# yangl1996/hbbft

Measured on AMD Instinct MI355X. Metric: RBC encode+Merkle+decode payload GB/s, N=64, 1/8 GPUs; fraction of HBM peak, higher is better.
Workload: dtype u8; 1 GPU; cfg3: N=64 f=21 (22+42 shards), 262144 B payloads, 32768 instances/GPU, f random erasures; n=64, f=21, payload_bytes=262144, instances_per_gpu=32768, global_batch=32768, parallelism=instance-sharded x1

## Files before the change

__graft_entry__.py:

```python
import os
import subprocess
import sys

ROOT = os.path.dirname(os.path.abspath(__file__))


def build_jobs():
    try:
        return max(1, int(os.environ["MAX_JOBS"]))
    except (KeyError, ValueError):
        return max(1, min(16, len(os.sched_getaffinity(0))))


def build():
    jobs = str(min(8, build_jobs()))
    oracle = subprocess.Popen(["make", "-s", "-j", "2", "-C", os.path.join(ROOT, "oracle")])
    try:
        subprocess.check_call(["make", "-s", "-j", jobs, "-C",
                               os.path.join(ROOT, "hbbft_amd", "csrc")])
    finally:
        rc = oracle.wait()
    if rc != 0:
        raise subprocess.CalledProcessError(rc, oracle.args)
    subprocess.check_call(["make", "-s", "-C", os.path.join(ROOT, "tests", "cpp")])
    if ROOT not in sys.path:
        sys.path.insert(0, ROOT)
    import hbbft_amd
    hbbft_amd.lib()
    todo = [t for t in jit_tasks() if not os.path.exists(
        os.path.join(ROOT, "hbbft_amd", "jit", _jit_name(*t)))]
    if todo:
        from concurrent.futures import ThreadPoolExecutor
        todo.sort(key=lambda t: -t[1] * t[2])
        with ThreadPoolExecutor(min(len(todo), build_jobs())) as pool:
            list(pool.map(_jit_spawn, todo))


def jit_tasks():
    if ROOT not in sys.path:
        sys.path.insert(0, ROOT)
    import hbbft_amd
    from hbbft_amd.sharded import Topology
    tasks = []
    for k, m in SPECIALISED:
        n = k + m
        for rb in [0] + [r for r in VALIDATOR_BLOCKS.get(n, []) if r < n]:
            tasks += [("enc", k, m, g, rb, None) for g in range(hbbft_amd.jit_encode_groups(k, m))]
    for n, pres, rb in decoder_patterns(Topology):
        f = (n - 1) // 3
        k, m = n - 2 * f, 2 * f
        kinds = ["dec", "decuf"]
        tasks += [(kind, k, m, g, rb, tuple(pres)) for kind in kinds
                  for g in range(hbbft_amd.jit_decode_groups(k, m, pres))]
    return tasks


def decoder_patterns(Topology):
    out = []
    n = 250
    f = (n - 1) // 3
    k = n - 2 * f
    out.append((n, [1 if k <= i < 2 * k else 0 for i in range(n)], 0))
    for nv in (16, 64, 128):
        for world in (1, 2, 4, 8):
            t = Topology(nv, world)
            for g in range(world):
                out.append((nv, t.receiver_present(g), t.rows_per_block))
    return out


def _jit_name(kind, k, m, group, rb, present):
    import hbbft_amd
    if kind == "enc":
        return hbbft_amd.jit_file_name(k, m, group, rb)
    return hbbft_amd.jit_decode_file_name(k, m, list(present), group, rb,
                                          fused_unframe=kind == "decuf")


_JIT_CHILD = ("import json, sys; sys.path.insert(0, sys.argv[1]); import __graft_entry__ as g; "
              "g._jit_one(*json.loads(sys.argv[2]))")


def _jit_spawn(task):
    import json
    subprocess.run([sys.executable, "-c", _JIT_CHILD, ROOT, json.dumps(task)], check=True,
                   stdin=subprocess.DEVNULL)


def _jit_one(kind, k, m, group, rb, present):
    if ROOT not in sys.path:
        sys.path.insert(0, ROOT)
    import hbbft_amd
    if kind == "enc":
        hbbft_amd.jit_build_encode(k, m, group=group, rows_per_block=rb)
    else:
        hbbft_amd.jit_build_decode(k, m, list(present), group, rows_per_block=rb,
                                   fused_unframe=kind == "decuf")


SPECIALISED = [(2, 2), (6, 10), (22, 42), (44, 84), (84, 166)]
VALIDATOR_BLOCKS = {16: [8, 4, 2], 64: [32, 16, 8], 128: [64, 32, 16]}


def smoke():
    if ROOT not in sys.path:
        sys.path.insert(0, ROOT)
    import numpy as np
    import torch

    import hbbft_amd as hb
    from oracle import pyoracle as orc

    assert torch.cuda.is_available(), "smoke() needs a GPU"
    from hbbft_amd.srchash import source_hash
    ver = hb.lib().hbrbc_version().decode()
    print("smoke: %s (tree src=%s)" % (ver, source_hash()))
    assert ver.endswith("src=" + source_hash()), "libhbrbc.so was not built from these sources"
    n, f, plen, count = 16, 5, 3000, 8
    rb = hb.RbcBatch(n, f, device=0)
    S = hb.shard_len(plen, rb.k)
    pay = np.stack([orc.gen_payload(7, i, plen) for i in range(count)])
    stride_p = (plen + 15) // 16 * 16
    payloads = torch.zeros((count, stride_p), dtype=torch.uint8, device="cuda:0")
    payloads[:, :plen] = torch.from_numpy(pay).cuda()
    slab = rb.alloc_slab(count, S)
    nodes = rb.alloc_nodes(count)
    rb.frame(payloads, plen, slab)
    rb.encode(slab, S)
    rb.merkle(slab, S, nodes)
    digests = torch.zeros((count, n, rb.dslots, 32), dtype=torch.uint8, device="cuda:0")
    ndig = torch.zeros((count, n), dtype=torch.uint8, device="cuda:0")
    rb.proofs(nodes, digests, ndig)
    ok = torch.zeros((count, n), dtype=torch.uint8, device="cuda:0")
    rb.validate(slab, S, digests, ndig, nodes, ok)
    present = torch.from_numpy(np.stack([orc.gen_present(9, i, n, f) for i in range(count)])).cuda()
    roots = nodes[:, -1, :].clone()
    slab2 = slab.clone()
    slab2[present == 0] = 0xA5
    nodes2 = rb.alloc_nodes(count)
    out = torch.zeros((count, (rb.k * S + 15) // 16 * 16), dtype=torch.uint8, device="cuda:0")
    plen_out = torch.zeros(count, dtype=torch.int32, device="cuda:0")
    status = torch.zeros(count, dtype=torch.int32, device="cuda:0")
    rb.decode(slab2, S, present, roots, nodes2, out, plen_out, status)
    torch.cuda.synchronize()
    slab_h, nodes_h = slab.cpu().numpy(), nodes.cpu().numpy()
    for i in range(count):
        sh, nd = orc.send_shards(n, f, pay[i].tobytes())
        assert np.array_equal(slab_h[i, :, :S], sh), "shards differ from oracle"
        assert np.array_equal(nodes_h[i], nd), "merkle nodes differ from oracle"
    assert ok.cpu().numpy().all(), "a valid proof was rejected"
    assert (status.cpu().numpy() == 0).all(), status
    assert (plen_out.cpu().numpy() == plen).all()
    assert np.array_equal(out.cpu().numpy()[:, :plen], pay), "decoded payload differs"
    print("smoke ok: N=%d f=%d P=%d x%d instances, bit-exact vs oracle" % (n, f, plen, count))

    from hbbft_amd import threshold as T
    from oracle import bls_oracle as B
    p1, q2 = B.g1_mul(B.G1_GEN, 5), B.g2_mul(B.G2_GEN, 7)
    g1 = torch.from_numpy(np.frombuffer(B.g1_bytes(p1), np.uint8).copy()).view(1, 96).cuda()
    g2 = torch.from_numpy(np.frombuffer(B.g2_bytes(q2), np.uint8).copy()).view(1, 192).cuda()
    gt, st = T.pairing_batch(g1, g2)
    assert st.item() == 0 and bytes(gt[0].cpu().numpy()) == B.gt_bytes(B.pairing(p1, q2)), \
        "pairing differs from oracle"
    cases = [B.decryption_share_case(3, 4, 5), B.decryption_share_case(3, 4, 5, tamper=True)]
    got = T.verify_decryption_shares([(B.g1_bytes(s), B.g1_bytes(pk), B.g2_bytes(h), B.g2_bytes(w))
                                      for s, h, pk, w in cases])
    assert got == [True, False], got
    print("smoke ok: BLS12-381 pairing bit-exact, decryption-share checks exact")


if __name__ == "__main__":
    build()
    if len(sys.argv) > 1 and sys.argv[1] == "smoke":
        smoke()
```

hbbft-hip/src/ffi.rs:

```rust
#![allow(non_camel_case_types, dead_code, clippy::too_many_arguments)]
use std::os::raw::{c_char, c_int, c_void};

#[repr(C)]
pub struct HbrbcCtx {
    _p: [u8; 0],
}

#[repr(C)]
#[derive(Clone, Copy)]
pub struct HbrbcSmArgs {
    pub count: usize,
    pub node_lo: u32,
    pub nodes: u32,
    pub rows_per_rank: u32,
    pub roots: u32,
    pub max_out: u32,
    pub max_faults: u32,
    pub round: i32,
    pub proposer: *const u8,
    pub role: *const u8,
    pub value_root: *const u8,
    pub value_tamper: *const u8,
    pub proof_ok: *const u8,
    pub decode_ok: *const u8,
    pub fake_from: *const u8,
    pub fake_root: *const u8,
    pub fake_list: *const u32,
    pub in_: *const u32,
    pub in_count: *const u32,
    pub out: *mut u32,
    pub out_count: *mut u32,
    pub state: *mut u8,
    pub output_root: *mut u8,
    pub faults: *mut u16,
    pub fault_count: *mut u32,
    pub emitted: *mut u32,
    pub active: *const u32,
    pub flags: u32,
}

extern "C" {
    pub fn hbrbc_last_error() -> *const c_char;
    pub fn hbrbc_version() -> *const c_char;
    pub fn hbrbc_coding_new(data_shards: usize, parity_shards: usize, device: c_int, out: *mut *mut HbrbcCtx) -> c_int;
    pub fn hbrbc_coding_free(ctx: *mut HbrbcCtx);
    pub fn hbrbc_data_shard_count(ctx: *const HbrbcCtx) -> usize;
    pub fn hbrbc_parity_shard_count(ctx: *const HbrbcCtx) -> usize;
    pub fn hbrbc_encoding_matrix(ctx: *const HbrbcCtx, out: *mut u8) -> c_int;
    pub fn hbrbc_stream(ctx: *const HbrbcCtx) -> *mut c_void;
    pub fn hbrbc_encode(ctx: *mut HbrbcCtx, shards: *const *mut u8, lens: *const usize, n_shards: usize) -> c_int;
    pub fn hbrbc_reconstruct(ctx: *mut HbrbcCtx, shards: *const *mut u8, lens: *const usize, present: *const u8, n_shards: usize) -> c_int;
    pub fn hbrbc_merkle_node_count(n: usize) -> usize;
    pub fn hbrbc_merkle_max_proof_len(n: usize) -> usize;
    pub fn hbrbc_merkle_build(values: *const *const u8, lens: *const usize, n: usize, nodes_out: *mut u8) -> c_int;
    pub fn hbrbc_merkle_proof(nodes: *const u8, n: usize, index: usize, digests_out: *mut u8, ndig_out: *mut usize) -> c_int;
    pub fn hbrbc_proof_validate(value: *const u8, len: usize, index: usize, digests: *const u8, ndig: usize, root: *const u8, n: usize, valid_out: *mut c_int) -> c_int;
    pub fn hbrbc_shard_len(payload_len: usize, data_shards: usize) -> usize;
    pub fn hbrbc_frame_batch(ctx: *mut HbrbcCtx, payloads: *const u8, payload_stride: usize, payload_len: usize, count: usize, shards: *mut u8, shard_len: usize, shard_stride: usize, inst_stride: usize, stream: *mut c_void) -> c_int;
    pub fn hbrbc_encode_batch(ctx: *mut HbrbcCtx, shards: *mut u8, shard_len: usize, shard_stride: usize, inst_stride: usize, count: usize, stream: *mut c_void) -> c_int;
    pub fn hbrbc_frame_encode_batch(ctx: *mut HbrbcCtx, payloads: *const u8, payload_stride: usize, payload_len: usize, count: usize, shards: *mut u8, shard_len: usize, shard_stride: usize, inst_stride: usize, stream: *mut c_void) -> c_int;
    pub fn hbrbc_frame_encode_ragged(ctx: *mut HbrbcCtx, payloads: *const u8, payload_stride: usize, payload_lens: *const u32, max_payload_len: usize, count: usize, shards: *mut u8, shard_stride: usize, inst_stride: usize, stream: *mut c_void) -> c_int;
    pub fn hbrbc_merkle_ragged(ctx: *mut HbrbcCtx, shards: *const u8, shard_lens: *const u32, shard_stride: usize, inst_stride: usize, count: usize, nodes: *mut u8, node_inst_stride: usize, stream: *mut c_void) -> c_int;
    pub fn hbrbc_merkle_batch(ctx: *mut HbrbcCtx, shards: *const u8, shard_len: usize, shard_stride: usize, inst_stride: usize, count: usize, nodes: *mut u8, node_inst_stride: usize, stream: *mut c_void) -> c_int;
    pub fn hbrbc_proofs_batch(ctx: *mut HbrbcCtx, nodes: *const u8, node_inst_stride: usize, count: usize, digests: *mut u8, ndig: *mut u8, stream: *mut c_void) -> c_int;
    pub fn hbrbc_validate_batch(ctx: *mut HbrbcCtx, values: *const u8, value_len: usize, value_stride: usize, value_inst_stride: usize, per_inst: usize, indices: *const u32, digests: *const u8, ndig: *const u8, roots: *const u8, root_stride: usize, tree_n: usize, count: usize, ok_out: *mut u8, stream: *mut c_void) -> c_int;
    pub fn hbrbc_reconstruct_batch(ctx: *mut HbrbcCtx, shards: *mut u8, shard_len: usize, shard_stride: usize, inst_stride: usize, present: *const u8, count: usize, status_out: *mut i32, stream: *mut c_void) -> c_int;
    pub fn hbrbc_decode_batch(ctx: *mut HbrbcCtx, shards: *mut u8, shard_len: usize, shard_stride: usize, inst_stride: usize, present: *const u8, count: usize, roots: *const u8, root_stride: usize, nodes: *mut u8, node_inst_stride: usize, payload_out: *mut u8, payload_stride: usize, payload_len_out: *mut u32, status_out: *mut i32, stream: *mut c_void) -> c_int;
    pub fn hbrbc_reserve(ctx: *mut HbrbcCtx, count: usize) -> c_int;
    pub fn hbrbc_frame_encode_rows(ctx: *mut HbrbcCtx, payloads: *const u8, payload_stride: usize, payload_len: usize, count: usize, shards: *mut u8, shard_len: usize, shard_stride: usize, rows_per_block: usize, block_stride: usize, inst_stride: usize, stream: *mut c_void) -> c_int;
    pub fn hbrbc_merkle_rows(ctx: *mut HbrbcCtx, shards: *const u8, shard_len: usize, shard_stride: usize, rows_per_block: usize, block_stride: usize, inst_stride: usize, count: usize, nodes: *mut u8, node_inst_stride: usize, stream: *mut c_void) -> c_int;
    pub fn hbrbc_validate_rows(ctx: *mut HbrbcCtx, values: *const u8, value_len: usize, value_stride: usize, rows_per_block: usize, block_stride: usize, value_inst_stride: usize, per_inst: usize, rows: *const u32, indices: *const u32, digests: *const u8, ndig: *const u8, digest_rows: usize, roots: *const u8, root_stride: usize, tree_n: usize, count: usize, ok_out: *mut u8, leaf_out: *mut u8, leaf_inst_stride: usize, stream: *mut c_void) -> c_int;
    pub fn hbrbc_reconstruct_rows(ctx: *mut HbrbcCtx, shards: *mut u8, shard_len: usize, shard_stride: usize, rows_per_block: usize, block_stride: usize, inst_stride: usize, present: *const u8, count: usize, status_out: *mut i32, stream: *mut c_void) -> c_int;
    pub fn hbrbc_decode_rows(ctx: *mut HbrbcCtx, shards: *mut u8, shard_len: usize, shard_stride: usize, rows_per_block: usize, block_stride: usize, inst_stride: usize, present: *const u8, count: usize, roots: *const u8, root_stride: usize, nodes: *mut u8, node_inst_stride: usize, known_leaves: c_int, payload_out: *mut u8, payload_stride: usize, payload_len_out: *mut u32, status_out: *mut i32, stream: *mut c_void) -> c_int;
    pub fn hbrbc_drop_rows(ctx: *mut HbrbcCtx, shards: *mut u8, shard_stride: usize, rows_per_block: usize, block_stride: usize, inst_stride: usize, present: *const u8, count: usize, fill: u8, stream: *mut c_void) -> c_int;
    pub fn hbrbc_decode_cache_clear(ctx: *mut HbrbcCtx) -> c_int;
    pub fn hbrbc_decode_cache_fill(ctx: *mut HbrbcCtx, patterns_out: *mut u32) -> c_int;
    pub fn hbrbc_decoder_specialise(ctx: *mut HbrbcCtx, present: *const u8, rows_per_block: usize) -> c_int;
    pub fn hbrbc_wire_proof_message_len(value_len: usize, ndig: usize) -> usize;
    pub fn hbrbc_wire_encode_batch(ctx: *mut HbrbcCtx, variant: u32, values: *const u8, value_len: usize, value_stride: usize, value_inst_stride: usize, per_inst: usize, indices: *const u32, digests: *const u8, ndig: *const u8, roots: *const u8, root_stride: usize, count: usize, out: *mut u8, msg_stride: usize, msg_len_out: *mut u32, stream: *mut c_void) -> c_int;
    pub fn hbrbc_wire_decode_batch(ctx: *mut HbrbcCtx, msgs: *const u8, msg_stride: usize, msg_len: *const u32, nmsg: usize, values: *mut u8, value_stride: usize, value_len_out: *mut u32, index_out: *mut u32, digests: *mut u8, ndig_out: *mut u8, roots: *mut u8, variant_out: *mut u32, status_out: *mut i32, stream: *mut c_void) -> c_int;
    pub fn hbrbc_encode_kernel(ctx: *const HbrbcCtx) -> *const c_char;
    pub fn hbrbc_jit_build_encode(data_shards: usize, parity_shards: usize, dir: *const c_char) -> c_int;
    pub fn hbrbc_jit_encode_groups(data_shards: usize, parity_shards: usize) -> usize;
    pub fn hbrbc_jit_build_encode_group(data_shards: usize, parity_shards: usize, group: usize, dir: *const c_char) -> c_int;
    pub fn hbrbc_jit_file_name(data_shards: usize, parity_shards: usize, group: usize, buf: *mut c_char, buf_len: usize) -> c_int;
    pub fn hbrbc_jit_build_encode_rows(data_shards: usize, parity_shards: usize, group: usize, rows_per_block: usize, dir: *const c_char) -> c_int;
    pub fn hbrbc_jit_encode_file_name(data_shards: usize, parity_shards: usize, group: usize, rows_per_block: usize, buf: *mut c_char, buf_len: usize) -> c_int;
    pub fn hbrbc_jit_decode_groups(data_shards: usize, parity_shards: usize, present: *const u8) -> usize;
    pub fn hbrbc_jit_build_decode(data_shards: usize, parity_shards: usize, present: *const u8, rows_per_block: usize, group: usize, dir: *const c_char) -> c_int;
    pub fn hbrbc_jit_build_decode_variant(data_shards: usize, parity_shards: usize, present: *const u8, rows_per_block: usize, group: usize, fused_unframe: c_int, dir: *const c_char) -> c_int;
    pub fn hbrbc_jit_decode_variant_file_name(data_shards: usize, parity_shards: usize, present: *const u8, rows_per_block: usize, group: usize, fused_unframe: c_int, buf: *mut c_char, buf_len: usize) -> c_int;
    pub fn hbrbc_jit_decode_file_name(data_shards: usize, parity_shards: usize, present: *const u8, rows_per_block: usize, group: usize, buf: *mut c_char, buf_len: usize) -> c_int;
    pub fn hbrbc_profile_enable(ctx: *mut HbrbcCtx, enable: c_int) -> c_int;
    pub fn hbrbc_profile_reset(ctx: *mut HbrbcCtx) -> c_int;
    pub fn hbrbc_profile_read(ctx: *mut HbrbcCtx, ms_out: *mut f64, launches_out: *mut u64) -> c_int;
    pub fn hbrbc_stage_name(stage: c_int) -> *const c_char;
    pub fn hbrbc_unframe_fused(ctx: *const HbrbcCtx, shard_len: usize, payload_stride: usize, rows_per_block: usize) -> c_int;
    pub fn hbrbc_pairing_workspace_size(pairings: usize) -> usize;
    pub fn hbrbc_pairing_batch(g1: *const u8, g2: *const u8, count: usize, gt_out: *mut u8, status_out: *mut u8, workspace: *mut c_void, stream: *mut c_void) -> c_int;
    pub fn hbrbc_pairing_check_batch(g1: *const u8, g2: *const u8, count: usize, ok_out: *mut u8, workspace: *mut c_void, stream: *mut c_void) -> c_int;
    pub fn hbrbc_g2_prepared_size(points: usize) -> usize;
    pub fn hbrbc_g2_prepare(g2: *const u8, count: usize, prepared: *mut c_void, stream: *mut c_void) -> c_int;
    pub fn hbrbc_pairing_check_prepared(g1: *const u8, prepared: *const c_void, points: usize, idx_b: *const u32, idx_d: *const u32, count: usize, ok_out: *mut u8, workspace: *mut c_void, stream: *mut c_void) -> c_int;
    pub fn hbrbc_g1_prepared_size(points: usize) -> usize;
    pub fn hbrbc_g1_prepare(g1: *const u8, count: usize, prepared: *mut c_void, stream: *mut c_void) -> c_int;
    pub fn hbrbc_pairing_check_prepared_keys(g1_a: *const u8, keys: *const c_void, key_points: usize, idx_c: *const u32, prepared: *const c_void, points: usize, idx_b: *const u32, idx_d: *const u32, count: usize, ok_out: *mut u8, workspace: *mut c_void, stream: *mut c_void) -> c_int;
    pub fn hbrbc_pairing_check_prepared_pts(a_prepared: *const c_void, keys: *const c_void, key_points: usize, idx_c: *const u32, prepared: *const c_void, points: usize, idx_b: *const u32, idx_d: *const u32, count: usize, ok_out: *mut u8, workspace: *mut c_void, stream: *mut c_void) -> c_int;
    pub fn hbrbc_pairing_check(a: *const u8, b: *const u8, c: *const u8, d: *const u8, result: *mut c_int) -> c_int;
    pub fn hbrbc_g1_combine_workspace_size(total_shares: usize, groups: usize) -> usize;
    pub fn hbrbc_lagrange_coeffs(idx: *const u32, offsets: *const u32, groups: usize, coeffs_out: *mut u8, status_out: *mut u8, stream: *mut c_void) -> c_int;
    pub fn hbrbc_g1_lincomb_prepared(a_prepared: *const c_void, prepared_count: usize, rows: *const i32, scalars: *const u8, offsets: *const u32, groups: usize, out96: *mut u8, out48: *mut u8, status_out: *mut u8, workspace: *mut c_void, stream: *mut c_void) -> c_int;
    pub fn hbrbc_decrypt_combine_prepared(a_prepared: *const c_void, prepared_count: usize, rows: *const i32, idx: *const u32, offsets: *const u32, groups: usize, out96: *mut u8, out48: *mut u8, status_out: *mut u8, workspace: *mut c_void, stream: *mut c_void) -> c_int;
    pub fn hbrbc_decrypt_combine(shares: *const u8, idx: *const u32, n: usize, out96: *mut u8, out48: *mut u8) -> c_int;
    pub fn hbrbc_g1_poly_eval_prepared(a_prepared: *const c_void, prepared_count: usize, rows: *const i32, offsets: *const u32, polys: usize, poly: *const i32, x: *const u32, evals: usize, out_table: *mut c_void, out96: *mut u8, out48: *mut u8, status_out: *mut u8, stream: *mut c_void) -> c_int;
    pub fn hbrbc_g1_base_mul_check(a_prepared: *const c_void, prepared_count: usize, rows: *const i32, scalars: *const u8, count: usize, ok_out: *mut u8, stream: *mut c_void) -> c_int;
    pub fn hbrbc_g2_points_size(points: usize) -> usize;
    pub fn hbrbc_g2_points_prepare(g2: *const u8, count: usize, table: *mut c_void, stream: *mut c_void) -> c_int;
    pub fn hbrbc_sig_check_prepared(sig_table: *const c_void, sig_count: usize, keys: *const c_void, key_points: usize, idx_key: *const u32, prepared: *const c_void, points: usize, idx_h: *const u32, count: usize, ok_out: *mut u8, workspace: *mut c_void, stream: *mut c_void) -> c_int;
    pub fn hbrbc_g2_combine_workspace_size(total_shares: usize, groups: usize) -> usize;
    pub fn hbrbc_g2_lincomb_prepared(sig_table: *const c_void, sig_count: usize, rows: *const i32, scalars: *const u8, offsets: *const u32, groups: usize, out192: *mut u8, out96: *mut u8, parity_out: *mut u8, status_out: *mut u8, workspace: *mut c_void, stream: *mut c_void) -> c_int;
    pub fn hbrbc_sig_combine_prepared(sig_table: *const c_void, sig_count: usize, rows: *const i32, idx: *const u32, offsets: *const u32, groups: usize, out192: *mut u8, out96: *mut u8, parity_out: *mut u8, status_out: *mut u8, workspace: *mut c_void, stream: *mut c_void) -> c_int;
    pub fn hbrbc_sig_combine(shares: *const u8, idx: *const u32, n: usize, out192: *mut u8, out96: *mut u8, parity: *mut u8) -> c_int;
    pub fn hbrbc_g1_prepare_compressed(g1c: *const u8, count: usize, prepared: *mut c_void, stream: *mut c_void) -> c_int;
    pub fn hbrbc_g2_points_prepare_compressed(g2c: *const u8, count: usize, table: *mut c_void, stream: *mut c_void) -> c_int;
    pub fn hbrbc_g1_decompress(g1c: *const u8, count: usize, out96: *mut u8, status: *mut u8, stream: *mut c_void) -> c_int;
    pub fn hbrbc_g2_decompress(g2c: *const u8, count: usize, out192: *mut u8, status: *mut u8, stream: *mut c_void) -> c_int;
    pub fn hbrbc_g1_base_mul(scalars: *const u8, count: usize, out_table: *mut c_void, out96: *mut u8, out48: *mut u8, status_out: *mut u8, stream: *mut c_void) -> c_int;
    pub fn hbrbc_g1_mul_prepared(a_prepared: *const c_void, prepared_count: usize, rows: *const i32, scalars: *const u8, nscalars: usize, sidx: *const i32, count: usize, out_table: *mut c_void, out96: *mut u8, out48: *mut u8, status_out: *mut u8, stream: *mut c_void) -> c_int;
    pub fn hbrbc_g2_mul_prepared(table: *const c_void, table_count: usize, rows: *const i32, scalars: *const u8, nscalars: usize, sidx: *const i32, count: usize, out_table: *mut c_void, out192: *mut u8, out96: *mut u8, status_out: *mut u8, stream: *mut c_void) -> c_int;
    pub fn hbrbc_fr_poly_eval(scalars: *const u8, nscalars: usize, rows: *const i32, offsets: *const u32, polys: usize, poly: *const i32, x: *const u32, evals: usize, out: *mut u8, status_out: *mut u8, stream: *mut c_void) -> c_int;
    pub fn hbrbc_fr_dot(a: *const u8, b: *const u8, offsets: *const u32, groups: usize, total: usize, out: *mut u8, status_out: *mut u8, stream: *mut c_void) -> c_int;
    pub fn hbrbc_sm_state_bytes(n: usize, roots: usize) -> usize;
    pub fn hbrbc_sm_round(ctx: *mut HbrbcCtx, args: *const HbrbcSmArgs, stream: *mut c_void) -> c_int;
}
```

hbbft_amd/__init__.py:

```python
import ctypes
import os

__all__ = [
    "RseError", "HbrbcUnavailable", "Coding", "MerkleTree", "Proof", "RbcBatch",
    "shard_len", "merkle_node_count", "max_proof_len", "lib", "LIB_PATH", "STAGES",
    "jit_build_encode", "jit_file_name", "WIRE_VARIANTS", "validate_proofs", "VALIDATE_STATS",
    "send_shards_batch", "SEND_STATS", "jit_decode_groups", "jit_build_decode",
    "jit_decode_file_name", "jit_encode_groups",
]

_HERE = os.path.dirname(os.path.abspath(__file__))
LIB_PATH = os.environ.get("HBRBC_LIB") or os.path.join(_HERE, "libhbrbc.so")

STATUS_NAMES = {
    0: "Ok", 1: "TooFewShards", 2: "TooManyShards", 3: "TooFewDataShards",
    4: "TooManyDataShards", 5: "TooFewParityShards", 6: "TooManyParityShards",
    7: "TooFewBufferShards", 8: "TooManyBufferShards", 9: "IncorrectShardSize",
    10: "TooFewShardsPresent", 11: "EmptyShard", 12: "InvalidShardFlags", 13: "InvalidIndex",
    64: "SingularMatrix", 65: "RootMismatch", 66: "NoPayloadLen",
    70: "WireTruncated", 71: "WireBadVariant", 72: "WireTooLarge",
    100: "InvalidArgument", 101: "DeviceError", 102: "NoDevice",
}
WIRE_VARIANTS = {"Value": 0, "Echo": 1, "Ready": 2, "CanDecode": 3, "EchoHash": 4}
STAGES = ["frame", "encode", "leaf_hash", "tree_levels", "proofs", "validate",
          "decode_matrix", "reconstruct", "unframe"]


class HbrbcUnavailable(RuntimeError):
    """libhbrbc.so is missing or no HIP device is visible (no fallback exists)."""


class RseError(Exception):

    def __init__(self, code, msg=""):
        self.code = code
        self.msg = msg
        self.name = STATUS_NAMES.get(code, "Status%d" % code)
        super().__init__("%s%s" % (self.name, (": " + msg) if msg else ""))

    def __reduce__(self):
        return (RseError, (self.code, self.msg))


_lib = None
_P = ctypes.c_void_p
_S = ctypes.c_size_t


def lib():
    global _lib
    if _lib is not None:
        return _lib
    if not os.path.exists(LIB_PATH):
        raise HbrbcUnavailable("%s not built (run __graft_entry__.build())" % LIB_PATH)
    L = ctypes.CDLL(LIB_PATH)
    sig = {
        "hbrbc_last_error": (ctypes.c_char_p, []),
        "hbrbc_version": (ctypes.c_char_p, []),
        "hbrbc_coding_new": (ctypes.c_int, [_S, _S, ctypes.c_int, ctypes.POINTER(_P)]),
        "hbrbc_coding_free": (None, [_P]),
        "hbrbc_data_shard_count": (_S, [_P]),
        "hbrbc_parity_shard_count": (_S, [_P]),
        "hbrbc_encoding_matrix": (ctypes.c_int, [_P, _P]),
        "hbrbc_stream": (_P, [_P]),
        "hbrbc_encode": (ctypes.c_int, [_P, _P, _P, _S]),
        "hbrbc_reconstruct": (ctypes.c_int, [_P, _P, _P, _P, _S]),
        "hbrbc_merkle_node_count": (_S, [_S]),
        "hbrbc_merkle_max_proof_len": (_S, [_S]),
        "hbrbc_merkle_build": (ctypes.c_int, [_P, _P, _S, _P]),
        "hbrbc_merkle_proof": (ctypes.c_int, [_P, _S, _S, _P, ctypes.POINTER(_S)]),
        "hbrbc_proof_validate": (ctypes.c_int, [_P, _S, _S, _P, _S, _P, _S,
                                                ctypes.POINTER(ctypes.c_int)]),
        "hbrbc_shard_len": (_S, [_S, _S]),
        "hbrbc_frame_batch": (ctypes.c_int, [_P, _P, _S, _S, _S, _P, _S, _S, _S, _P]),
        "hbrbc_encode_batch": (ctypes.c_int, [_P, _P, _S, _S, _S, _S, _P]),
        "hbrbc_frame_encode_batch": (ctypes.c_int, [_P, _P, _S, _S, _S, _P, _S, _S, _S, _P]),
        "hbrbc_merkle_batch": (ctypes.c_int, [_P, _P, _S, _S, _S, _S, _P, _S, _P]),
        "hbrbc_proofs_batch": (ctypes.c_int, [_P, _P, _S, _S, _P, _P, _P]),
        "hbrbc_validate_batch": (ctypes.c_int, [_P, _P, _S, _S, _S, _S, _P, _P, _P, _P, _S, _S,
                                                _S, _P, _P]),
        "hbrbc_reconstruct_batch": (ctypes.c_int, [_P, _P, _S, _S, _S, _P, _S, _P, _P]),
        "hbrbc_decode_batch": (ctypes.c_int, [_P, _P, _S, _S, _S, _P, _S, _P, _S, _P, _S, _P, _S,
                                              _P, _P, _P]),
        "hbrbc_reserve": (ctypes.c_int, [_P, _S]),
        "hbrbc_profile_enable": (ctypes.c_int, [_P, ctypes.c_int]),
        "hbrbc_profile_reset": (ctypes.c_int, [_P]),
        "hbrbc_profile_read": (ctypes.c_int, [_P, _P, _P]),
        "hbrbc_stage_name": (ctypes.c_char_p, [ctypes.c_int]),
        "hbrbc_encode_kernel": (ctypes.c_char_p, [_P]),
        "hbrbc_wire_proof_message_len": (_S, [_S, _S]),
        "hbrbc_wire_encode_batch": (ctypes.c_int, [_P, ctypes.c_uint32, _P, _S, _S, _S, _S, _P, _P,
                                                   _P, _P, _S, _S, _P, _S, _P, _P]),
        "hbrbc_wire_decode_batch": (ctypes.c_int, [_P, _P, _S, _P, _S, _P, _S, _P, _P, _P, _P, _P,
                                                   _P, _P, _P]),
        "hbrbc_jit_build_encode": (ctypes.c_int, [_S, _S, ctypes.c_char_p]),
        "hbrbc_jit_encode_groups": (_S, [_S, _S]),
        "hbrbc_jit_build_encode_group": (ctypes.c_int, [_S, _S, _S, ctypes.c_char_p]),
        "hbrbc_jit_file_name": (ctypes.c_int, [_S, _S, _S, ctypes.c_char_p, _S]),
        "hbrbc_frame_encode_rows": (ctypes.c_int, [_P, _P, _S, _S, _S, _P, _S, _S, _S, _S, _S, _P]),
        "hbrbc_frame_encode_ragged": (ctypes.c_int, [_P, _P, _S, _P, _S, _S, _P, _S, _S, _P]),
        "hbrbc_merkle_ragged": (ctypes.c_int, [_P, _P, _P, _S, _S, _S, _P, _S, _P]),
        "hbrbc_merkle_rows": (ctypes.c_int, [_P, _P, _S, _S, _S, _S, _S, _S, _P, _S, _P]),
        "hbrbc_validate_rows": (ctypes.c_int, [_P, _P, _S, _S, _S, _S, _S, _S, _P, _P, _P, _P, _S,
                                               _P, _S, _S, _S, _P, _P, _S, _P]),
        "hbrbc_reconstruct_rows": (ctypes.c_int, [_P, _P, _S, _S, _S, _S, _S, _P, _S, _P, _P]),
        "hbrbc_decode_rows": (ctypes.c_int, [_P, _P, _S, _S, _S, _S, _S, _P, _S, _P, _S, _P, _S,
                                             ctypes.c_int, _P, _S, _P, _P, _P]),
        "hbrbc_decode_cache_clear": (ctypes.c_int, [_P]),
        "hbrbc_decode_cache_fill": (ctypes.c_int, [_P, ctypes.POINTER(ctypes.c_uint32)]),
        "hbrbc_decoder_specialise": (ctypes.c_int, [_P, _P, _S]),
        "hbrbc_jit_build_encode_rows": (ctypes.c_int, [_S, _S, _S, _S, ctypes.c_char_p]),
        "hbrbc_jit_encode_file_name": (ctypes.c_int, [_S, _S, _S, _S, ctypes.c_char_p, _S]),
        "hbrbc_jit_decode_groups": (_S, [_S, _S, _P]),
        "hbrbc_jit_build_decode": (ctypes.c_int, [_S, _S, _P, _S, _S, ctypes.c_char_p]),
        "hbrbc_jit_decode_file_name": (ctypes.c_int, [_S, _S, _P, _S, _S, ctypes.c_char_p, _S]),
        "hbrbc_jit_build_decode_variant": (ctypes.c_int, [_S, _S, _P, _S, _S, ctypes.c_int,
                                                          ctypes.c_char_p]),
        "hbrbc_jit_decode_variant_file_name": (ctypes.c_int, [_S, _S, _P, _S, _S, ctypes.c_int,
                                                              ctypes.c_char_p, _S]),
        "hbrbc_unframe_fused": (ctypes.c_int, [_P, _S, _S, _S]),
        "hbrbc_drop_rows": (ctypes.c_int, [_P, _P, _S, _S, _S, _S, _P, _S, ctypes.c_uint8, _P]),
        "hbrbc_pairing_workspace_size": (_S, [_S]),
        "hbrbc_g2_prepared_size": (_S, [_S]),
        "hbrbc_g2_prepare": (ctypes.c_int, [_P, _S, _P, _P]),
        "hbrbc_pairing_check_prepared": (ctypes.c_int, [_P, _P, _S, _P, _P, _S, _P, _P, _P]),
        "hbrbc_pairing_batch": (ctypes.c_int, [_P, _P, _S, _P, _P, _P, _P]),
        "hbrbc_pairing_check_batch": (ctypes.c_int, [_P, _P, _S, _P, _P, _P]),
        "hbrbc_g1_prepared_size": (_S, [_S]),
        "hbrbc_g1_prepare": (ctypes.c_int, [_P, _S, _P, _P]),
        "hbrbc_pairing_check_prepared_keys": (ctypes.c_int, [_P, _P, _S, _P, _P, _S, _P, _P, _S, _P,
                                                             _P, _P]),
        "hbrbc_pairing_check_prepared_pts": (ctypes.c_int, [_P, _P, _S, _P, _P, _S, _P, _P, _S, _P,
                                                            _P, _P]),
        "hbrbc_pairing_check": (ctypes.c_int, [ctypes.c_char_p, ctypes.c_char_p, ctypes.c_char_p,
                                               ctypes.c_char_p, ctypes.POINTER(ctypes.c_int)]),
        "hbrbc_g1_combine_workspace_size": (_S, [_S, _S]),
        "hbrbc_lagrange_coeffs": (ctypes.c_int, [_P, _P, _S, _P, _P, _P]),
        "hbrbc_g1_lincomb_prepared": (ctypes.c_int, [_P, _S, _P, _P, _P, _S, _P, _P, _P, _P, _P]),
        "hbrbc_decrypt_combine_prepared": (ctypes.c_int, [_P, _S, _P, _P, _P, _S, _P, _P, _P, _P,
                                                          _P]),
        "hbrbc_decrypt_combine": (ctypes.c_int, [ctypes.c_char_p, _P, _S, ctypes.c_char_p,
                                                 ctypes.c_char_p]),
        "hbrbc_g2_points_size": (_S, [_S]),
        "hbrbc_g2_points_prepare": (ctypes.c_int, [_P, _S, _P, _P]),
        "hbrbc_sig_check_prepared": (ctypes.c_int, [_P, _S, _P, _S, _P, _P, _S, _P, _S, _P, _P,
                                                    _P]),
        "hbrbc_g2_combine_workspace_size": (_S, [_S, _S]),
        "hbrbc_g2_lincomb_prepared": (ctypes.c_int, [_P, _S, _P, _P, _P, _S, _P, _P, _P, _P, _P,
                                                     _P]),
        "hbrbc_sig_combine_prepared": (ctypes.c_int, [_P, _S, _P, _P, _P, _S, _P, _P, _P, _P, _P,
                                                      _P]),
        "hbrbc_sig_combine": (ctypes.c_int, [ctypes.c_char_p, _P, _S, ctypes.c_char_p,
                                             ctypes.c_char_p, ctypes.c_char_p]),
        "hbrbc_g1_prepare_compressed": (ctypes.c_int, [_P, _S, _P, _P]),
        "hbrbc_g2_points_prepare_compressed": (ctypes.c_int, [_P, _S, _P, _P]),
        "hbrbc_g1_decompress": (ctypes.c_int, [_P, _S, _P, _P, _P]),
        "hbrbc_g2_decompress": (ctypes.c_int, [_P, _S, _P, _P, _P]),
        "hbrbc_g1_poly_eval_prepared": (ctypes.c_int, [_P, _S, _P, _P, _S, _P, _P, _S, _P, _P, _P,
                                                       _P, _P]),
        "hbrbc_g1_base_mul_check": (ctypes.c_int, [_P, _S, _P, _P, _S, _P, _P]),
        "hbrbc_g1_base_mul": (ctypes.c_int, [_P, _S, _P, _P, _P, _P, _P]),
        "hbrbc_g1_mul_prepared": (ctypes.c_int, [_P, _S, _P, _P, _S, _P, _S, _P, _P, _P, _P, _P]),
        "hbrbc_g2_mul_prepared": (ctypes.c_int, [_P, _S, _P, _P, _S, _P, _S, _P, _P, _P, _P, _P]),
        "hbrbc_fr_poly_eval": (ctypes.c_int, [_P, _S, _P, _P, _S, _P, _P, _S, _P, _P, _P]),
        "hbrbc_fr_dot": (ctypes.c_int, [_P, _P, _P, _S, _S, _P, _P, _P]),
    }
    for name, (res, args) in sig.items():
        fn = getattr(L, name)
        fn.restype = res
        fn.argtypes = args
    _lib = L
    return L


def _check(code):
    if code == 102:
        raise HbrbcUnavailable(lib().hbrbc_last_error().decode(errors="replace") or "no HIP device")
    if code != 0:
        raise RseError(code, lib().hbrbc_last_error().decode(errors="replace"))


def jit_build_encode(data_shards, parity_shards, directory=None, group=None, rows_per_block=0):
    d = directory.encode() if directory else None
    groups = range(jit_encode_groups(data_shards, parity_shards)) if group is None else [group]
    for g in groups:
        _check(lib().hbrbc_jit_build_encode_rows(data_shards, parity_shards, g, rows_per_block, d))


def jit_file_name(data_shards, parity_shards, group=0, rows_per_block=0):
    buf = ctypes.create_string_buffer(256)
    _check(lib().hbrbc_jit_encode_file_name(data_shards, parity_shards, group, rows_per_block,
                                            buf, 256))
    return buf.value.decode()


def _mask_buffer(present):
    import numpy as np
    return np.ascontiguousarray(np.asarray(present, dtype=np.uint8) != 0, dtype=np.uint8)


def jit_decode_groups(data_shards, parity_shards, present):
    m = _mask_buffer(present)
    return lib().hbrbc_jit_decode_groups(data_shards, parity_shards, m.ctypes.data)


def jit_build_decode(data_shards, parity_shards, present, group, rows_per_block=0,
                     directory=None, fused_unframe=False):
    m = _mask_buffer(present)
    d = directory.encode() if directory else None
    _check(lib().hbrbc_jit_build_decode_variant(data_shards, parity_shards, m.ctypes.data,
                                                rows_per_block, group, int(fused_unframe), d))


def jit_decode_file_name(data_shards, parity_shards, present, group=0, rows_per_block=0,
                         fused_unframe=False):
    m = _mask_buffer(present)
    buf = ctypes.create_string_buffer(256)
    _check(lib().hbrbc_jit_decode_variant_file_name(data_shards, parity_shards, m.ctypes.data,
                                                    rows_per_block, group, int(fused_unframe),
                                                    buf, 256))
    return buf.value.decode()


def jit_encode_groups(data_shards, parity_shards):
    return lib().hbrbc_jit_encode_groups(data_shards, parity_shards)


def shard_len(payload_len, data_shards):
    return (payload_len + 4 + data_shards - 1) // data_shards


def merkle_node_count(n):
    total, sz = 0, n
    while True:
        total += sz
        if sz <= 1:
            return total
        sz = (sz + 1) // 2


def max_proof_len(n):
    d, sz = 0, n
    while sz > 1:
        d += 1
        sz = (sz + 1) // 2
    return d


def _as_buffer(b):
    import numpy as np
    if isinstance(b, np.ndarray):
        assert b.dtype == np.uint8 and b.flags.c_contiguous
        return b
    if isinstance(b, bytearray):
        return np.frombuffer(b, dtype=np.uint8)
    return np.frombuffer(bytearray(b), dtype=np.uint8)


def _addr(a):
    return a.ctypes.data if a.size else 0


class Coding:

    def __init__(self, data_shard_num, parity_shard_num, device=-1):
        h = _P()
        _check(lib().hbrbc_coding_new(data_shard_num, parity_shard_num, device, ctypes.byref(h)))
        self._h = h

    @classmethod
    def for_validators(cls, n, device=-1):
        f = (n - 1) // 3
        return cls(n - 2 * f, 2 * f, device)

    @property
    def handle(self):
        return self._h

    def close(self):
        if self._h:
            lib().hbrbc_coding_free(self._h)
            self._h = None

    def __del__(self):
        try:
            self.close()
        except Exception:
            pass

    def data_shard_count(self):
        return lib().hbrbc_data_shard_count(self._h)

    def encode_kernel(self):
        return lib().hbrbc_encode_kernel(self._h).decode()

    def parity_shard_count(self):
        return lib().hbrbc_parity_shard_count(self._h)

    def encoding_matrix(self):
        import numpy as np
        k, m = self.data_shard_count(), self.parity_shard_count()
        out = np.zeros((k + m, k), np.uint8)
        _check(lib().hbrbc_encoding_matrix(self._h, out.ctypes.data))
        return out

    def encode(self, shards):
# ... 242 lines not shown
                                        slab.stride(0), slab.shape[0], self._stream(stream)))

    def merkle(self, slab, S, nodes, stream=None):
        _check(lib().hbrbc_merkle_batch(self.coding.handle, _ptr(slab), S, slab.stride(1),
                                        slab.stride(0), slab.shape[0], _ptr(nodes),
                                        nodes.stride(0), self._stream(stream)))

    def proofs(self, nodes, digests, ndig, stream=None):
        _check(lib().hbrbc_proofs_batch(self.coding.handle, _ptr(nodes), nodes.stride(0),
                                        nodes.shape[0], _ptr(digests), _ptr(ndig),
                                        self._stream(stream)))

    def validate(self, slab, S, digests, ndig, nodes, ok, indices=None, leaf_out=None,
                 stream=None):
        count = slab.shape[0]
        root = nodes[:, -1, :]
        if leaf_out is not None:
            self.validate_layout(slab, S, count, self.n, slab.stride(1), 0, 0, slab.stride(0),
                                 digests, ndig, self.n, root, ok, indices=indices,
                                 leaf_out=leaf_out, stream=stream)
            return
        _check(lib().hbrbc_validate_batch(self.coding.handle, _ptr(slab), S, slab.stride(1),
                                          slab.stride(0), self.n, _ptr(indices), _ptr(digests),
                                          _ptr(ndig), _ptr(root), nodes.stride(0), self.n,
                                          count, _ptr(ok), self._stream(stream)))

    def validate_rows(self, values, S, per_inst, indices, digests, ndig, roots, ok, stream=None):
        count = values.shape[0]
        for t in (indices, digests, ndig, ok):
            assert t.is_contiguous() and t.shape[0] == count and t.shape[1] == per_inst
        _check(lib().hbrbc_validate_batch(self.coding.handle, _ptr(values), S, values.stride(1),
                                          values.stride(0), per_inst, _ptr(indices), _ptr(digests),
                                          _ptr(ndig), _ptr(roots), roots.stride(0), self.n, count,
                                          _ptr(ok), self._stream(stream)))

    def frame_encode_ragged(self, payloads, plens, max_plen, slab, stream=None):
        _check(lib().hbrbc_frame_encode_ragged(self.coding.handle, _ptr(payloads),
                                               payloads.stride(0), _ptr(plens), max_plen,
                                               slab.shape[0], _ptr(slab), slab.stride(1),
                                               slab.stride(0), self._stream(stream)))

    def merkle_ragged(self, slab, slens, nodes, stream=None):
        _check(lib().hbrbc_merkle_ragged(self.coding.handle, _ptr(slab), _ptr(slens),
                                         slab.stride(1), slab.stride(0), slab.shape[0],
                                         _ptr(nodes), nodes.stride(0), self._stream(stream)))

    def frame_encode_rows(self, payloads, plen, base, count, shard_stride, rows_per_block,
                          block_stride, inst_stride, stream=None):
        S = shard_len(plen, self.k)
        _check(lib().hbrbc_frame_encode_rows(self.coding.handle, _ptr(payloads), payloads.stride(0),
                                             plen, count, _ptr(base), S, shard_stride,
                                             rows_per_block, block_stride, inst_stride,
                                             self._stream(stream)))

    def merkle_rows(self, base, S, count, shard_stride, rows_per_block, block_stride, inst_stride,
                    nodes, stream=None):
        _check(lib().hbrbc_merkle_rows(self.coding.handle, _ptr(base), S, shard_stride,
                                       rows_per_block, block_stride, inst_stride, count,
                                       _ptr(nodes), nodes.stride(0), self._stream(stream)))

    def validate_layout(self, base, S, count, per_inst, shard_stride, rows_per_block, block_stride,
                        inst_stride, digests, ndig, digest_rows, roots, ok, rows=None,
                        indices=None, leaf_out=None, stream=None):
        _check(lib().hbrbc_validate_rows(
            self.coding.handle, _ptr(base), S, shard_stride, rows_per_block, block_stride,
            inst_stride, per_inst, _ptr(rows), _ptr(indices), _ptr(digests), _ptr(ndig),
            digest_rows, _ptr(roots), roots.stride(0), self.n, count, _ptr(ok), _ptr(leaf_out),
            leaf_out.stride(0) if leaf_out is not None else 0, self._stream(stream)))

    def decode_rows(self, base, S, count, shard_stride, rows_per_block, block_stride, inst_stride,
                    present, roots, nodes, payload_out, plen_out, status, known_leaves=False,
                    stream=None):
        _check(lib().hbrbc_decode_rows(
            self.coding.handle, _ptr(base), S, shard_stride, rows_per_block, block_stride,
            inst_stride, _ptr(present), count, _ptr(roots), roots.stride(0), _ptr(nodes),
            nodes.stride(0), 1 if known_leaves else 0, _ptr(payload_out), payload_out.stride(0),
            _ptr(plen_out), _ptr(status), self._stream(stream)))

    def specialise_decoder(self, present, rows_per_block=0):
        m = _mask_buffer(present)
        assert m.size == self.n
        _check(lib().hbrbc_decoder_specialise(self.coding.handle, m.ctypes.data, rows_per_block))

    def decode_cache_clear(self):
        _check(lib().hbrbc_decode_cache_clear(self.coding.handle))

    def decode_cache_fill(self):
        v = ctypes.c_uint32(0)
        _check(lib().hbrbc_decode_cache_fill(self.coding.handle, ctypes.byref(v)))
        return v.value

    def reconstruct(self, slab, S, present, status, stream=None):
        _check(lib().hbrbc_reconstruct_batch(self.coding.handle, _ptr(slab), S, slab.stride(1),
                                             slab.stride(0), _ptr(present), slab.shape[0],
                                             _ptr(status), self._stream(stream)))

    def drop_rows(self, slab, present, fill=0xA5, stream=None):
        _check(lib().hbrbc_drop_rows(self.coding.handle, _ptr(slab), slab.stride(1), 0, 0,
                                     slab.stride(0), _ptr(present), slab.shape[0], fill,
                                     self._stream(stream)))

    def unframe_fused(self, S, payload_stride, rows_per_block=0):
        return bool(lib().hbrbc_unframe_fused(self.coding.handle, S, payload_stride,
                                              rows_per_block))

    def decode(self, slab, S, present, roots, nodes, payload_out, plen_out, status,
               known_leaves=False, stream=None):
        if known_leaves:
            self.decode_rows(slab, S, slab.shape[0], slab.stride(1), 0, 0, slab.stride(0),
                             present, roots, nodes, payload_out, plen_out, status,
                             known_leaves=True, stream=stream)
            return
        _check(lib().hbrbc_decode_batch(self.coding.handle, _ptr(slab), S, slab.stride(1),
                                        slab.stride(0), _ptr(present), slab.shape[0],
                                        _ptr(roots), roots.stride(0), _ptr(nodes),
                                        nodes.stride(0), _ptr(payload_out),
                                        payload_out.stride(0), _ptr(plen_out), _ptr(status),
                                        self._stream(stream)))

    def wire_slot(self, S):
        return (lib().hbrbc_wire_proof_message_len(S, self.dslots) + 15) // 16 * 16

    def wire_encode(self, values, S, digests, ndig, roots, out, msg_len, variant=0, indices=None,
                    stream=None):
        count, per_inst = values.shape[0], values.shape[1]
        _check(lib().hbrbc_wire_encode_batch(self.coding.handle, variant, _ptr(values), S,
                                             values.stride(1), values.stride(0), per_inst,
                                             _ptr(indices), _ptr(digests), _ptr(ndig),
                                             _ptr(roots), roots.stride(0), count, _ptr(out),
                                             out.stride(0), _ptr(msg_len), self._stream(stream)))

    def wire_decode(self, msgs, msg_len, values, value_len, index, digests, ndig, roots, variant,
                    status, stream=None):
        _check(lib().hbrbc_wire_decode_batch(self.coding.handle, _ptr(msgs), msgs.stride(0),
                                             _ptr(msg_len), msgs.shape[0], _ptr(values),
                                             values.stride(0), _ptr(value_len), _ptr(index),
                                             _ptr(digests), _ptr(ndig), _ptr(roots), _ptr(variant),
                                             _ptr(status), self._stream(stream)))

    def own_stream(self):
        import torch
        return torch.cuda.ExternalStream(lib().hbrbc_stream(self.coding.handle), device=self.device)

    def reserve(self, count):
        _check(lib().hbrbc_reserve(self.coding.handle, count))

    def profile(self, enable=True):
        _check(lib().hbrbc_profile_enable(self.coding.handle, 1 if enable else 0))

    def profile_reset(self):
        _check(lib().hbrbc_profile_reset(self.coding.handle))

    def profile_read(self):
        ms = (ctypes.c_double * len(STAGES))()
        cnt = (ctypes.c_uint64 * len(STAGES))()
        _check(lib().hbrbc_profile_read(self.coding.handle, ms, cnt))
        return {STAGES[i]: (ms[i], cnt[i]) for i in range(len(STAGES))}


SEND_STATS = {"trees": 0, "launches": 0}
_SEND_BATCH = {}


def send_shards_batch(items, device=0):
    import numpy as np
    import torch
# ... 91 lines not shown
```

hbbft_amd/csrc/api.hip:

```cpp
#include <hip/hip_runtime.h>

#include <algorithm>
#include <cstdarg>
#include <cstdio>
#include <cstdlib>
#include <cstring>
#include <map>
#include <mutex>
#include <string>
#include <vector>

#include <dlfcn.h>
#include <sys/stat.h>

#include "../../include/hbrbc.h"
#include "device_common.hpp"
#include "jit.hpp"
#include "launchers.hpp"

using namespace hbrbc;

namespace {

thread_local std::string g_err;
// ... 138 lines not shown
            p = nullptr;
            cap = 0;
        }
        size_t b = round_up(bytes < 256 ? 256 : bytes, 256);
        hipError_t e = hipMalloc(&p, b);
        if (e == hipSuccess) cap = b;
        return e;
    }
    void release() {
        if (p) (void)hipFree(p);
        p = nullptr;
        cap = 0;
    }
    template <class T>
    T *as() const {
        return static_cast<T *>(p);
    }
};

struct PinBuf {
    void *p = nullptr;
    size_t cap = 0;
    hipError_t ensure(size_t bytes) {
        if (bytes <= cap) return hipSuccess;
        if (p) {
            (void)hipHostFree(p);
            p = nullptr;
            cap = 0;
        }
        size_t b = round_up(bytes < 4096 ? 4096 : bytes, 4096);
        hipError_t e = hipHostMalloc(&p, b, hipHostMallocDefault);
        if (e == hipSuccess) cap = b;
        return e;
    }
    void release() {
        if (p) (void)hipHostFree(p);
        p = nullptr;
        cap = 0;
    }
    template <class T>
    T *as() const {
        return static_cast<T *>(p);
    }
};

RowMap make_rows(size_t n, size_t shard_stride, size_t rows_per_block, size_t block_stride) {
    RowMap r = plain_rows(shard_stride);
    if (rows_per_block && rows_per_block < n) {
        r.rb = (uint32_t)rows_per_block;
        r.bst = block_stride;
    }
    return r;
}
inline int code_rb(const RowMap &r) { return r.plain() ? 256 : (int)r.rb; }

}

struct hbrbc_ctx {
    int device = 0;
    size_t k = 0, m = 0, n = 0;
    int rt_enc = 2, rt_rec = 2;
    int gf_mode = 0;
    std::vector<uint8_t> matrix;
    hipStream_t stream = nullptr;
    struct SpecGroup {
        int r_lo, r_hi;
        hipModule_t mod;
        hipFunction_t fn, fe;
        bool lds = false;
    };
    std::map<int, std::vector<SpecGroup>> enc_spec;
    int rt_spec = 2;
    int depth_spec = 4;
    std::string enc_kind = "none";
    struct DecSpec {
        uint64_t hash;
        int rt;
        std::vector<SpecGroup> groups;
        std::vector<SpecGroup> uf_groups;
        int uf_state = 0;
        std::vector<uint8_t> present;
    };
    std::map<int, DecSpec> dec_spec;
    std::string jit_missing;
    std::vector<hipStream_t> side;
    std::vector<hipEvent_t> side_ev;
    DevBuf d_matrix, d_enc_coefs, d_enc_in, d_enc_out;
    size_t ws_count = 0;
    int pc_cap = 0;
    size_t pc_inserted = 0;
    DevBuf pc_hash, pc_keys, pc_coefs, pc_in, pc_out, pc_nout, pc_status, pc_fill;
    DevBuf ws_pat, ws_own, ws_status, ws_list, ws_counter;
    std::mutex shim_mu;
    DevBuf st_slab, st_nodes, st_aux;
    PinBuf pin;
    bool prof = false;
    std::vector<hipEvent_t> ev_pool;
    size_t ev_used = 0;
    struct Rec {
        int stage;
        hipEvent_t a, b;
    };
    std::vector<Rec> recs;

    hipEvent_t take_event() {
        if (ev_used == ev_pool.size()) {
            hipEvent_t e;
            if (hipEventCreate(&e) != hipSuccess) return nullptr;
            ev_pool.push_back(e);
        }
        return ev_pool[ev_used++];
    }
    size_t coef_stride() const { return (m + rt_rec - 1) / rt_rec * k * 16 + 16; }
};

namespace {

struct StageTimer {
    hbrbc_ctx *c;
    int stage;
    hipStream_t s;
    hipEvent_t a = nullptr;
    StageTimer(hbrbc_ctx *c_, int st, hipStream_t s_) : c(c_), stage(st), s(s_) {
        if (c && c->prof) {
            a = c->take_event();
            if (a) (void)hipEventRecord(a, s);
        }
    }
    ~StageTimer() {
        if (a) {
            hipEvent_t b = c->take_event();
            if (b) {
                (void)hipEventRecord(b, s);
                c->recs.push_back({stage, a, b});
            }
        }
    }
};

inline hipStream_t pick(hbrbc_ctx *, void *stream) { return static_cast<hipStream_t>(stream); }

int check_slab(const void *base, size_t shard_len, size_t shard_stride, size_t inst_stride,
               size_t n, size_t count, size_t rows_per_block = 0, size_t block_stride = 0) {
    if (count == 0) return HBRBC_OK;
    if (!base) return fail(HBRBC_E_INVALID_ARG, "null shard slab");
    if (reinterpret_cast<uintptr_t>(base) % 16)
        return fail(HBRBC_E_INVALID_ARG, "shard slab base must be 16-byte aligned");
    if (shard_stride % 16 || shard_stride < shard_len)
        return fail(HBRBC_E_INVALID_ARG, "shard_stride %zu must be a multiple of 16 and >= %zu",
                    shard_stride, shard_len);
    if (shard_len > 0xFFFFFFFFull) return fail(HBRBC_E_INVALID_ARG, "shard_len too large");
    if (rows_per_block && rows_per_block < n) {
        if (rows_per_block > 255)
            return fail(HBRBC_E_INVALID_ARG, "rows_per_block %zu > 255", rows_per_block);
        if (block_stride % 16 || inst_stride % 16 || inst_stride < rows_per_block * shard_stride)
            return fail(HBRBC_E_INVALID_ARG, "blocked layout: inst_stride %zu must be a multiple "
                        "of 16 and >= rows_per_block * shard_stride", inst_stride);
        if (block_stride < count * inst_stride)
            return fail(HBRBC_E_INVALID_ARG, "blocked layout: block_stride %zu < count * "
                        "inst_stride", block_stride);
        if ((uint64_t)rows_per_block * shard_stride >= 0x7FFFFFFFull)
            return fail(HBRBC_E_INVALID_ARG, "row block larger than 2 GiB");
        return HBRBC_OK;
    }
    if (count > 1 && (inst_stride % 16 || inst_stride < n * shard_stride))
        return fail(HBRBC_E_INVALID_ARG, "inst_stride %zu must be a multiple of 16 and >= %zu",
                    inst_stride, n * shard_stride);
    return HBRBC_OK;
}

int check_nodes(const void *nodes, size_t node_inst_stride, size_t n, size_t count) {
    if (count == 0) return HBRBC_OK;
    if (!nodes || reinterpret_cast<uintptr_t>(nodes) % 16)
        return fail(HBRBC_E_INVALID_ARG, "node slab must be non-null and 16-byte aligned");
    if (node_inst_stride % 16 || (count > 1 && node_inst_stride < 32 * hbrbc_merkle_node_count(n)))
        return fail(HBRBC_E_INVALID_ARG, "node_inst_stride %zu too small or unaligned",
                    node_inst_stride);
    return HBRBC_OK;
}

int ensure_workspace(hbrbc_ctx *c, size_t count) {
    if (count <= c->ws_count) return HBRBC_OK;
    const size_t k = c->k, m = c->m;
    int cap = 1024;
    while ((size_t)cap < 2 * count) cap *= 2;
    const size_t slots = (size_t)cap + count;
    HB_HIP(c->pc_hash.ensure((size_t)cap * sizeof(uint64_t)));
    HB_HIP(c->pc_keys.ensure(slots * 8 * sizeof(uint32_t)));
    HB_HIP(c->pc_coefs.ensure(slots * c->coef_stride()));
    HB_HIP(c->pc_in.ensure((slots * k + 4) * sizeof(uint32_t)));
    HB_HIP(c->pc_out.ensure((slots * m + 4) * sizeof(uint32_t)));
    HB_HIP(c->pc_nout.ensure(slots * sizeof(int)));
    HB_HIP(c->pc_status.ensure(slots * sizeof(int32_t)));
    HB_HIP(c->pc_fill.ensure(sizeof(uint32_t)));
    HB_HIP(c->ws_pat.ensure(count * sizeof(int)));
    HB_HIP(c->ws_own.ensure(count));
    HB_HIP(c->ws_status.ensure(count * sizeof(int32_t)));
    HB_HIP(c->ws_list.ensure((count * std::max<size_t>(m, 1) + 1) * sizeof(uint2)));
    HB_HIP(c->ws_counter.ensure(sizeof(uint32_t)));
    HB_HIP(hipMemset(c->pc_hash.p, 0, (size_t)cap * sizeof(uint64_t)));
    HB_HIP(hipMemset(c->pc_fill.p, 0, sizeof(uint32_t)));
    c->pc_cap = cap;
    c->pc_inserted = 0;
    c->ws_count = count;
    return HBRBC_OK;
}

PatternCache cache_view(hbrbc_ctx *c) {
    PatternCache pc;
    pc.hash = c->pc_hash.as<uint64_t>();
    pc.keys = c->pc_keys.as<uint32_t>();
    pc.coefs = c->pc_coefs.as<uint8_t>();
    pc.coef_stride = c->coef_stride();
    pc.in_idx = c->pc_in.as<uint32_t>();
    pc.out_idx = c->pc_out.as<uint32_t>();
    pc.nout = c->pc_nout.as<int>();
    pc.status = c->pc_status.as<int32_t>();
    pc.fill = c->pc_fill.as<uint32_t>();
    pc.cap = c->pc_cap;
    return pc;
}

bool merkle_split() {
    const char *e = getenv("HBRBC_MERKLE_FUSED");
    return !(e && !std::strcmp(e, "1"));
}

int run_merkle(hbrbc_ctx *c, const uint8_t *shards, size_t shard_len, const RowMap &rows,
               size_t inst_stride, size_t n, size_t count, uint8_t *nodes,
               size_t node_inst_stride, bool known_leaves, hipStream_t s) {
    if (!known_leaves && merkle_fused_ok(n) && !merkle_split()) {
        StageTimer t(c, HBRBC_STAGE_LEAF_HASH, s);
        HB_HIP(launch_merkle_fused(shards, shard_len, rows, inst_stride, n, count, nodes,
                                   node_inst_stride, s));
        return HBRBC_OK;
    }
    {
        StageTimer t(c, HBRBC_STAGE_LEAF_HASH, s);
        if (!known_leaves) {
            HB_HIP(launch_leaf_hash(shards, shard_len, rows, inst_stride, n, count, nodes,
                                    node_inst_stride, s));
        } else if (c->m > 0) {
            HB_HIP(launch_leaf_hash_rebuilt(shards, shard_len, rows, inst_stride, count,
                                            c->ws_pat.as<int>(), c->pc_out.as<uint32_t>(), c->m,
                                            c->pc_nout.as<int>(), (int)c->m, nodes,
                                            node_inst_stride, c->ws_counter.as<uint32_t>(),
                                            c->ws_list.as<uint2>(), s));
        }
    }
    StageTimer t(c, HBRBC_STAGE_TREE_LEVELS, s);
    const char *lv = getenv("HBRBC_TREE_LEVELS_LDS");
    if (n <= 512 && lv && !std::strcmp(lv, "1")) {
        HB_HIP(launch_tree_levels(nodes, node_inst_stride, n, count, s));
        return HBRBC_OK;
    }
    size_t off = 0, sz = n;
    while (sz > 1) {
        const size_t nsz = (sz + 1) / 2;
        HB_HIP(launch_tree_level(nodes, node_inst_stride, off, sz, off + sz, nsz, count, s));
        off += sz;
        sz = nsz;
    }
    return HBRBC_OK;
}

hipError_t launch_xor_group(const hbrbc_ctx::SpecGroup &g, bool fused, int rt, XorArgs a,
                            size_t count, hipStream_t s);
hipError_t launch_groups(hbrbc_ctx *c, const std::vector<hbrbc_ctx::SpecGroup> &gs, size_t first,
                         int rt, const XorArgs &x, size_t count, hipStream_t s);

bool unframe_fusable(const hbrbc_ctx *c, size_t shard_len, size_t payload_stride) {
    const char *e = getenv("HBRBC_UNFRAME_FUSED");
    if (e && !std::strcmp(e, "0")) return false;
    return c->m > 0 && payload_stride % 16 == 0 && (uint64_t)c->k * shard_len > 4;
}

enum JitMode { JIT_DEFAULT, JIT_OFF, JIT_COMPILE, JIT_LOAD };
JitMode jit_mode() {
    const char *e = getenv("HBRBC_JIT");
    if (!e) return JIT_DEFAULT;
    if (!std::strcmp(e, "0")) return JIT_OFF;
    if (!std::strcmp(e, "1")) return JIT_COMPILE;
    if (!std::strcmp(e, "load")) return JIT_LOAD;
    return JIT_DEFAULT;
}

bool decode_programs(const std::vector<uint8_t> &mat, size_t k, size_t n, const uint8_t *present,
                     int rb, std::vector<XorProgram> &out, uint64_t &hash, int &rt, bool uf);
int load_program(const XorProgram &p, bool compile, hbrbc_ctx::SpecGroup &g);
void drop_groups(std::vector<hbrbc_ctx::SpecGroup> &gs);

bool uf_decoder(hbrbc_ctx *c, hbrbc_ctx::DecSpec &d, int rb) {
    if (d.uf_state == 0) {
        std::vector<XorProgram> progs;
        uint64_t hash = 0;
        int rt = 2;
        const bool compile = jit_mode() == JIT_DEFAULT || jit_mode() == JIT_COMPILE;
        const std::string saved = g_err;
        d.uf_state = -1;
        if (decode_programs(c->matrix, c->k, c->n, d.present.data(), rb, progs, hash, rt, true)) {
            d.uf_state = 1;
            for (const auto &p : progs) {
                hbrbc_ctx::SpecGroup g{0, (int)p.out_rows.size(), nullptr, nullptr, nullptr};
                if (load_program(p, compile, g)) {
                    drop_groups(d.uf_groups);
                    d.uf_state = -1;
                    break;
                }
                d.uf_groups.push_back(g);
            }
        }
        g_err = saved;
    }
    return d.uf_state == 1;
}

int run_reconstruct(hbrbc_ctx *c, uint8_t *shards, size_t shard_len, const RowMap &rows,
                    size_t inst_stride, const uint8_t *present, size_t count, int32_t *status,
                    hipStream_t s, uint8_t *uf_payload = nullptr, size_t uf_stride = 0,
                    bool *fused_out = nullptr) {
    if (fused_out) *fused_out = false;
    int st = ensure_workspace(c, count);
    if (st) return st;
    if (c->pc_inserted + count > 4 * (size_t)c->pc_cap) {
        HB_HIP(hipMemsetAsync(c->pc_hash.p, 0, (size_t)c->pc_cap * sizeof(uint64_t), s));
        HB_HIP(hipMemsetAsync(c->pc_fill.p, 0, sizeof(uint32_t), s));
        c->pc_inserted = 0;
    }
    c->pc_inserted += count;
    const auto ds = c->dec_spec.find(code_rb(rows));
    const bool spec = ds != c->dec_spec.end() && !ds->second.groups.empty();
    {
        StageTimer t(c, HBRBC_STAGE_DECODE_MATRIX, s);
        DecodeMatrixArgs a;
        a.n = (int)c->n;
        a.k = (int)c->k;
        a.rt = c->rt_rec;
        a.matrix = c->d_matrix.as<uint8_t>();
        a.present = present;
        a.count = count;
        a.cache = cache_view(c);
        a.pat = c->ws_pat.as<int>();
        a.own = c->ws_own.as<uint8_t>();
        a.status = status;
        if (spec) {
            a.spec_hash = ds->second.hash;
            pattern_mask(ds->second.present.data(), (int)c->n, a.spec_mask);
        }
        HB_HIP(launch_decode_matrix(a, s));
    }
    if (c->m == 0) return HBRBC_OK;
    StageTimer t(c, HBRBC_STAGE_RECONSTRUCT, s);
    if (spec && uf_payload && !uf_decoder(c, ds->second, code_rb(rows))) uf_payload = nullptr;
    if (spec) {
        XorArgs x{};
        x.base = shards;
        x.inst_stride = inst_stride;
        x.shard_stride = rows.sst;
        x.block_stride = rows.bst;
        x.row_bytes = (unsigned)round_up(shard_len, 16);
        x.pat = c->ws_pat.as<int>();
        x.slot_hash = reinterpret_cast<const unsigned long *>(c->pc_hash.as<uint64_t>());
        x.hash_slots = c->pc_cap;
        x.p_only = -1;
        x.S = (unsigned)shard_len;
        if (uf_payload) {
            x.uf_payload = uf_payload;
            x.uf_stride = uf_stride;
            x.uf_status = status;
        }
        HB_HIP(launch_groups(c, uf_payload ? ds->second.uf_groups : ds->second.groups, 0,
                             ds->second.rt, x, count, s));
    }
    GfApplyArgs g{};
    g.base = shards;
    g.inst_stride = inst_stride;
    g.rows = rows;
    g.n16 = (int)((shard_len + 15) / 16);
    g.coefs = c->pc_coefs.as<uint8_t>();
    g.coef_slot_stride = c->coef_stride();
    g.in_idx = c->pc_in.as<uint32_t>();
    g.in_idx_stride = c->k;
    g.out_idx = c->pc_out.as<uint32_t>();
    g.out_idx_stride = c->m;
    g.nout = c->pc_nout.as<int>();
    g.nout_uniform = 0;
    g.pat = c->ws_pat.as<int>();
    g.slot_hash = c->pc_hash.as<uint64_t>();
    g.skip_hash = spec ? ds->second.hash : 0;
    g.hash_slots = c->pc_cap;
    g.max_rows = (int)c->m;
    g.nin = (int)c->k;
    g.rt = c->rt_rec;
    g.mode = c->gf_mode;
    g.count = count;
    if (uf_payload) {
        g.payload = uf_payload;
        g.payload_stride = uf_stride;
        g.payload_S = (uint32_t)shard_len;
        g.payload_k = (uint32_t)c->k;
        g.rstatus = status;
        if (fused_out) *fused_out = true;
    }
    HB_HIP(launch_gf_apply(g, s));
    return HBRBC_OK;
}

std::string jit_dir() {
    if (const char *e = getenv("HBRBC_JIT_DIR")) return e;
    Dl_info info;
    if (dladdr(reinterpret_cast<void *>(&hbrbc_version), &info) && info.dli_fname) {
        std::string p = info.dli_fname;
        const size_t cut = p.find_last_of('/');
        return (cut == std::string::npos ? std::string(".") : p.substr(0, cut)) + "/jit";
    }
    return "jit";
}

std::string jit_file(const std::string &dir, const std::string &kernel) {
    const char *aux = getenv("HBRBC_ST_AUX");
    return dir + "/" + kernel + (aux && std::strcmp(aux, "2") ? std::string("_a") + aux : std::string()) +
           "_v23.co";
}

int spec_depth() {
    if (const char *e = getenv("HBRBC_JIT_DEPTH")) return std::max(1, std::min(8, atoi(e)));
    return 4;
}

int spec_fdepth() {
    if (const char *e = getenv("HBRBC_JIT_FDEPTH")) return std::max(1, std::min(8, atoi(e)));
    return 2;
}

bool spec_spread() {
    const char *e = getenv("HBRBC_JIT_SPREAD");
    return !(e && !std::strcmp(e, "0"));
}

bool spec_split() {
    const char *e = getenv("HBRBC_JIT_SPLIT");
    return !(e && !std::strcmp(e, "0"));
}

int spec_sync() {
    if (const char *e = getenv("HBRBC_JIT_SYNC")) return std::max(0, std::min(64, atoi(e)));
    return 0;
}

bool spec_lds(size_t nin, size_t nout) {
    if (const char *e = getenv("HBRBC_JIT_LDS")) return !std::strcmp(e, "1");
    return nin >= 16 && nout >= 14;
}

int spec_net() {
    if (const char *e = getenv("HBRBC_JIT_NET")) return std::max(0, std::min(2, atoi(e)));
    return 0;
}

int spec_lds_stage() {
    if (const char *e = getenv("HBRBC_JIT_LDS_STAGE")) return std::max(1, std::min(32, atoi(e)));
    return 0;
}
// ... 59 lines not shown
    XorProgram p;
    p.sync = spec_sync();
    p.fdepth = spec_fdepth();
    p.spread = spec_spread();
    p.split = spec_split();
    p.name = encode_kernel_name(k, m, rt, depth, r_lo, r_hi, rb, p.sync, p.fdepth, p.spread, p.split);
    for (size_t j = 0; j < k; ++j) p.in_rows.push_back((int)j);
    for (int r = r_lo; r < r_hi; ++r) p.out_rows.push_back((int)(k + r));
    p.coefs.assign(parity_rows + (size_t)r_lo * k, parity_rows + (size_t)r_hi * k);
    p.rt = rt;
    p.depth = depth;
    p.rb = rb;
    p.fused = true;
    spec_variant(p);
    return p;
}

bool decode_programs(const std::vector<uint8_t> &mat, size_t k, size_t n, const uint8_t *present,
                     int rb, std::vector<XorProgram> &out, uint64_t &hash, int &rt,
                     bool uf = false) {
    std::vector<int> valid, missing;
    std::vector<uint8_t> rows;
    if (!recovery_rows(mat, k, n, present, valid, missing, rows)) return false;
    hash = pattern_hash(present, (int)n);
    rt = spec_row_tile(k, missing.size());
    const int depth = spec_depth();
    const auto groups = xor_groups(k, missing.size(), rt);
    out.clear();
    for (size_t gi = 0; gi < groups.size(); ++gi) {
        XorProgram p;
        p.sync = spec_sync();
        p.split = spec_split();
        p.name = decode_kernel_name(n, hash, rt, depth, groups[gi].first, groups[gi].second, rb,
                                    p.sync, p.split) + (uf ? "_uf" : "");
        p.in_rows = valid;
        p.out_rows.assign(missing.begin() + groups[gi].first, missing.begin() + groups[gi].second);
        p.coefs.assign(rows.begin() + (size_t)groups[gi].first * k,
                       rows.begin() + (size_t)groups[gi].second * k);
        p.rt = rt;
        p.depth = depth;
        p.rb = rb;
        p.guard = hash;
        p.uf_k = uf ? (int)k : 0;
        p.uf_inputs = uf && gi == 0;
        if (uf) p.name.resize(p.name.size() - 3);
        spec_variant(p);
        if (uf) p.name += "_uf";
        out.push_back(std::move(p));
    }
    return true;
}

int load_program(const XorProgram &p, bool compile, hbrbc_ctx::SpecGroup &g) {
    const std::string path = jit_file(jit_dir(), p.name);
    std::vector<char> code;
    if (!read_file(path, code)) {
        if (!compile) return fail(HBRBC_E_INVALID_ARG, "no cached code object %s", path.c_str());
        std::string log;
        if (compile_source(gen_xor_source(p), code, log))
            return fail(HBRBC_E_DEVICE, "hiprtc: %s", log.substr(0, 400).c_str());
        mkdir(jit_dir().c_str(), 0755);
        (void)write_file(path, code);
    }
    g.mod = nullptr;
    g.fn = g.fe = nullptr;
    const int npass = (int)((p.out_rows.size() + p.rt - 1) / p.rt);
    g.lds = p.lds && npass >= 2 && npass <= 8;
    HB_HIP(hipModuleLoadData(&g.mod, code.data()));
    if (hipModuleGetFunction(&g.fn, g.mod, p.name.c_str()) != hipSuccess ||
        (p.fused && hipModuleGetFunction(&g.fe, g.mod, (p.name + "_fe").c_str()) != hipSuccess)) {
        (void)hipModuleUnload(g.mod);
        g.mod = nullptr;
        return fail(HBRBC_E_DEVICE, "kernel missing in %s", path.c_str());
    }
    return HBRBC_OK;
}

void drop_groups(std::vector<hbrbc_ctx::SpecGroup> &gs) {
    for (auto &g : gs)
        if (g.mod) (void)hipModuleUnload(g.mod);
    gs.clear();
}

const std::vector<hbrbc_ctx::SpecGroup> *spec_encoder(hbrbc_ctx *c, int rb) {
    auto it = c->enc_spec.find(rb);
    if (it != c->enc_spec.end()) return it->second.empty() ? nullptr : &it->second;
    std::vector<hbrbc_ctx::SpecGroup> gs;
    const bool off = c->m == 0 || jit_mode() == JIT_OFF || c->k * c->m > 16384;
    if (!off) {
        const bool compile = jit_mode() == JIT_COMPILE;
        const std::string saved = g_err;
        for (const auto &rg : xor_groups(c->k, c->m, c->rt_spec)) {
            const XorProgram p = encode_program(c->k, c->m, c->matrix.data() + c->k * c->k,
                                                c->rt_spec, c->depth_spec, rg.first, rg.second, rb);
            hbrbc_ctx::SpecGroup g{rg.first, rg.second, nullptr, nullptr, nullptr};
            if (load_program(p, compile, g)) {
                drop_groups(gs);
                break;
            }
            gs.push_back(g);
        }
        if (gs.empty() && jit_mode() == JIT_LOAD) {
            c->jit_missing = g_err;
        } else {
            g_err = saved;
        }
    }
    auto &slot = c->enc_spec[rb];
    slot = std::move(gs);
    return slot.empty() ? nullptr : &slot;
}

bool spec_pass_split() {
    const char *e = getenv("HBRBC_SPEC_SPLIT");
    return e && !std::strcmp(e, "1");
}

hipError_t launch_xor_group(const hbrbc_ctx::SpecGroup &g, bool fused, int rt, XorArgs a,
                            size_t count, hipStream_t s) {
    a.waves_per_row = (a.row_bytes + 64 * 32 - 1) / (64 * 32);
    const size_t blocks = (size_t)a.waves_per_row * count;
    if (blocks > 0xFFFFFFFFull) return hipErrorInvalidValue;
    const int npass = (g.r_hi - g.r_lo + rt - 1) / rt;
    void *args[] = {&a.base,     &a.inst_stride, &a.shard_stride, &a.block_stride,
                    &a.row_bytes, &a.waves_per_row, &a.payloads,  &a.payload_stride,
                    &a.P,        &a.S,           &a.pat,          &a.slot_hash,
                    &a.hash_slots, &a.p_only,     &a.uf_payload,   &a.uf_stride,
                    &a.uf_status};
    hipFunction_t fn = fused ? g.fe : g.fn;
    if (!spec_pass_split() || g.lds) {
        a.p_only = -1;
        const unsigned threads = 64u * (unsigned)xor_waves(npass);
        return hipModuleLaunchKernel(fn, (unsigned)blocks, 1, 1, threads, 1, 1, 0, s, args, nullptr);
    }
    for (a.p_only = 0; a.p_only < npass; ++a.p_only) {
        const hipError_t e = hipModuleLaunchKernel(fn, (unsigned)blocks, 1, 1, 64u, 1, 1, 0, s, args,
                                                   nullptr);
        if (e != hipSuccess) return e;
    }
    return hipSuccess;
}

bool xor_streams() {
    const char *e = getenv("HBRBC_XOR_STREAMS");
    return e && !std::strcmp(e, "1");
}

size_t xor_tile() {
    const char *e = getenv("HBRBC_XOR_TILE");
    return e ? (size_t)atoll(e) : 0;
}

hipError_t launch_groups(hbrbc_ctx *c, const std::vector<hbrbc_ctx::SpecGroup> &gs, size_t first,
                         int rt, const XorArgs &x, size_t count, hipStream_t s) {
    const size_t ng = gs.size() - first;
    if (ng == 0) return hipSuccess;
    const size_t tile = xor_tile();
    if (ng > 1 && tile && count > tile) {
        for (size_t i0 = 0; i0 < count; i0 += tile) {
            XorArgs y = x;
            y.base = x.base + i0 * x.inst_stride;
            if (y.payloads) y.payloads = x.payloads + i0 * x.payload_stride;
            if (y.pat) y.pat = x.pat + i0;
            if (y.uf_payload) y.uf_payload = x.uf_payload + i0 * x.uf_stride;
            if (y.uf_status) y.uf_status = x.uf_status + i0;
            const size_t cnt = std::min(tile, count - i0);
// ... 103 lines not shown
                    payload_len, c->k);
    if (payload_len > 0xFFFFFFFFull) return fail(HBRBC_E_INVALID_ARG, "payload too large");
    if (payload_len && (!payloads || reinterpret_cast<uintptr_t>(payloads) % 4 ||
                        payload_stride % 4 || payload_stride < round_up(payload_len, 4)))
        return fail(HBRBC_E_INVALID_ARG, "payload buffer must be 4-byte aligned with stride >= "
                                         "round_up(len, 4)");
    return HBRBC_OK;
}

int decode_rows(hbrbc_ctx *c, uint8_t *shards, size_t shard_len, const RowMap &rows,
                size_t inst_stride, const uint8_t *present, size_t count, const uint8_t *roots,
                size_t root_stride, uint8_t *nodes, size_t node_inst_stride, bool known_leaves,
                uint8_t *payload_out, size_t payload_stride, uint32_t *payload_len_out,
                int32_t *status_out, hipStream_t s) {
    int st = ensure_workspace(c, count);
    if (st) return st;
    int32_t *rstat = c->ws_status.as<int32_t>();
    bool fused = false;
    const bool fusable = unframe_fusable(c, shard_len, payload_stride);
    st = run_reconstruct(c, shards, shard_len, rows, inst_stride, present, count, rstat, s,
                         fusable ? payload_out : nullptr, payload_stride, &fused);
    if (st) return st;
    st = run_merkle(c, shards, shard_len, rows, inst_stride, c->n, count, nodes, node_inst_stride,
                    known_leaves, s);
    if (st) return st;
    StageTimer t(c, HBRBC_STAGE_UNFRAME, s);
    HB_HIP(launch_decode_check(rstat, nodes, node_inst_stride, hbrbc_merkle_node_count(c->n) - 1,
                               roots, root_stride, shards, shard_len, rows, inst_stride, c->k,
                               count, payload_len_out, status_out, s));
    if (fused)
        HB_HIP(launch_unframe_fixup(shards, (uint32_t)shard_len, rows, inst_stride, (uint32_t)c->k,
                                    count, payload_len_out, status_out, payload_out,
                                    payload_stride, s));
    else
        HB_HIP(launch_unframe(shards, shard_len, rows, inst_stride, c->k, count, payload_len_out,
                              status_out, payload_out, payload_stride, s));
    return HBRBC_OK;
}

}

extern "C" {

const char *hbrbc_last_error(void) { return g_err.c_str(); }

int hbrbc_coding_new(size_t data_shards, size_t parity_shards, int device, hbrbc_ctx **out) {
    if (!out) return fail(HBRBC_E_INVALID_ARG, "out is null");
    *out = nullptr;
    if (data_shards == 0) return fail(HBRBC_E_TOO_FEW_DATA_SHARDS, "no data shards");
    if (data_shards + parity_shards > 256)
        return fail(HBRBC_E_TOO_MANY_SHARDS, "data + parity = %zu > 256",
                    data_shards + parity_shards);
    int ndev = 0;
    if (hipGetDeviceCount(&ndev) != hipSuccess || ndev == 0)
        return fail(HBRBC_E_NO_DEVICE, "no HIP device visible");
    if (device < 0) HB_HIP(hipGetDevice(&device));
    if (device >= ndev) return fail(HBRBC_E_NO_DEVICE, "device %d of %d", device, ndev);
    HB_HIP(hipSetDevice(device));
    static std::once_flag cfg_once;
    static hipError_t cfg_err = hipSuccess;
    std::call_once(cfg_once, [] { cfg_err = configure_kernels(); });
    HB_HIP(cfg_err);

    hbrbc_ctx *c = new hbrbc_ctx();
    c->device = device;
    c->k = data_shards;
    c->m = parity_shards;
    c->n = data_shards + parity_shards;
    c->rt_enc = gf_row_tile((int)c->m);
    {
        const int h = (int)((c->m + 1) / 2);
        int rt = ((h + 3) / 4 + 1) & ~1;
        if (rt < 6) rt = (h + 1) & ~1;
        c->rt_rec = std::max(2, std::min(16, std::max(rt, std::min(6, (h + 1) & ~1))));
        if (c->rt_rec == 6 && (h + 6) / 7 < (h + 5) / 6) c->rt_rec = 7;
        if (h >= 14 && h <= 42) c->rt_rec = 7;
    }
    if (const char *e = getenv("HBRBC_GF")) {
        if (!std::strcmp(e, "bitslice_likely")) c->gf_mode = 1;
        else if (!std::strcmp(e, "bitslice_mask")) c->gf_mode = 2;
        else if (!std::strcmp(e, "bitslice_pair")) c->gf_mode = 3;
        else if (!std::strcmp(e, "bitslice_x2")) c->gf_mode = 4;
        else c->gf_mode = 0;
    }
    if (const char *e = getenv("HBRBC_RT_ENC")) c->rt_enc = std::max(2, std::min(16, atoi(e) & ~1));
    if (const char *e = getenv("HBRBC_RT_REC")) {
        const int r = atoi(e);
        c->rt_rec = (r == 5 || r == 7) ? r : std::max(2, std::min(16, r & ~1));
    }
    if (!build_matrix(c->k, c->n, c->matrix)) {
        delete c;
        return fail(HBRBC_E_SINGULAR_MATRIX, "singular Vandermonde top block");
    }
    int st = HBRBC_OK;
    auto guard = [&](hipError_t e) {
        if (e != hipSuccess && st == HBRBC_OK)
            st = fail(HBRBC_E_DEVICE, "context setup: %s", hipGetErrorString(e));
    };
    guard(hipStreamCreateWithFlags(&c->stream, hipStreamNonBlocking));
    guard(c->d_matrix.ensure(c->matrix.size()));
    if (st == HBRBC_OK)
        guard(hipMemcpy(c->d_matrix.p, c->matrix.data(), c->matrix.size(), hipMemcpyHostToDevice));
    if (c->m > 0 && st == HBRBC_OK) {
        const size_t rt = (size_t)c->rt_enc, npass = (c->m + rt - 1) / rt;
        std::vector<uint8_t> tab(npass * c->k * 16, 0);
        for (size_t r = 0; r < c->m; ++r)
            for (size_t j = 0; j < c->k; ++j)
                tab[((r / rt) * c->k + j) * 16 + (r % rt)] = c->matrix[(c->k + r) * c->k + j];
        std::vector<uint32_t> in(c->k), outi(c->m);
        for (size_t j = 0; j < c->k; ++j) in[j] = (uint32_t)j;
        for (size_t r = 0; r < c->m; ++r) outi[r] = (uint32_t)(c->k + r);
        guard(c->d_enc_coefs.ensure(tab.size()));
        guard(c->d_enc_in.ensure(in.size() * sizeof(uint32_t)));
        guard(c->d_enc_out.ensure(outi.size() * sizeof(uint32_t)));
        if (st == HBRBC_OK) {
            guard(hipMemcpy(c->d_enc_coefs.p, tab.data(), tab.size(), hipMemcpyHostToDevice));
            guard(hipMemcpy(c->d_enc_in.p, in.data(), in.size() * sizeof(uint32_t),
                            hipMemcpyHostToDevice));
            guard(hipMemcpy(c->d_enc_out.p, outi.data(), outi.size() * sizeof(uint32_t),
                            hipMemcpyHostToDevice));
        }
    }
    if (st != HBRBC_OK) {
        hbrbc_coding_free(c);
        return st;
    }
    c->rt_spec = spec_row_tile(c->k, c->m);
    c->depth_spec = spec_depth();
    c->enc_kind = c->m == 0 ? "trivial" : (spec_encoder(c, 256) ? "specialised" : "bitslice");
    if (c->m > 0 && c->enc_kind == "bitslice") {
        if (jit_mode() == JIT_COMPILE && c->k * c->m <= 16384) c->enc_kind = "jit-failed";
        if (jit_mode() == JIT_LOAD && c->k * c->m <= 16384) {
            const std::string msg = c->jit_missing;
            hbrbc_coding_free(c);
            return fail(HBRBC_E_INVALID_ARG, "HBRBC_JIT=load: %s", msg.c_str());
        }
    }
    *out = c;
    return HBRBC_OK;
}

void hbrbc_coding_free(hbrbc_ctx *c) {
    if (!c) return;
    (void)hipSetDevice(c->device);
    if (c->stream) (void)hipStreamSynchronize(c->stream);
    for (DevBuf *b : {&c->d_matrix, &c->d_enc_coefs, &c->d_enc_in, &c->d_enc_out, &c->pc_hash,
                      &c->pc_keys, &c->pc_coefs, &c->pc_in, &c->pc_out, &c->pc_nout, &c->pc_status,
                      &c->pc_fill, &c->ws_pat, &c->ws_own, &c->ws_status, &c->ws_list,
                      &c->ws_counter, &c->st_slab, &c->st_nodes, &c->st_aux})
        b->release();
    c->pin.release();
    for (hipEvent_t e : c->ev_pool) (void)hipEventDestroy(e);
    for (hipEvent_t e : c->side_ev) (void)hipEventDestroy(e);
    for (hipStream_t q : c->side) (void)hipStreamDestroy(q);
    for (auto &kv : c->enc_spec) drop_groups(kv.second);
    for (auto &kv : c->dec_spec) {
        drop_groups(kv.second.groups);
        drop_groups(kv.second.uf_groups);
    }
    if (c->stream) (void)hipStreamDestroy(c->stream);
    delete c;
}

size_t hbrbc_data_shard_count(const hbrbc_ctx *c) { return c ? c->k : 0; }
size_t hbrbc_parity_shard_count(const hbrbc_ctx *c) { return c ? c->m : 0; }
void *hbrbc_stream(const hbrbc_ctx *c) { return c ? c->stream : nullptr; }

int hbrbc_encoding_matrix(const hbrbc_ctx *c, uint8_t *out) {
    if (!c || !out) return fail(HBRBC_E_INVALID_ARG, "null argument");
    std::memcpy(out, c->matrix.data(), c->matrix.size());
    return HBRBC_OK;
}

size_t hbrbc_shard_len(size_t payload_len, size_t data_shards) {
    return data_shards ? (payload_len + 4 + data_shards - 1) / data_shards : 0;
}

size_t hbrbc_merkle_node_count(size_t n) {
    size_t total = 0, sz = n;
    for (;;) {
        total += sz;
        if (sz <= 1) break;
        sz = (sz + 1) / 2;
    }
    return total;
}

size_t hbrbc_merkle_max_proof_len(size_t n) {
    size_t d = 0, sz = n;
    while (sz > 1) {
        ++d;
        sz = (sz + 1) / 2;
    }
    return d;
}

int hbrbc_frame_batch(hbrbc_ctx *c, const uint8_t *payloads, size_t payload_stride,
                      size_t payload_len, size_t count, uint8_t *shards, size_t shard_len,
                      size_t shard_stride, size_t inst_stride, void *stream) {
    if (!c) return fail(HBRBC_E_INVALID_ARG, "null context");
    if (count == 0) return HBRBC_OK;
    int st = check_payloads(c, payloads, payload_stride, payload_len, shard_len);
    if (st) return st;
    st = check_slab(shards, shard_len, shard_stride, inst_stride, c->n, count);
    if (st) return st;
    HB_HIP(hipSetDevice(c->device));
    return frame_rows(c, payloads, payload_stride, payload_len, count, shards, shard_len,
                      plain_rows(shard_stride), inst_stride, pick(c, stream));
}

int hbrbc_encode_batch(hbrbc_ctx *c, uint8_t *shards, size_t shard_len, size_t shard_stride,
                       size_t inst_stride, size_t count, void *stream) {
    if (!c) return fail(HBRBC_E_INVALID_ARG, "null context");
    if (c->m == 0 || count == 0) return HBRBC_OK;
    if (shard_len == 0) return fail(HBRBC_E_EMPTY_SHARD, "empty shards");
    int st = check_slab(shards, shard_len, shard_stride, inst_stride, c->n, count);
    if (st) return st;
    HB_HIP(hipSetDevice(c->device));
    return encode_rows(c, shards, shard_len, plain_rows(shard_stride), inst_stride, count,
                       pick(c, stream));
}

int hbrbc_frame_encode_rows(hbrbc_ctx *c, const uint8_t *payloads, size_t payload_stride,
                            size_t payload_len, size_t count, uint8_t *shards, size_t shard_len,
                            size_t shard_stride, size_t rows_per_block, size_t block_stride,
                            size_t inst_stride, void *stream) {
    if (!c) return fail(HBRBC_E_INVALID_ARG, "null context");
    if (count == 0) return HBRBC_OK;
    int st = check_payloads(c, payloads, payload_stride, payload_len, shard_len);
    if (st) return st;
    st = check_slab(shards, shard_len, shard_stride, inst_stride, c->n, count, rows_per_block,
                    block_stride);
    if (st) return st;
    HB_HIP(hipSetDevice(c->device));
    hipStream_t s = pick(c, stream);
    const RowMap rows = make_rows(c->n, shard_stride, rows_per_block, block_stride);
    const std::vector<hbrbc_ctx::SpecGroup> *gs = nullptr;
    if (c->m > 0 && shard_stride == round_up(shard_len, 16) && payload_len <= 0x7FFFFFFFull &&
        shard_len * c->k < 0x7FFFFFFFull) {
        gs = spec_encoder(c, code_rb(rows));
        if (!gs && jit_mode() == JIT_LOAD && c->k * c->m <= 16384)
            return fail(HBRBC_E_INVALID_ARG, "HBRBC_JIT=load: %s", c->jit_missing.c_str());
    }
    const char *fe = getenv("HBRBC_FUSE");
// ... 298 lines not shown
    HB_HIP(hipDeviceSynchronize());
    HB_HIP(hipMemcpy(patterns_out, c->pc_fill.p, sizeof(uint32_t), hipMemcpyDeviceToHost));
    return HBRBC_OK;
}

int hbrbc_decoder_specialise(hbrbc_ctx *c, const uint8_t *present, size_t rows_per_block) {
    if (!c || !present) return fail(HBRBC_E_INVALID_ARG, "null argument");
    if (c->m == 0) return HBRBC_OK;
    HB_HIP(hipSetDevice(c->device));
    const int rb = (rows_per_block && rows_per_block < c->n) ? (int)rows_per_block : 256;
    if (rb > 255 && rb != 256) return fail(HBRBC_E_INVALID_ARG, "rows_per_block > 255");
    std::vector<XorProgram> progs;
    uint64_t hash = 0;
    int rt = 2;
    if (!decode_programs(c->matrix, c->k, c->n, present, rb, progs, hash, rt))
        return fail(HBRBC_E_INVALID_ARG, "pattern has nothing to rebuild or too few shards");
    const bool compile = jit_mode() == JIT_DEFAULT || jit_mode() == JIT_COMPILE;
    hbrbc_ctx::DecSpec d;
    d.hash = hash;
    d.rt = rt;
    d.present.assign(present, present + c->n);
    int ng = 0;
    for (const auto &p : progs) {
        hbrbc_ctx::SpecGroup g{0, (int)p.out_rows.size(), nullptr, nullptr, nullptr};
        (void)ng;
        const int st = load_program(p, compile, g);
        if (st) {
            drop_groups(d.groups);
            return st;
        }
        d.groups.push_back(g);
    }
    HB_HIP(hipDeviceSynchronize());
    auto it = c->dec_spec.find(rb);
    if (it != c->dec_spec.end()) {
        drop_groups(it->second.groups);
        drop_groups(it->second.uf_groups);
    }
    c->dec_spec[rb] = std::move(d);
    return HBRBC_OK;
}

size_t hbrbc_jit_decode_groups(size_t data_shards, size_t parity_shards, const uint8_t *present) {
    std::vector<uint8_t> mat;
    const size_t n = data_shards + parity_shards;
    if (!present || data_shards == 0 || n > 256 || !build_matrix(data_shards, n, mat)) return 0;
    std::vector<XorProgram> progs;
    uint64_t hash;
    int rt;
    return decode_programs(mat, data_shards, n, present, 256, progs, hash, rt) ? progs.size() : 0;
}

int hbrbc_jit_build_decode(size_t data_shards, size_t parity_shards, const uint8_t *present,
                           size_t rows_per_block, size_t group, const char *dir) {
    return hbrbc_jit_build_decode_variant(data_shards, parity_shards, present, rows_per_block,
                                          group, 0, dir);
}

int hbrbc_jit_build_decode_variant(size_t data_shards, size_t parity_shards,
                                   const uint8_t *present, size_t rows_per_block, size_t group,
                                   int fused_unframe, const char *dir) {
    std::vector<uint8_t> mat;
    const size_t n = data_shards + parity_shards;
    if (!present || data_shards == 0 || n > 256)
        return fail(HBRBC_E_INVALID_ARG, "need data >= 1, data + parity <= 256, a pattern");
    if (!build_matrix(data_shards, n, mat))
        return fail(HBRBC_E_SINGULAR_MATRIX, "singular Vandermonde top block");
    const int rb = (rows_per_block && rows_per_block < n) ? (int)rows_per_block : 256;
    std::vector<XorProgram> progs;
    uint64_t hash;
    int rt;
    if (!decode_programs(mat, data_shards, n, present, rb, progs, hash, rt, fused_unframe != 0))
        return fail(HBRBC_E_INVALID_ARG, "pattern has nothing to rebuild or too few shards");
    if (group >= progs.size()) return fail(HBRBC_E_INVALID_ARG, "group %zu of %zu", group, progs.size());
    std::vector<char> code;
    std::string log;
    if (compile_source(gen_xor_source(progs[group]), code, log))
        return fail(HBRBC_E_DEVICE, "hiprtc: %s", log.substr(0, 400).c_str());
    const std::string d = dir ? std::string(dir) : jit_dir();
    mkdir(d.c_str(), 0755);
    const std::string path = jit_file(d, progs[group].name);
    return write_file(path, code) ? HBRBC_OK
                                  : fail(HBRBC_E_INVALID_ARG, "cannot write %s", path.c_str());
}

int hbrbc_encode(hbrbc_ctx *c, uint8_t *const *shards, const size_t *lens, size_t n_shards) {
    if (!c) return fail(HBRBC_E_INVALID_ARG, "null context");
    if (c->m == 0) return HBRBC_OK;
    if (n_shards < c->n) return fail(HBRBC_E_TOO_FEW_SHARDS, "%zu < %zu shards", n_shards, c->n);
    if (n_shards > c->n) return fail(HBRBC_E_TOO_MANY_SHARDS, "%zu > %zu shards", n_shards, c->n);
    if (!shards || !lens) return fail(HBRBC_E_INVALID_ARG, "null argument");
    const size_t len = lens[0];
    if (len == 0) return fail(HBRBC_E_EMPTY_SHARD, "empty shard");
    for (size_t i = 0; i < n_shards; ++i)
        if (lens[i] != len) return fail(HBRBC_E_INCORRECT_SHARD_SIZE, "shard %zu length", i);
    std::lock_guard<std::mutex> lk(c->shim_mu);
    HB_HIP(hipSetDevice(c->device));
    const size_t stride = round_up(len, 16);
    HB_HIP(c->st_slab.ensure(c->n * stride));
    HB_HIP(c->pin.ensure(c->n * stride));
    uint8_t *slab = c->st_slab.as<uint8_t>(), *pin = c->pin.as<uint8_t>();
    for (size_t j = 0; j < c->k; ++j) {
        std::memcpy(pin + j * stride, shards[j], len);
        std::memset(pin + j * stride + len, 0, stride - len);
    }
    HB_HIP(hipMemcpyAsync(slab, pin, c->k * stride, hipMemcpyHostToDevice, c->stream));
    int st = encode_rows(c, slab, len, plain_rows(stride), c->n * stride, 1, c->stream);
    if (st) return st;
    HB_HIP(hipMemcpyAsync(pin + c->k * stride, slab + c->k * stride, c->m * stride,
                          hipMemcpyDeviceToHost, c->stream));
    HB_HIP(hipStreamSynchronize(c->stream));
    for (size_t r = c->k; r < c->n; ++r) std::memcpy(shards[r], pin + r * stride, len);
    return HBRBC_OK;
}

int hbrbc_reconstruct(hbrbc_ctx *c, uint8_t *const *shards, const size_t *lens,
                      const uint8_t *present, size_t n_shards) {
    if (!c || !present) return fail(HBRBC_E_INVALID_ARG, "null argument");
    if (c->m == 0) {
        for (size_t i = 0; i < n_shards; ++i)
            if (!present[i]) return fail(HBRBC_E_TOO_FEW_SHARDS_PRESENT, "trivial coding");
        return HBRBC_OK;
    }
    if (n_shards < c->n) return fail(HBRBC_E_TOO_FEW_SHARDS, "%zu < %zu shards", n_shards, c->n);
    if (n_shards > c->n) return fail(HBRBC_E_TOO_MANY_SHARDS, "%zu > %zu shards", n_shards, c->n);
    if (!shards || !lens) return fail(HBRBC_E_INVALID_ARG, "null argument");
    size_t np = 0, len = 0;
    bool have = false;
    for (size_t i = 0; i < n_shards; ++i) {
        if (!present[i]) continue;
        if (lens[i] == 0) return fail(HBRBC_E_EMPTY_SHARD, "shard %zu empty", i);
        ++np;
        if (have && lens[i] != len) return fail(HBRBC_E_INCORRECT_SHARD_SIZE, "shard %zu", i);
        len = lens[i];
        have = true;
    }
    if (np == c->n) return HBRBC_OK;
    if (np < c->k) return fail(HBRBC_E_TOO_FEW_SHARDS_PRESENT, "%zu < %zu present", np, c->k);
    std::lock_guard<std::mutex> lk(c->shim_mu);
    HB_HIP(hipSetDevice(c->device));
    const size_t stride = round_up(len, 16);
    const size_t pres_off = c->n * stride, stat_off = round_up(pres_off + c->n, 16);
    HB_HIP(c->st_slab.ensure(stat_off + 16));
    HB_HIP(c->pin.ensure(stat_off + 16));
    uint8_t *slab = c->st_slab.as<uint8_t>(), *pin = c->pin.as<uint8_t>();
    for (size_t i = 0; i < c->n; ++i) {
        pin[pres_off + i] = present[i] ? 1 : 0;
        if (present[i]) std::memcpy(pin + i * stride, shards[i], len);
        else std::memset(pin + i * stride, 0, len);
        std::memset(pin + i * stride + len, 0, stride - len);
    }
    HB_HIP(hipMemcpyAsync(slab, pin, pres_off + c->n, hipMemcpyHostToDevice, c->stream));
    int32_t *dstat = reinterpret_cast<int32_t *>(slab + stat_off);
    int st = run_reconstruct(c, slab, len, plain_rows(stride), c->n * stride, slab + pres_off, 1,
                             dstat, c->stream);
    if (st) return st;
    HB_HIP(hipMemcpyAsync(pin + stat_off, dstat, sizeof(int32_t), hipMemcpyDeviceToHost,
                          c->stream));
    for (size_t i = 0; i < c->n; ++i)
        if (!present[i])
            HB_HIP(hipMemcpyAsync(pin + i * stride, slab + i * stride, len, hipMemcpyDeviceToHost,
                                  c->stream));
    HB_HIP(hipStreamSynchronize(c->stream));
    int32_t status = 0;
    std::memcpy(&status, pin + stat_off, sizeof status);
    if (status) return fail(status, "reconstruct status %d", status);
// ... 972 lines not shown
```

hbbft_amd/csrc/jit.hip:

```cpp
#include <hip/hip_runtime.h>
#include <hip/hiprtc.h>

#include <algorithm>
#include <cstdio>
#include <cstdlib>
#include <set>
#include <sstream>
#include <string>
#include <vector>

#include "jit.hpp"

namespace hbrbc {

namespace {

uint8_t gf_mul_host(uint8_t a, uint8_t b) {
    uint8_t r = 0;
    while (b) {
        if (b & 1) r ^= a;
        const bool hi = a & 0x80;
        a = (uint8_t)(a << 1);
        if (hi) a ^= 0x1D;
        b >>= 1;
// ... 409 lines not shown
                else
                    o << "      HB_LD(l[" << b << "], h[" << b << "], " << blk(row) << ", " << rin(row) << "u)";
                o << " __asm__ volatile(\"\" ::: \"memory\");\n";
            };
            for (int m = 0; m < depth; ++m) load((size_t)m);
            for (size_t m = 0; m < mine.size(); ++m) {
                const int jj = mine[m];
                const int row = p.in_rows[jj];
                const std::string c = std::to_string(m % nbuf);
                if (m + depth < mine.size()) load(m + depth);
                if (fused) {
                    o << "      { uint32_t x[8];\n";
                    if (p.split)
                        o << "        hb_window2(q0[" << c << "], q2[" << c << "], q1[" << c << "], q3[" << c
                          << "], (" << row << "u * S - 4u) & 3u, x);\n";
                    else
                        o << "        hb_window(q0[" << c << "], q1[" << c << "], q2[" << c << "], (" << row
                          << "u * S - 4u) & 3u, x);\n";
                    if (row < 4)
                        o << "        if (" << row << "u * S < 4u) { if (off == 0u) "
                          << (p.split ? "hb_frame_head2(q0[" + c + "], " : "hb_frame_head(q0[" + c + "], q1[" + c + "], ")
                          << "P, " << row << "u * S, x); }\n";
                    o << "        if (edge) {\n"
                         "          _Pragma(\"unroll\") for (int i_ = 0; i_ < 8; ++i_) {\n"
                         "            const int lim_ = (int)S - (int)(i_ < 4 ? off + 4 * i_ : off2 + 4 * (i_ - 4));\n"
                         "            x[i_] = lim_ >= 4 ? x[i_] : (lim_ <= 0 ? 0u : x[i_] & (0xFFFFFFFFu >> (8 * (4 - lim_))));\n"
                         "          }\n        }\n";
                    if (p.out_rows.front() == nin)
                        o << "        if (active) {\n"
                             "          __builtin_amdgcn_raw_buffer_store_b128((u32x4){x[0], x[1], x[2], x[3]}, rs"
                          << blk(row) << ", off, " << rin(row) << "u * sst, HB_ST_AUX);\n"
                             "          if (full) __builtin_amdgcn_raw_buffer_store_b128((u32x4){x[4], x[5], x[6], x[7]}, "
                             "rs" << blk(row) << ", off2, " << rin(row) << "u * sst, HB_ST_AUX);\n        }\n";
                } else {
                    o << "      { const u32x4 hh = full ? h[" << c << "] : (u32x4)(0u);\n"
                      << "        uint32_t x[8] = {l[" << c << "][0], l[" << c << "][1], l[" << c << "][2], l[" << c
                      << "][3], hh[0], hh[1], hh[2], hh[3]};\n";
                    if (p.uf_k > 0 && p.uf_inputs && row < p.uf_k)
                        o << "        if (ufp && active) { hb_uf_put(ufp, S, " << row
                          << "u, off, x[0], x[1], x[2], x[3]); if (full) hb_uf_put(ufp, S, " << row
                          << "u, off2, x[4], x[5], x[6], x[7]); }\n";
                }
                o << "        hb_tr(x);\n"
                     "        hb_pl[" << (jj - lo) << "][0][lane] = (u32x4){x[0], x[1], x[2], x[3]};\n"
                     "        hb_pl[" << (jj - lo) << "][1][lane] = (u32x4){x[4], x[5], x[6], x[7]};\n"
                     "      }\n";
            }
            if (!mine.empty()) o << "    }\n";
            o << "    __syncthreads();\n";
            for (int jj = lo; jj < hi && rows; ++jj) {
                o << "    { const u32x4 pa_ = hb_pl[" << (jj - lo) << "][0][lane], pb_ = hb_pl[" << (jj - lo)
                  << "][1][lane];\n"
                     "      const uint32_t x[8] = {pa_[0], pa_[1], pa_[2], pa_[3], pb_[0], pb_[1], pb_[2], pb_[3]};\n";
                gen_network(o, cv, t0, rows, (size_t)jj, rt, p.net);
                o << "      for (int t_ = 0; t_ < " << rows << "; ++t_) for (int q_ = 0; q_ < 8; ++q_) "
                     "__asm__ volatile(\"\" : \"+v\"(a[t_][q_]));\n"
                     "      __asm__ volatile(\"\" ::: \"memory\");\n    }\n";
            }
            if (st + 1 < nstage) o << "    __syncthreads();\n";
        }
        if (rows) {
            o << "    if (active) {\n";
            for (int t = 0; t < rows; ++t) {
                const int row = p.out_rows[t0 + t];
                const std::string at = "a[" + std::to_string(t) + "]";
                o << "      { hb_tr(" << at << "); const unsigned so_ = " << rin(row) << "u * sst;\n"
                  << "        __builtin_amdgcn_raw_buffer_store_b128((u32x4){" << at << "[0], " << at << "[1], "
                  << at << "[2], " << at << "[3]}, rs" << blk(row) << ", off, so_, HB_ST_AUX);\n"
                  << "        if (full) __builtin_amdgcn_raw_buffer_store_b128((u32x4){" << at << "[4], " << at
                  << "[5], " << at << "[6], " << at << "[7]}, rs" << blk(row) << ", off2, so_, HB_ST_AUX); }\n";
                if (p.uf_k > 0 && row < p.uf_k)
                    o << "      if (ufp) { hb_uf_put(ufp, S, " << row << "u, off, " << at << "[0], " << at
                      << "[1], " << at << "[2], " << at << "[3]); if (full) hb_uf_put(ufp, S, " << row
                      << "u, off2, " << at << "[4], " << at << "[5], " << at << "[6], " << at << "[7]); }\n";
            }
            o << "    }\n";
        }
        o << "    break; }\n";
    }
    o << "  }\n}\n#undef HB_LD\n" << (fused ? "#undef HB_LDF\n#undef HB_LDF2\n" : "");
    return o.str();
}

}

int xor_waves(int npass) { return std::max(1, std::min(8, npass)); }

std::string encode_kernel_name(size_t k, size_t m, int rt, int depth, int r_lo, int r_hi, int rb,
                               int sync, int fdepth, bool spread, bool split) {
    char b[128];
    snprintf(b, sizeof b, "hbrbc_enc_k%zu_m%zu_rt%d_d%d_r%d_%d", k, m, rt, depth, r_lo, r_hi);
    std::string s = b;
    if (rb < 256) s += "_b" + std::to_string(rb);
    if (sync > 0) s += "_s" + std::to_string(sync);
    if (fdepth != 2) s += "_f" + std::to_string(fdepth);
    if (!spread) s += "_w0";
    if (!split) s += "_c";
    return s;
}

std::string decode_kernel_name(size_t n, uint64_t hash, int rt, int depth, int r_lo, int r_hi,
                               int rb, int sync, bool split) {
    char b[128];
    snprintf(b, sizeof b, "hbrbc_dec_n%zu_%016llx_rt%d_d%d_r%d_%d", n, (unsigned long long)hash,
             rt, depth, r_lo, r_hi);
    std::string s = b;
    if (rb < 256) s += "_b" + std::to_string(rb);
    if (sync > 0) s += "_s" + std::to_string(sync);
    if (!split) s += "_c";
    return s;
}

std::vector<std::pair<int, int>> xor_groups(size_t nin, size_t nout, int rt) {
    const char *ge = getenv("HBRBC_JIT_GROUP");
    const size_t kMaxCoefs = ge ? std::max<size_t>(256, (size_t)atol(ge)) : (size_t)4096;
    std::vector<std::pair<int, int>> g;
    size_t per = nout;
    if (nin * nout > kMaxCoefs) per = std::max<size_t>((size_t)rt, kMaxCoefs / nin / rt * rt);
    if (nin >= 16 && rt <= 8) per = std::min(per, (size_t)(8 * rt));
    for (size_t lo = 0; lo < nout; lo += per) g.push_back({(int)lo, (int)std::min(nout, lo + per)});
    return g;
}

std::string gen_xor_source(const XorProgram &p) {
    const int npass = (int)((p.out_rows.size() + p.rt - 1) / p.rt);
    const bool lds = p.lds && npass >= 2 && npass <= 8;
    auto gen = [&](bool fused) { return lds ? gen_xor_kernel_lds(p, fused) : gen_xor_kernel(p, fused); };
    std::string s = std::string(kPrelude) + gen(false);
    if (p.fused) s += gen(true);
    return s;
}

int compile_source(const std::string &src, std::vector<char> &code, std::string &log) {
    hiprtcProgram prog;
    if (hiprtcCreateProgram(&prog, src.c_str(), "hbrbc_xor.hip", 0, nullptr, nullptr) !=
        HIPRTC_SUCCESS) {
        log = "hiprtcCreateProgram failed";
        return -1;
    }
    const char *aux = getenv("HBRBC_ST_AUX");
    const std::string aux_def = std::string("-DHB_ST_AUX=") + (aux ? aux : "2");
    const char *opts[] = {"--offload-arch=gfx950", "-O3", "-std=c++17", aux_def.c_str()};
    const hiprtcResult r = hiprtcCompileProgram(prog, 4, opts);
    size_t lsz = 0;
    hiprtcGetProgramLogSize(prog, &lsz);
    if (lsz > 1) {
        log.resize(lsz);
        hiprtcGetProgramLog(prog, &log[0]);
    }
    if (r != HIPRTC_SUCCESS) {
        hiprtcDestroyProgram(&prog);
        return -2;
    }
    size_t csz = 0;
    hiprtcGetCodeSize(prog, &csz);
    code.resize(csz);
    hiprtcGetCode(prog, code.data());
    hiprtcDestroyProgram(&prog);
    return 0;
}

}
```

hbbft_amd/csrc/jit.hpp:

```cpp
#pragma once

#include <stddef.h>
#include <stdint.h>

#include <string>
#include <utility>
#include <vector>

namespace hbrbc {

struct XorProgram {
    std::string name;
    std::vector<int> in_rows, out_rows;
    std::vector<uint8_t> coefs;
    int rt = 2, depth = 4, rb = 256;
    int sync = 0;
    int fdepth = 2;
    bool spread = true;
    bool split = true;
    uint64_t guard = 0;
    bool fused = false;
    int uf_k = 0;
    bool uf_inputs = false;
    bool lds = false;
    int lds_stage = 0;
    int net = 0;
    int wpe = 0;
};

struct XorArgs {
    uint8_t *base;
    unsigned long inst_stride, shard_stride, block_stride;
    unsigned row_bytes, waves_per_row;
    const uint8_t *payloads;
    unsigned long payload_stride;
    unsigned P, S;
    const int *pat;
    const unsigned long *slot_hash;
    int hash_slots;
    int p_only;
    uint8_t *uf_payload;
    unsigned long uf_stride;
    const int *uf_status;
};

int xor_waves(int npass);
std::string gen_xor_source(const XorProgram &p);
int compile_source(const std::string &src, std::vector<char> &code, std::string &log);

std::string encode_kernel_name(size_t k, size_t m, int rt, int depth, int r_lo, int r_hi, int rb,
                               int sync = 0, int fdepth = 2, bool spread = true,
                               bool split = false);
std::string decode_kernel_name(size_t n, uint64_t hash, int rt, int depth, int r_lo, int r_hi,
                               int rb, int sync = 0, bool split = true);
std::vector<std::pair<int, int>> xor_groups(size_t nin, size_t nout, int rt);

}
```

hbbft_amd/csrc/kernels.hip:

```cpp
#include <algorithm>
#include <cstdlib>
#include <cstring>

#include "device_common.hpp"
#include "launchers.hpp"

namespace hbrbc {

namespace {

constexpr int kBlock = 256;

inline unsigned grid_for(size_t threads, size_t cap = 256 * 32) {
    size_t b = (threads + kBlock - 1) / kBlock;
    if (b == 0) b = 1;
    if (b > cap) b = cap;
    return (unsigned)b;
}

__device__ __forceinline__ uint4 funnel16(const uint32_t (&d)[5], uint32_t sh) {
    if (sh == 0) return make_uint4(d[0], d[1], d[2], d[3]);
    return make_uint4(__builtin_amdgcn_alignbit(d[1], d[0], sh),
                      __builtin_amdgcn_alignbit(d[2], d[1], sh),
                      __builtin_amdgcn_alignbit(d[3], d[2], sh),
// ... 85 lines not shown
            byte = (P >> (8 * (3 - b))) & 0xFFu;
        else
            byte = (b - 4 < P) ? pay[b - 4] : 0u;
        w[q >> 2] |= byte << (8 * (q & 3));
    }
    *dst = make_uint4(w[0], w[1], w[2], w[3]);
}

__global__ __launch_bounds__(kBlock) void frame_fixup_kernel(
    const uint8_t *__restrict__ payloads, size_t payload_stride, uint32_t P,
    uint8_t *__restrict__ shards, uint32_t S, RowMap rows, size_t inst_stride,
    uint32_t k, uint32_t m, const uint8_t *__restrict__ matrix, size_t count) {
    const size_t inst = blockIdx.x * (size_t)kBlock + threadIdx.x;
    if (inst >= count) return;
    const uint8_t *pay = payloads + inst * payload_stride;
    uint8_t *ib = shards + inst * inst_stride;
    for (uint32_t t = P & ~3u; t < P; ++t) {
        const uint8_t v = pay[t];
        const uint32_t b = t + 4, j = b / S, pos = b - j * S;
        ib[rows.off(j) + pos] = v;
        if (!v) continue;
        for (uint32_t r = 0; r < m; ++r) {
            const uint8_t c = matrix[(size_t)(k + r) * k + j];
            if (c) ib[rows.off(k + r) + pos] ^= kGf.exp[kGf.log[c] + kGf.log[v]];
        }
    }
}

#ifndef HB_NT
#define HB_NT 1
#endif
typedef unsigned int hb_u32x4 __attribute__((ext_vector_type(4)));
__device__ __forceinline__ void store16_stream(void *p, uint32_t a, uint32_t b, uint32_t c,
                                               uint32_t d) {
#if HB_NT
    __builtin_nontemporal_store((hb_u32x4){a, b, c, d}, reinterpret_cast<hb_u32x4 *>(p));
#else
    *reinterpret_cast<uint4 *>(p) = make_uint4(a, b, c, d);
#endif
}

__device__ __forceinline__ void bs_transpose(uint32_t (&w)[8]) {
#pragma unroll
    for (int s = 0; s < 3; ++s) {
        const int d = 1 << s;
        const uint32_t m = s == 0 ? 0x55555555u : (s == 1 ? 0x33333333u : 0x0F0F0F0Fu);
#pragma unroll
        for (int i = 0; i < 8; ++i) {
            if (i & d) continue;
            const uint32_t x = w[i], y = w[i | d];
            const uint32_t t = ((x >> d) ^ y) & m;
            w[i | d] = y ^ t;
            w[i] = x ^ (t << d);
        }
    }
}

typedef uint32_t hb_u32x4_a1 __attribute__((ext_vector_type(4), aligned(1)));
__device__ __forceinline__ void unframe_put(uint8_t *pb, uint32_t S, uint32_t row, uint32_t pos,
                                            uint32_t a, uint32_t b, uint32_t c, uint32_t d) {
    const int64_t dst = (int64_t)row * S + pos - 4;
    if (pos + 16 <= S && dst >= 0)
        *reinterpret_cast<hb_u32x4_a1 *>(pb + dst) = (hb_u32x4_a1){a, b, c, d};
}

__device__ __forceinline__ uint32_t rfl(uint32_t v) {
    return (uint32_t)__builtin_amdgcn_readfirstlane((int)v);
}

template <int RT, int MODE>
#ifdef HB_GF_WPE
#define HB_GF_ATTR __attribute__((amdgpu_waves_per_eu(HB_GF_WPE)))
#else
#define HB_GF_ATTR
#endif
__global__ __launch_bounds__(256) HB_GF_ATTR void gf_bitslice_kernel(
    uint8_t *__restrict__ base, size_t inst_stride, RowMap rows, uint32_t row_bytes,
    const uint8_t *__restrict__ coefs, size_t coef_slot_stride,
    const uint32_t *__restrict__ in_idx, size_t in_idx_stride,
    const uint32_t *__restrict__ out_idx, size_t out_idx_stride,
    const int *__restrict__ nout_arr, int nout_uniform, const int *__restrict__ pat,
    const uint64_t *__restrict__ slot_hash, uint64_t skip_hash, int hash_slots, int nin,
    uint32_t waves_per_row, uint32_t piece, uint8_t *__restrict__ uf_payload, size_t uf_stride,
    uint32_t uf_S, uint32_t uf_k, const int32_t *__restrict__ uf_status) {
    const size_t inst = blockIdx.x / waves_per_row;
    const int slot = pat ? pat[inst] : (int)inst;
    if (skip_hash && slot < hash_slots && slot_hash[slot] == skip_hash) return;
    const int wave = (int)(threadIdx.x >> 6), nwaves = (int)(blockDim.x >> 6);
    const uint32_t wchunk = blockIdx.x - (uint32_t)inst * waves_per_row, lane = threadIdx.x & 63;
    uint32_t off = piece == 16 ? (wchunk * 64 + lane) * 32 : wchunk * 2048 + lane * 16;
    const bool active = off < row_bytes;
    if (!active) off = row_bytes - 16;
    const bool full = off + piece + 16 <= row_bytes;
    const uint32_t d2 = full ? piece : 0;
    uint8_t *ib = base + inst * inst_stride;
    const int nout = nout_arr ? nout_arr[slot] : nout_uniform;
    const int npass = (nout + RT - 1) / RT;
    const uint8_t *cf = coefs + (size_t)slot * coef_slot_stride;
    const uint32_t *iidx = in_idx + (size_t)slot * in_idx_stride;
    const uint32_t *oidx = out_idx + (size_t)slot * out_idx_stride;
    uint8_t *ufp = (uf_payload && uf_status[inst] == 0) ? uf_payload + inst * uf_stride : nullptr;
    if (ufp && npass == 0 && wave == 0 && active) {
        for (uint32_t r = 0; r < uf_k; ++r) {
            const uint8_t *src = ib + rows.off(r) + off;
            const uint4 l = *reinterpret_cast<const uint4 *>(src);
            unframe_put(ufp, uf_S, r, off, l.x, l.y, l.z, l.w);
            if (full) {
                const uint4 h = *reinterpret_cast<const uint4 *>(src + d2);
                unframe_put(ufp, uf_S, r, off + d2, h.x, h.y, h.z, h.w);
            }
        }
    }
    for (int p = __builtin_amdgcn_readfirstlane(wave); p < npass; p += nwaves) {
        uint32_t acc[RT][8];
#pragma unroll
        for (int t = 0; t < RT; ++t)
#pragma unroll
            for (int q = 0; q < 8; ++q) acc[t][q] = 0u;
        const uint4 *cfp = reinterpret_cast<const uint4 *>(cf) + (size_t)p * nin;
        auto row_of = [&](int jj) { return iidx[jj < nin ? jj : nin - 1]; };
        auto coef_of = [&](int jj) { return cfp[jj < nin ? jj : nin - 1]; };
        auto load_row = [&](uint32_t r, uint4 &l, uint4 &h) {
            const uint8_t *src = ib + rows.off(r) + off;
            l = *reinterpret_cast<const uint4 *>(src);
            h = *reinterpret_cast<const uint4 *>(src + d2);
        };
        auto consume = [&](uint32_t r, const uint4 &cw, const uint4 &lo, const uint4 &h) {
            const uint4 hi = full ? h : make_uint4(0, 0, 0, 0);
            if (ufp && p == 0) {
                if (r < uf_k && active) {
                    unframe_put(ufp, uf_S, r, off, lo.x, lo.y, lo.z, lo.w);
                    if (full) unframe_put(ufp, uf_S, r, off + d2, hi.x, hi.y, hi.z, hi.w);
                }
            }
            uint32_t x[8] = {lo.x, lo.y, lo.z, lo.w, hi.x, hi.y, hi.z, hi.w};
            bs_transpose(x);
            const uint32_t c4[4] = {cw.x, cw.y, cw.z, cw.w};
            if constexpr (MODE == 3) {
#pragma unroll
                for (int b = 0; b < 8; b += 2) {
                    const uint32_t h = x[(7 - b) & 7];
                    const uint32_t o[3] = {x[(1 - b) & 7], x[(2 - b) & 7], x[(3 - b) & 7]};
                    x[(1 - b) & 7] ^= h;
                    x[(2 - b) & 7] ^= h;
                    x[(3 - b) & 7] ^= h;
                    auto lo_plane = [&](int q) {
                        const int i = (q - b) & 7;
                        return i == ((1 - b) & 7) ? o[0] : i == ((2 - b) & 7) ? o[1]
                                                         : i == ((3 - b) & 7) ? o[2] : x[i];
                    };
#pragma unroll
                    for (int t = 0; t < RT; ++t) {
                        const uint32_t two = (c4[t >> 2] >> (8 * (t & 3) + b)) & 3u;
                        if (two == 3u) {
#pragma unroll
                            for (int q = 0; q < 8; ++q) acc[t][q] ^= lo_plane(q) ^ x[(q - b - 1) & 7];
                        } else if (two == 1u) {
#pragma unroll
                            for (int q = 0; q < 8; ++q) acc[t][q] ^= lo_plane(q);
                        } else if (two == 2u) {
#pragma unroll
                            for (int q = 0; q < 8; ++q) acc[t][q] ^= x[(q - b - 1) & 7];
                        }
                    }
                    if (b < 6) {
                        const uint32_t h2 = x[(6 - b) & 7];
                        x[(0 - b) & 7] ^= h2;
                        x[(1 - b) & 7] ^= h2;
                        x[(2 - b) & 7] ^= h2;
                    }
// ... 674 lines not shown
        for (int col0 = 0; col0 < d; ++col0) {
            if (tid < 64) {
                int p = -1;
                for (int r0 = col0; r0 < d && p < 0; r0 += 64) {
                    const int r = r0 + tid;
                    const unsigned long long bal = __ballot(r < d && aug[r * w2 + col0] != 0);
                    if (bal) p = r0 + __ffsll((long long)bal) - 1;
                }
                if (tid == 0) meta[2] = p;
            }
            if (tid == 0) {
                const int p = meta[2];
                if (p < 0)
                    meta[4] = 1;
                else
                    meta[3] = gf_inv_lds(exp_t, log_t, aug[p * w2 + col0]);
            }
            __syncthreads();
            if (meta[4]) {
                if (tid == 0) {
                    c.nout[slot] = 0;
                    c.status[slot] = 64;
                }
                return;
            }
            const int p = meta[2];
            const uint8_t inv = (uint8_t)meta[3];
            if (p != col0) {
                for (int col = tid; col < w2; col += nt) {
                    uint8_t t = aug[col0 * w2 + col];
                    aug[col0 * w2 + col] = aug[p * w2 + col];
                    aug[p * w2 + col] = t;
                }
            }
            __syncthreads();
            for (int col = tid; col < w2; col += nt)
                aug[col0 * w2 + col] = gf_mul_lds(exp_t, log_t, inv, aug[col0 * w2 + col]);
            __syncthreads();
            for (int r = tid; r < d; r += nt) fac[r] = (r == col0) ? 0 : aug[r * w2 + col0];
            __syncthreads();
            for (int e = tid; e < d * w2; e += nt) {
                const int r = e / w2, col = e - r * w2;
                const uint8_t f = fac[r];
                if (f) aug[e] ^= gf_mul_lds(exp_t, log_t, f, aug[col0 * w2 + col]);
            }
            __syncthreads();
        }
        for (int e = tid; e < d * kd; e += nt) {
            const int i = e / kd, cc = e - i * kd;
            uint8_t acc = 0;
            for (int r = 0; r < d; ++r)
                acc ^= gf_mul_lds(exp_t, log_t, aug[i * w2 + d + r],
                                  matrix[(size_t)valid[kd + r] * k + valid[cc]]);
            X[e] = acc;
        }
        __syncthreads();
    }
    uint8_t *tab = c.coefs + (size_t)slot * c.coef_stride;
    const int nrows = (nm + rt - 1) / rt * rt;
    for (int e = tid; e < nrows * k; e += nt) {
        const int t = e / k, j = e - t * k;
        const int row = t < nm ? missing[t] : -1;
        uint8_t coef = 0;
        if (row < 0) {
            coef = 0;
        } else if (row < k) {
            coef = j < kd ? X[t * kd + j] : aug[t * w2 + d + (j - kd)];
        } else {
            const uint8_t *mr = matrix + (size_t)row * k;
            if (j < kd) {
                coef = mr[valid[j]];
                for (int i = 0; i < d; ++i) coef ^= gf_mul_lds(exp_t, log_t, mr[missing[i]], X[i * kd + j]);
            } else {
                for (int i = 0; i < d; ++i)
                    coef ^= gf_mul_lds(exp_t, log_t, mr[missing[i]], aug[i * w2 + d + (j - kd)]);
            }
        }
        tab[((size_t)(t / rt) * k + j) * 16 + (t % rt)] = coef;
    }
    for (int j = tid; j < k; j += nt) c.in_idx[(size_t)slot * k + j] = valid[j];
    for (int t = tid; t < nm; t += nt) c.out_idx[(size_t)slot * m + t] = missing[t];
    if (tid == 0) {
        c.nout[slot] = nm;
        c.status[slot] = 0;
    }
}

__global__ __launch_bounds__(kBlock) void pattern_status_kernel(
    size_t count, const int *__restrict__ pat, const int32_t *__restrict__ slot_status,
    int32_t *__restrict__ status) {
    const size_t inst = blockIdx.x * (size_t)kBlock + threadIdx.x;
    if (inst < count) status[inst] = slot_status[pat[inst]];
}

__device__ __forceinline__ uint8_t logical_byte(const uint8_t *ib, uint64_t b, uint32_t S,
                                                const RowMap &rows) {
    const uint32_t r = (uint32_t)b / S;
    return ib[rows.off(r) + ((uint32_t)b - r * S)];
}

__global__ __launch_bounds__(kBlock) void decode_check_kernel(
    const int32_t *__restrict__ recon_status, const uint8_t *__restrict__ nodes,
    size_t node_inst_stride, uint32_t root_node, const uint8_t *__restrict__ roots,
    size_t root_stride, const uint8_t *__restrict__ shards, uint32_t S, RowMap rows,
    size_t inst_stride, uint32_t k, size_t count, uint32_t *__restrict__ plen_out,
    int32_t *__restrict__ status_out) {
    const size_t inst = blockIdx.x * (size_t)kBlock + threadIdx.x;
    if (inst >= count) return;
    int32_t st = recon_status[inst];
    uint32_t len = 0;
    if (st == 0) {
        uint32_t a[8], b[8];
        load_digest(nodes + inst * node_inst_stride + (size_t)root_node * 32, a);
        load_digest(roots + inst * root_stride, b);
        bool same = true;
#pragma unroll
        for (int w = 0; w < 8; ++w) same = same && a[w] == b[w];
        const uint64_t total = (uint64_t)k * S;
        if (!same) {
            st = 65;
        } else if (total < 4) {
            st = 66;
        } else {
            const uint8_t *ib = shards + inst * inst_stride;
            uint32_t v = 0;
            for (int q = 0; q < 4; ++q) v = (v << 8) | logical_byte(ib, (uint64_t)q, S, rows);
            len = (uint32_t)min<uint64_t>((uint64_t)v, total - 4);
        }
    }
    plen_out[inst] = len;
    status_out[inst] = st;
}

__global__ __launch_bounds__(kBlock) void unframe_kernel(
    const uint8_t *__restrict__ shards, uint32_t S, RowMap rows, size_t inst_stride,
    uint32_t k, const uint32_t *__restrict__ plen, const int32_t *__restrict__ status,
    uint8_t *__restrict__ payload_out, size_t payload_stride, uint32_t chunks,
    uint32_t blocks_per_inst) {
    const size_t inst = blockIdx.x / blocks_per_inst;
    const uint32_t c = (blockIdx.x - (uint32_t)inst * blocks_per_inst) * kBlock + threadIdx.x;
    if (c >= chunks) return;
    const uint32_t len = status[inst] == 0 ? plen[inst] : 0u;
    const uint32_t o = c * 16;
    uint32_t w[4] = {0u, 0u, 0u, 0u};
    if (o < len) {
        const uint64_t total = (uint64_t)k * S;
        const uint8_t *ib = shards + inst * inst_stride;
        const uint64_t lb = 4 + (uint64_t)o;
        const uint32_t row = (uint32_t)lb / S;
        const uint32_t off = (uint32_t)lb - row * S;
        const uint32_t sh = off & 15u;
        const uint32_t sh0 = __builtin_amdgcn_readfirstlane(sh);
        const uint8_t *rp = ib + rows.off(row);
        if (__all(off + 16 <= S && sh == sh0)) {
            const uint4 v = load16_shifted(rp + (off - sh), sh0);
            w[0] = v.x; w[1] = v.y; w[2] = v.z; w[3] = v.w;
        } else if (off + 16 <= S) {
            const uint32_t *rw = reinterpret_cast<const uint32_t *>(rp) + (off >> 2);
            const uint32_t s8 = (off & 3) * 8;
            uint32_t d[5];
#pragma unroll
            for (int q = 0; q < 4; ++q) d[q] = rw[q];
            d[4] = s8 ? rw[4] : 0u;
            const uint4 v = funnel16(d, s8);
            w[0] = v.x; w[1] = v.y; w[2] = v.z; w[3] = v.w;
        } else {
// ... 62 lines not shown
    for (int i = 0; i < 8; ++i) w[i] = 0;
    for (int i = 0; i < n && i < 256; ++i)
        if (present[i]) w[i / 32] |= 1u << (i % 32);
}

uint64_t pattern_hash(const uint8_t *present, int n) {
    uint32_t w[8];
    pattern_mask(present, n, w);
    return pat_hash_words(w, n);
}

hipError_t configure_kernels() {
    int dev = 0;
    hipError_t e = hipGetDevice(&dev);
    if (e != hipSuccess) return e;
    e = hipDeviceGetAttribute(&g_num_cus, hipDeviceAttributeMultiprocessorCount, dev);
    if (e != hipSuccess) return e;
    for (const void *k : {reinterpret_cast<const void *>(decode_matrix_kernel),
                          reinterpret_cast<const void *>(leaf_hash_kernel<false>),
                          reinterpret_cast<const void *>(leaf_hash_kernel<true>),
                          reinterpret_cast<const void *>(leaf_hash_list_kernel),

                          reinterpret_cast<const void *>(validate_kernel<false>),
                          reinterpret_cast<const void *>(validate_kernel<true>)}) {
        e = hipFuncSetAttribute(k, hipFuncAttributeMaxDynamicSharedMemorySize, 160 * 1024);
        if (e != hipSuccess) return e;
    }
    for (const void *k : {reinterpret_cast<const void *>(merkle_tree_kernel<false>),
                          reinterpret_cast<const void *>(merkle_tree_kernel<true>)}) {
        e = hipFuncSetAttribute(k, hipFuncAttributeMaxDynamicSharedMemorySize,
                                160 * 1024 - 2 * kBlock * 32);
        if (e != hipSuccess) return e;
    }
    return hipSuccess;
}

hipError_t launch_frame(const uint8_t *payloads, size_t payload_stride, size_t payload_len,
                        size_t count, uint8_t *shards, size_t shard_len, const RowMap &rows,
                        size_t inst_stride, size_t data_shards, hipStream_t s,
                        const uint32_t *plens, size_t row_fill) {
    const size_t chunks = ((plens ? row_fill : shard_len) + 15) / 16;
    if (count == 0 || chunks == 0) return hipSuccess;
    const size_t bpr = (chunks + kBlock - 1) / kBlock;
    const size_t blocks = bpr * count * data_shards;
    if (blocks > 0xFFFFFFFFull) return hipErrorInvalidValue;
    hipLaunchKernelGGL(frame_kernel, dim3((unsigned)blocks), dim3(kBlock), 0, s, payloads,
                       payload_stride, (uint32_t)payload_len, shards, (uint32_t)shard_len, rows,
                       inst_stride, (uint32_t)data_shards, (uint32_t)bpr, plens,
                       (uint32_t)(plens ? row_fill : 0));
    return hipGetLastError();
}

hipError_t launch_frame_fixup(const uint8_t *payloads, size_t payload_stride, size_t payload_len,
                              uint8_t *shards, size_t shard_len, const RowMap &rows,
                              size_t inst_stride, size_t k, size_t m, const uint8_t *matrix,
                              size_t count, hipStream_t s) {
    if (count == 0 || (payload_len & 3) == 0) return hipSuccess;
    hipLaunchKernelGGL(frame_fixup_kernel, dim3(grid_for(count, (size_t)1 << 30)), dim3(kBlock), 0,
                       s, payloads, payload_stride, (uint32_t)payload_len, shards,
                       (uint32_t)shard_len, rows, inst_stride, (uint32_t)k, (uint32_t)m, matrix,
                       count);
    return hipGetLastError();
}

hipError_t launch_gf_apply(const GfApplyArgs &a, hipStream_t s) {
    if (a.count == 0 || a.n16 == 0) return hipSuccess;
    if (!a.nout && a.nout_uniform == 0) return hipSuccess;
    const uint32_t row_bytes = (uint32_t)a.n16 * 16;
    const uint32_t wpr = (row_bytes + 64 * 32 - 1) / (64 * 32);
    const size_t blocks = (size_t)wpr * a.count;
    if (blocks > 0xFFFFFFFFull) return hipErrorInvalidValue;
    const int max_rows = a.nout ? a.max_rows : a.nout_uniform;
    const int npass_max = std::max(1, (max_rows + a.rt - 1) / a.rt);
    const int path = (npass_max + 3) / 4;
    int nw = std::max(1, std::min(4, (npass_max + path - 1) / path));
    if (const char *we = getenv("HBRBC_GF_WAVES")) nw = std::max(1, std::min(4, atoi(we)));
    const char *pe = getenv("HBRBC_GF_SPLIT");
    const uint32_t piece = (pe && !strcmp(pe, "0")) ? 16u : 1024u;
#define HB_BS_LAUNCH(RT, MODE)                                                                   \
    hipLaunchKernelGGL((gf_bitslice_kernel<RT, MODE>), dim3((unsigned)blocks), dim3(64 * nw), 0, \
                       s, a.base, a.inst_stride, a.rows, row_bytes, a.coefs, a.coef_slot_stride, \
                       a.in_idx, a.in_idx_stride, a.out_idx, a.out_idx_stride, a.nout,          \
                       a.nout_uniform, a.pat, a.slot_hash, a.skip_hash, a.hash_slots, a.nin, wpr,   \
                       piece, a.payload, a.payload_stride, a.payload_S, a.payload_k, a.rstatus)
#define HB_BS_CASE(RT)                                                                           \
    case RT:                                                                                     \
        if (a.mode == 4)                                                                         \
            HB_BS_LAUNCH(RT, 4);                                                                 \
        else if (a.mode == 3)                                                                    \
            HB_BS_LAUNCH(RT, 3);                                                                 \
        else if (a.mode == 2)                                                                    \
            HB_BS_LAUNCH(RT, 2);                                                                 \
        else if (a.mode == 1)                                                                    \
            HB_BS_LAUNCH(RT, 1);                                                                 \
        else                                                                                     \
            HB_BS_LAUNCH(RT, 0);                                                                 \
        break
    switch (a.rt) {
        HB_BS_CASE(2);
        HB_BS_CASE(4);
        HB_BS_CASE(5);
        HB_BS_CASE(6);
        HB_BS_CASE(7);
        HB_BS_CASE(8);
        HB_BS_CASE(10);
        HB_BS_CASE(12);
        HB_BS_CASE(14);
        HB_BS_CASE(16);
        default:
            return hipErrorInvalidValue;
    }
#undef HB_BS_CASE
#undef HB_BS_LAUNCH
    return hipGetLastError();
}

int gf_row_tile(int rows) {
    if (rows <= 0) return 2;
    const int passes = (rows + 15) / 16;
    int rt = (rows + passes - 1) / passes;
    rt = (rt + 1) & ~1;
    return rt < 2 ? 2 : (rt > 16 ? 16 : rt);
}

hipError_t launch_leaf_hash(const uint8_t *shards, size_t shard_len, const RowMap &rows,
                            size_t inst_stride, size_t n, size_t count, uint8_t *nodes,
                            size_t node_inst_stride, hipStream_t s, const uint32_t *slens) {
    const size_t total = n * count;
    if (total == 0) return hipSuccess;
    if (pair_sponges(total)) {
        hipLaunchKernelGGL(leaf_hash_pl_kernel, dim3(grid_for(2 * total, (size_t)1 << 30)),
                           dim3(kBlock), 0, s, shards, (uint32_t)shard_len, rows, inst_stride,
                           (uint32_t)n, total, nodes, node_inst_stride, slens);
        return hipGetLastError();
    }
    const bool v16 = few_sponges(total);
    hipLaunchKernelGGL(v16 ? leaf_hash_kernel<true> : leaf_hash_kernel<false>,
                       dim3(grid_for(total, (size_t)1 << 30)), dim3(kBlock),
                       v16 ? 0 : shaped_lds(total, kSpongeMaxWaves), s, shards, (uint32_t)shard_len,
                       rows, inst_stride, (uint32_t)n, total, nodes, node_inst_stride, slens);
    return hipGetLastError();
}

bool merkle_fused_ok(size_t n) {
    return n >= 2 && n <= (size_t)kBlock && (kBlock % n) * 16 <= (size_t)kBlock;
}

hipError_t launch_merkle_fused(const uint8_t *shards, size_t shard_len, const RowMap &rows,
                               size_t inst_stride, size_t n, size_t count, uint8_t *nodes,
                               size_t node_inst_stride, hipStream_t s, const uint32_t *slens) {
    if (count == 0) return hipSuccess;
    if (!merkle_fused_ok(n)) return hipErrorInvalidValue;
    const size_t ipb = kBlock / n;
    const size_t blocks = (count + ipb - 1) / ipb;
    if (blocks > 0xFFFFFFFFull) return hipErrorInvalidValue;
    const bool v16 = few_sponges(count * n);
    const size_t dyn = v16 ? 0 : shaped_lds(blocks * kBlock, kSpongeMaxWaves, 2 * kBlock * 32);
    hipLaunchKernelGGL(v16 ? merkle_tree_kernel<true> : merkle_tree_kernel<false>, dim3((unsigned)blocks),
                       dim3(kBlock), dyn, s, shards, (uint32_t)shard_len, rows, inst_stride,
                       (uint32_t)n, (uint32_t)ipb, count, nodes, node_inst_stride, slens);
    return hipGetLastError();
}

hipError_t launch_leaf_hash_rebuilt(const uint8_t *shards, size_t shard_len, const RowMap &rows,
                                    size_t inst_stride, size_t count, const int *pat,
                                    const uint32_t *out_idx, size_t out_idx_stride,
                                    const int *nout, int max_rows, uint8_t *nodes,
// ... 233 lines not shown
```

hbbft_amd/csrc/launchers.hpp:

```cpp
#pragma once

#include <hip/hip_runtime.h>
#include <stddef.h>
#include <stdint.h>

#include "../../include/hbrbc.h"

namespace hbrbc {

struct RowMap {
    uint64_t sst = 0, bst = 0;
    uint32_t rb = 0xFFFFFFFFu;
    __host__ __device__ __forceinline__ uint64_t off(uint32_t j) const {
        if (j < rb) return (uint64_t)j * sst;
        const uint32_t q = j / rb;
        return (uint64_t)q * bst + (uint64_t)(j - q * rb) * sst;
    }
    __host__ __device__ __forceinline__ bool plain() const { return rb == 0xFFFFFFFFu; }
};
inline RowMap plain_rows(size_t sst) {
    RowMap r;
    r.sst = sst;
    return r;
}

hipError_t launch_frame(const uint8_t *payloads, size_t payload_stride, size_t payload_len,
                        size_t count, uint8_t *shards, size_t shard_len, const RowMap &rows,
                        size_t inst_stride, size_t data_shards, hipStream_t s,
                        const uint32_t *plens = nullptr, size_t row_fill = 0);

hipError_t launch_frame_fixup(const uint8_t *payloads, size_t payload_stride, size_t payload_len,
                              uint8_t *shards, size_t shard_len, const RowMap &rows,
                              size_t inst_stride, size_t k, size_t m, const uint8_t *matrix,
                              size_t count, hipStream_t s);

struct GfApplyArgs {
    uint8_t *base;
    size_t inst_stride;
    RowMap rows;
    int n16;
    const uint8_t *coefs;
    size_t coef_slot_stride;
    const uint32_t *in_idx;
    size_t in_idx_stride;
    const uint32_t *out_idx;
    size_t out_idx_stride;
    const int *nout;
    int nout_uniform;
    const int *pat;
    const uint64_t *slot_hash;
    uint64_t skip_hash;
    int hash_slots;
    int max_rows;
    int nin;
    int rt;
    int mode;
    size_t count;
    uint8_t *payload = nullptr;
    size_t payload_stride = 0;
    uint32_t payload_S = 0, payload_k = 0;
    const int32_t *rstatus = nullptr;
};
int gf_row_tile(int rows);
hipError_t launch_gf_apply(const GfApplyArgs &a, hipStream_t s);

hipError_t launch_leaf_hash(const uint8_t *shards, size_t shard_len, const RowMap &rows,
                            size_t inst_stride, size_t n, size_t count, uint8_t *nodes,
                            size_t node_inst_stride, hipStream_t s,
                            const uint32_t *slens = nullptr);
bool merkle_fused_ok(size_t n);
hipError_t launch_merkle_fused(const uint8_t *shards, size_t shard_len, const RowMap &rows,
                               size_t inst_stride, size_t n, size_t count, uint8_t *nodes,
                               size_t node_inst_stride, hipStream_t s,
                               const uint32_t *slens = nullptr);
hipError_t launch_leaf_hash_rebuilt(const uint8_t *shards, size_t shard_len, const RowMap &rows,
                                    size_t inst_stride, size_t count, const int *pat,
                                    const uint32_t *out_idx, size_t out_idx_stride,
                                    const int *nout, int max_rows, uint8_t *nodes,
                                    size_t node_inst_stride, uint32_t *counter, uint2 *list,
                                    hipStream_t s);
hipError_t launch_ragged_hash(const uint8_t *base, const uint64_t *offsets,
                              const uint32_t *lens, size_t nvals, uint8_t *out, hipStream_t s);
hipError_t launch_tree_level(uint8_t *nodes, size_t node_inst_stride, size_t prev_off,
                             size_t prev_size, size_t cur_off, size_t cur_size, size_t count,
                             hipStream_t s);
hipError_t launch_tree_levels(uint8_t *nodes, size_t node_inst_stride, size_t n, size_t count,
                              hipStream_t s);
hipError_t launch_proofs(const uint8_t *nodes, size_t node_inst_stride, size_t n, size_t count,
                         uint8_t *digests, size_t dslots, uint8_t *ndig, hipStream_t s);
struct ValidateArgs {
    const uint8_t *values;
    size_t value_len, value_inst_stride, per_inst;
    RowMap vrows;
    const uint32_t *rows;
    const uint32_t *indices;
    const uint8_t *digests;
    size_t dslots, dig_rows;
    const uint8_t *ndig;
    const uint8_t *roots;
    size_t root_stride, tree_n, count;
    uint8_t *ok_out;
    uint8_t *leaf_out;
    size_t leaf_inst_stride;
};
hipError_t launch_validate(const ValidateArgs &a, hipStream_t s);

struct PatternCache {
    uint64_t *hash;
    uint32_t *keys;
    uint8_t *coefs;
    size_t coef_stride;
    uint32_t *in_idx;
    uint32_t *out_idx;
    int *nout;
    int32_t *status;
    uint32_t *fill;
    int cap;
};
struct DecodeMatrixArgs {
    int n, k, rt;
    const uint8_t *matrix;
    const uint8_t *present;
    size_t count;
    PatternCache cache;
    int *pat;
    uint8_t *own;
    int32_t *status;
    uint64_t spec_hash = 0;
    uint32_t spec_mask[8] = {};
};
hipError_t launch_decode_matrix(const DecodeMatrixArgs &a, hipStream_t s);
uint64_t pattern_hash(const uint8_t *present, int n);
void pattern_mask(const uint8_t *present, int n, uint32_t (&w)[8]);

hipError_t launch_decode_check(const int32_t *recon_status, const uint8_t *nodes,
                               size_t node_inst_stride, size_t root_node, const uint8_t *roots,
                               size_t root_stride, const uint8_t *shards, size_t shard_len,
                               const RowMap &rows, size_t inst_stride, size_t data_shards,
                               size_t count, uint32_t *plen_out, int32_t *status_out,
                               hipStream_t s);
hipError_t launch_unframe_fixup(const uint8_t *shards, uint32_t S, const RowMap &rows,
                                size_t inst_stride, uint32_t k, size_t count, const uint32_t *plen,
                                const int32_t *status, uint8_t *payload_out, size_t payload_stride,
                                hipStream_t s);
hipError_t launch_unframe(const uint8_t *shards, size_t shard_len, const RowMap &rows,
                          size_t inst_stride, size_t data_shards, size_t count,
                          const uint32_t *plen, const int32_t *status, uint8_t *payload_out,
                          size_t payload_stride, hipStream_t s);

hipError_t launch_drop_rows(uint8_t *shards, size_t shard_stride, const RowMap &rows,
                            size_t inst_stride, size_t n, size_t count, const uint8_t *present,
                            uint8_t fill, hipStream_t s);

struct WireEncodeArgs {
    uint32_t variant;
    const uint8_t *values;
    size_t value_len, value_stride, value_inst_stride, per_inst;
    const uint32_t *indices;
    const uint8_t *digests;
    size_t dslots;
    const uint8_t *ndig;
    const uint8_t *roots;
    size_t root_stride, count;
    uint8_t *out;
    size_t msg_stride;
    uint32_t *msg_len;
};
hipError_t launch_wire_encode(const WireEncodeArgs &a, hipStream_t s);
struct WireDecodeArgs {
    const uint8_t *msgs;
    size_t msg_stride;
    const uint32_t *msg_len;
    size_t nmsg;
    uint8_t *values;
    size_t value_stride, value_cap;
    uint32_t *value_len, *index;
    uint8_t *digests;
    size_t dslots;
    uint8_t *ndig, *roots;
    uint32_t *variant;
    int32_t *status;
};
hipError_t launch_wire_decode(const WireDecodeArgs &a, hipStream_t s);

hipError_t launch_pairing_miller(const uint8_t *g1, size_t g1_stride, const uint8_t *g2,
                                 size_t g2_stride, size_t n, int pair_inputs, uint32_t *ws,
                                 uint8_t *status, hipStream_t s);
hipError_t launch_pairing_miller2(const uint8_t *g1, const uint8_t *g2, size_t count,
                                  uint32_t *ws, uint8_t *status, hipStream_t s);
size_t pairing_prepared_words(size_t points);
hipError_t launch_g2_prepare(const uint8_t *g2, size_t count, uint32_t *prep, uint8_t *pst,
                             hipStream_t s);
hipError_t launch_pairing_miller_prepared(const uint8_t *g1, const uint32_t *prep,
                                          const uint8_t *pst, const uint32_t *ib,
                                          const uint32_t *id, size_t points, size_t count,
                                          uint32_t *ws, uint8_t *status, hipStream_t s);
size_t g1_key_words(size_t points);
// ... 91 lines not shown
```

include/hbrbc.h:

```cpp
#ifndef HBRBC_H
#define HBRBC_H

#include <stddef.h>
#include <stdint.h>

#ifdef __cplusplus
extern "C" {
#endif

enum hbrbc_status {
    HBRBC_OK = 0,
    HBRBC_E_TOO_FEW_SHARDS = 1,
    HBRBC_E_TOO_MANY_SHARDS = 2,
    HBRBC_E_TOO_FEW_DATA_SHARDS = 3,
    HBRBC_E_TOO_MANY_DATA_SHARDS = 4,
    HBRBC_E_TOO_FEW_PARITY_SHARDS = 5,
    HBRBC_E_TOO_MANY_PARITY_SHARDS = 6,
    HBRBC_E_TOO_FEW_BUFFER_SHARDS = 7,
    HBRBC_E_TOO_MANY_BUFFER_SHARDS = 8,
    HBRBC_E_INCORRECT_SHARD_SIZE = 9,
    HBRBC_E_TOO_FEW_SHARDS_PRESENT = 10,
    HBRBC_E_EMPTY_SHARD = 11,
    HBRBC_E_INVALID_SHARD_FLAGS = 12,
    HBRBC_E_INVALID_INDEX = 13,
// ... 58 lines not shown
                         size_t value_stride, size_t value_inst_stride, size_t per_inst,
                         const uint32_t *indices, const uint8_t *digests, const uint8_t *ndig,
                         const uint8_t *roots, size_t root_stride, size_t tree_n, size_t count,
                         uint8_t *ok_out, void *stream);
int hbrbc_reconstruct_batch(hbrbc_ctx *ctx, uint8_t *shards, size_t shard_len,
                            size_t shard_stride, size_t inst_stride, const uint8_t *present,
                            size_t count, int32_t *status_out, void *stream);
int hbrbc_decode_batch(hbrbc_ctx *ctx, uint8_t *shards, size_t shard_len, size_t shard_stride,
                       size_t inst_stride, const uint8_t *present, size_t count,
                       const uint8_t *roots, size_t root_stride, uint8_t *nodes,
                       size_t node_inst_stride, uint8_t *payload_out, size_t payload_stride,
                       uint32_t *payload_len_out, int32_t *status_out, void *stream);
int hbrbc_reserve(hbrbc_ctx *ctx, size_t count);

int hbrbc_frame_encode_rows(hbrbc_ctx *ctx, const uint8_t *payloads, size_t payload_stride,
                            size_t payload_len, size_t count, uint8_t *shards, size_t shard_len,
                            size_t shard_stride, size_t rows_per_block, size_t block_stride,
                            size_t inst_stride, void *stream);
int hbrbc_merkle_rows(hbrbc_ctx *ctx, const uint8_t *shards, size_t shard_len, size_t shard_stride,
                      size_t rows_per_block, size_t block_stride, size_t inst_stride, size_t count,
                      uint8_t *nodes, size_t node_inst_stride, void *stream);
int hbrbc_validate_rows(hbrbc_ctx *ctx, const uint8_t *values, size_t value_len,
                        size_t value_stride, size_t rows_per_block, size_t block_stride,
                        size_t value_inst_stride, size_t per_inst, const uint32_t *rows,
                        const uint32_t *indices, const uint8_t *digests, const uint8_t *ndig,
                        size_t digest_rows, const uint8_t *roots, size_t root_stride,
                        size_t tree_n, size_t count, uint8_t *ok_out, uint8_t *leaf_out,
                        size_t leaf_inst_stride, void *stream);
int hbrbc_reconstruct_rows(hbrbc_ctx *ctx, uint8_t *shards, size_t shard_len, size_t shard_stride,
                           size_t rows_per_block, size_t block_stride, size_t inst_stride,
                           const uint8_t *present, size_t count, int32_t *status_out,
                           void *stream);
int hbrbc_decode_rows(hbrbc_ctx *ctx, uint8_t *shards, size_t shard_len, size_t shard_stride,
                      size_t rows_per_block, size_t block_stride, size_t inst_stride,
                      const uint8_t *present, size_t count, const uint8_t *roots,
                      size_t root_stride, uint8_t *nodes, size_t node_inst_stride,
                      int known_leaves, uint8_t *payload_out, size_t payload_stride,
                      uint32_t *payload_len_out, int32_t *status_out, void *stream);

int hbrbc_drop_rows(hbrbc_ctx *ctx, uint8_t *shards, size_t shard_stride, size_t rows_per_block,
                    size_t block_stride, size_t inst_stride, const uint8_t *present, size_t count,
                    uint8_t fill, void *stream);

int hbrbc_decode_cache_clear(hbrbc_ctx *ctx);
int hbrbc_decode_cache_fill(hbrbc_ctx *ctx, uint32_t *patterns_out);
int hbrbc_decoder_specialise(hbrbc_ctx *ctx, const uint8_t *present, size_t rows_per_block);

size_t hbrbc_wire_proof_message_len(size_t value_len, size_t ndig);
int hbrbc_wire_encode_batch(hbrbc_ctx *ctx, uint32_t variant, const uint8_t *values,
                            size_t value_len, size_t value_stride, size_t value_inst_stride,
                            size_t per_inst, const uint32_t *indices, const uint8_t *digests,
                            const uint8_t *ndig, const uint8_t *roots, size_t root_stride,
                            size_t count, uint8_t *out, size_t msg_stride, uint32_t *msg_len_out,
                            void *stream);
int hbrbc_wire_decode_batch(hbrbc_ctx *ctx, const uint8_t *msgs, size_t msg_stride,
                            const uint32_t *msg_len, size_t nmsg, uint8_t *values,
                            size_t value_stride, uint32_t *value_len_out, uint32_t *index_out,
                            uint8_t *digests, uint8_t *ndig_out, uint8_t *roots,
                            uint32_t *variant_out, int32_t *status_out, void *stream);

const char *hbrbc_encode_kernel(const hbrbc_ctx *ctx);
int hbrbc_jit_build_encode(size_t data_shards, size_t parity_shards, const char *dir);
size_t hbrbc_jit_encode_groups(size_t data_shards, size_t parity_shards);
int hbrbc_jit_build_encode_group(size_t data_shards, size_t parity_shards, size_t group,
                                 const char *dir);
int hbrbc_jit_file_name(size_t data_shards, size_t parity_shards, size_t group, char *buf,
                        size_t buf_len);
int hbrbc_jit_build_encode_rows(size_t data_shards, size_t parity_shards, size_t group,
                                size_t rows_per_block, const char *dir);
int hbrbc_jit_encode_file_name(size_t data_shards, size_t parity_shards, size_t group,
                               size_t rows_per_block, char *buf, size_t buf_len);
size_t hbrbc_jit_decode_groups(size_t data_shards, size_t parity_shards, const uint8_t *present);
int hbrbc_jit_build_decode(size_t data_shards, size_t parity_shards, const uint8_t *present,
                           size_t rows_per_block, size_t group, const char *dir);
int hbrbc_jit_build_decode_variant(size_t data_shards, size_t parity_shards,
                                   const uint8_t *present, size_t rows_per_block, size_t group,
                                   int fused_unframe, const char *dir);
int hbrbc_jit_decode_variant_file_name(size_t data_shards, size_t parity_shards,
                                       const uint8_t *present, size_t rows_per_block,
                                       size_t group, int fused_unframe, char *buf,
                                       size_t buf_len);
int hbrbc_jit_decode_file_name(size_t data_shards, size_t parity_shards, const uint8_t *present,
                               size_t rows_per_block, size_t group, char *buf, size_t buf_len);

enum hbrbc_stage {
    HBRBC_STAGE_FRAME = 0,
    HBRBC_STAGE_ENCODE = 1,
    HBRBC_STAGE_LEAF_HASH = 2,
    HBRBC_STAGE_TREE_LEVELS = 3,
    HBRBC_STAGE_PROOFS = 4,
    HBRBC_STAGE_VALIDATE = 5,
    HBRBC_STAGE_DECODE_MATRIX = 6,
    HBRBC_STAGE_RECONSTRUCT = 7,
    HBRBC_STAGE_UNFRAME = 8,
    HBRBC_STAGE_COUNT = 9
};
int hbrbc_profile_enable(hbrbc_ctx *ctx, int enable);
int hbrbc_profile_reset(hbrbc_ctx *ctx);
int hbrbc_profile_read(hbrbc_ctx *ctx, double *ms_out, uint64_t *launches_out);
const char *hbrbc_stage_name(int stage);

int hbrbc_unframe_fused(const hbrbc_ctx *ctx, size_t shard_len, size_t payload_stride,
                        size_t rows_per_block);

#define HBRBC_G1_BYTES 96
#define HBRBC_G2_BYTES 192
#define HBRBC_GT_BYTES 576
size_t hbrbc_pairing_workspace_size(size_t pairings);
int hbrbc_pairing_batch(const uint8_t *g1, const uint8_t *g2, size_t count, uint8_t *gt_out,
                        uint8_t *status_out, void *workspace, void *stream);
int hbrbc_pairing_check_batch(const uint8_t *g1, const uint8_t *g2, size_t count,
                              uint8_t *ok_out, void *workspace, void *stream);
size_t hbrbc_g2_prepared_size(size_t points);
int hbrbc_g2_prepare(const uint8_t *g2, size_t count, void *prepared, void *stream);
int hbrbc_pairing_check_prepared(const uint8_t *g1, const void *prepared, size_t points,
                                 const uint32_t *idx_b, const uint32_t *idx_d, size_t count,
                                 uint8_t *ok_out, void *workspace, void *stream);
size_t hbrbc_g1_prepared_size(size_t points);
int hbrbc_g1_prepare(const uint8_t *g1, size_t count, void *prepared, void *stream);
int hbrbc_pairing_check_prepared_keys(const uint8_t *g1_a, const void *keys, size_t key_points,
                                      const uint32_t *idx_c, const void *prepared, size_t points,
                                      const uint32_t *idx_b, const uint32_t *idx_d, size_t count,
                                      uint8_t *ok_out, void *workspace, void *stream);
int hbrbc_pairing_check_prepared_pts(const void *a_prepared, const void *keys, size_t key_points,
                                     const uint32_t *idx_c, const void *prepared, size_t points,
                                     const uint32_t *idx_b, const uint32_t *idx_d, size_t count,
                                     uint8_t *ok_out, void *workspace, void *stream);
int hbrbc_pairing_check(const uint8_t a[96], const uint8_t b[192], const uint8_t c[96],
                        const uint8_t d[192], int *result);
#define HBRBC_G1_COMPRESSED_BYTES 48
#define HBRBC_FR_BYTES 32
size_t hbrbc_g1_combine_workspace_size(size_t total_shares, size_t groups);
int hbrbc_lagrange_coeffs(const uint32_t *idx, const uint32_t *offsets, size_t groups,
                          uint8_t *coeffs_out, uint8_t *status_out, void *stream);
int hbrbc_g1_lincomb_prepared(const void *a_prepared, size_t prepared_count, const int32_t *rows,
                              const uint8_t *scalars, const uint32_t *offsets, size_t groups,
                              uint8_t *out96, uint8_t *out48, uint8_t *status_out,
                              void *workspace, void *stream);
int hbrbc_decrypt_combine_prepared(const void *a_prepared, size_t prepared_count,
                                   const int32_t *rows, const uint32_t *idx,
                                   const uint32_t *offsets, size_t groups, uint8_t *out96,
                                   uint8_t *out48, uint8_t *status_out, void *workspace,
                                   void *stream);
int hbrbc_decrypt_combine(const uint8_t *shares, const uint32_t *idx, size_t n, uint8_t out96[96],
                          uint8_t out48[48]);

int hbrbc_g1_poly_eval_prepared(const void *a_prepared, size_t prepared_count, const int32_t *rows,
                                const uint32_t *offsets, size_t polys, const int32_t *poly,
                                const uint32_t *x, size_t evals, void *out_table, uint8_t *out96,
                                uint8_t *out48, uint8_t *status_out, void *stream);
int hbrbc_g1_base_mul_check(const void *a_prepared, size_t prepared_count, const int32_t *rows,
                            const uint8_t *scalars, size_t count, uint8_t *ok_out, void *stream);

#define HBRBC_G2_COMPRESSED_BYTES 96
size_t hbrbc_g2_points_size(size_t points);
int hbrbc_g2_points_prepare(const uint8_t *g2, size_t count, void *table, void *stream);
int hbrbc_sig_check_prepared(const void *sig_table, size_t sig_count, const void *keys,
                             size_t key_points, const uint32_t *idx_key, const void *prepared,
                             size_t points, const uint32_t *idx_h, size_t count, uint8_t *ok_out,
                             void *workspace, void *stream);
size_t hbrbc_g2_combine_workspace_size(size_t total_shares, size_t groups);
int hbrbc_g2_lincomb_prepared(const void *sig_table, size_t sig_count, const int32_t *rows,
                              const uint8_t *scalars, const uint32_t *offsets, size_t groups,
                              uint8_t *out192, uint8_t *out96, uint8_t *parity_out,
                              uint8_t *status_out, void *workspace, void *stream);
int hbrbc_sig_combine_prepared(const void *sig_table, size_t sig_count, const int32_t *rows,
// ... 76 lines not shown
```

Before: 109.3 GB/s.

## Add JIT repair kernel fusing data-row rebuild and parity regeneration in one pass

Adds a JIT-generated repair kernel for small k (k<=32, k*m<=1024). It rebuilds up to dcap missing data rows with the per-pattern cached coefficients, accumulating in LDS with workgroup-scope atomic XORs. It then regenerates missing parity rows through straight-line bit-sliced XOR networks baked from the parity matrix, optionally fusing the unframe step. The generic GF apply kernel skips instances the repair kernel handles, which is meant to cut the generic per-pattern reconstruct cost and extra passes over HBM. In exchange it adds build-time JIT variants, extra LDS and register pressure, and new env knobs.

Measured after the change: 110.0 GB/s (median of 6 runs). No clear change (+0.5%).

```diff
diff --git a/__graft_entry__.py b/__graft_entry__.py
--- a/__graft_entry__.py
+++ b/__graft_entry__.py
@@ -52,6 +52,7 @@
         kinds = ["dec", "decuf"]
         tasks += [(kind, k, m, g, rb, tuple(pres)) for kind in kinds
                   for g in range(hbbft_amd.jit_decode_groups(k, m, pres))]
+    tasks += [(kind, k, m, 0, 0, None) for k, m in REPAIR for kind in ("rep", "repuf")]
     return tasks
 
 
@@ -73,6 +74,8 @@
     import hbbft_amd
     if kind == "enc":
         return hbbft_amd.jit_file_name(k, m, group, rb)
+    if kind in ("rep", "repuf"):
+        return hbbft_amd.jit_repair_file_name(k, m, fused_unframe=kind == "repuf")
     return hbbft_amd.jit_decode_file_name(k, m, list(present), group, rb,
                                           fused_unframe=kind == "decuf")
 
@@ -93,12 +96,15 @@
     import hbbft_amd
     if kind == "enc":
         hbbft_amd.jit_build_encode(k, m, group=group, rows_per_block=rb)
+    elif kind in ("rep", "repuf"):
+        hbbft_amd.jit_build_repair(k, m, fused_unframe=kind == "repuf")
     else:
         hbbft_amd.jit_build_decode(k, m, list(present), group, rows_per_block=rb,
                                    fused_unframe=kind == "decuf")
 
 
 SPECIALISED = [(2, 2), (6, 10), (22, 42), (44, 84), (84, 166)]
+REPAIR = [(2, 2), (6, 10), (22, 42)]
 VALIDATOR_BLOCKS = {16: [8, 4, 2], 64: [32, 16, 8], 128: [64, 32, 16]}
 
 
diff --git a/hbbft-hip/src/ffi.rs b/hbbft-hip/src/ffi.rs
--- a/hbbft-hip/src/ffi.rs
+++ b/hbbft-hip/src/ffi.rs
@@ -91,6 +91,9 @@
     pub fn hbrbc_jit_build_decode_variant(data_shards: usize, parity_shards: usize, present: *const u8, rows_per_block: usize, group: usize, fused_unframe: c_int, dir: *const c_char) -> c_int;
     pub fn hbrbc_jit_decode_variant_file_name(data_shards: usize, parity_shards: usize, present: *const u8, rows_per_block: usize, group: usize, fused_unframe: c_int, buf: *mut c_char, buf_len: usize) -> c_int;
     pub fn hbrbc_jit_decode_file_name(data_shards: usize, parity_shards: usize, present: *const u8, rows_per_block: usize, group: usize, buf: *mut c_char, buf_len: usize) -> c_int;
+    pub fn hbrbc_jit_build_repair(data_shards: usize, parity_shards: usize, fused_unframe: c_int, dir: *const c_char) -> c_int;
+    pub fn hbrbc_jit_repair_file_name(data_shards: usize, parity_shards: usize, fused_unframe: c_int, buf: *mut c_char, buf_len: usize) -> c_int;
+    pub fn hbrbc_repair_info(ctx: *mut HbrbcCtx, fused_unframe: c_int, loaded: *mut c_int, dcap: *mut c_int) -> c_int;
     pub fn hbrbc_profile_enable(ctx: *mut HbrbcCtx, enable: c_int) -> c_int;
     pub fn hbrbc_profile_reset(ctx: *mut HbrbcCtx) -> c_int;
     pub fn hbrbc_profile_read(ctx: *mut HbrbcCtx, ms_out: *mut f64, launches_out: *mut u64) -> c_int;
diff --git a/hbbft_amd/__init__.py b/hbbft_amd/__init__.py
--- a/hbbft_amd/__init__.py
+++ b/hbbft_amd/__init__.py
@@ -6,7 +6,7 @@
     "shard_len", "merkle_node_count", "max_proof_len", "lib", "LIB_PATH", "STAGES",
     "jit_build_encode", "jit_file_name", "WIRE_VARIANTS", "validate_proofs", "VALIDATE_STATS",
     "send_shards_batch", "SEND_STATS", "jit_decode_groups", "jit_build_decode",
-    "jit_decode_file_name", "jit_encode_groups",
+    "jit_decode_file_name", "jit_encode_groups", "jit_build_repair", "jit_repair_file_name",
 ]
 
 _HERE = os.path.dirname(os.path.abspath(__file__))
@@ -118,6 +118,10 @@
                                                           ctypes.c_char_p]),
         "hbrbc_jit_decode_variant_file_name": (ctypes.c_int, [_S, _S, _P, _S, _S, ctypes.c_int,
                                                               ctypes.c_char_p, _S]),
+        "hbrbc_jit_build_repair": (ctypes.c_int, [_S, _S, ctypes.c_int, ctypes.c_char_p]),
+        "hbrbc_jit_repair_file_name": (ctypes.c_int, [_S, _S, ctypes.c_int, ctypes.c_char_p, _S]),
+        "hbrbc_repair_info": (ctypes.c_int, [_P, ctypes.c_int, ctypes.POINTER(ctypes.c_int),
+                                             ctypes.POINTER(ctypes.c_int)]),
         "hbrbc_unframe_fused": (ctypes.c_int, [_P, _S, _S, _S]),
         "hbrbc_drop_rows": (ctypes.c_int, [_P, _P, _S, _S, _S, _S, _P, _S, ctypes.c_uint8, _P]),
         "hbrbc_pairing_workspace_size": (_S, [_S]),
@@ -222,6 +226,18 @@
     return buf.value.decode()
 
 
+def jit_build_repair(data_shards, parity_shards, fused_unframe=False, directory=None):
+    d = directory.encode() if directory else None
+    _check(lib().hbrbc_jit_build_repair(data_shards, parity_shards, int(fused_unframe), d))
+
+
+def jit_repair_file_name(data_shards, parity_shards, fused_unframe=False):
+    buf = ctypes.create_string_buffer(256)
+    _check(lib().hbrbc_jit_repair_file_name(data_shards, parity_shards, int(fused_unframe),
+                                            buf, 256))
+    return buf.value.decode()
+
+
 def jit_encode_groups(data_shards, parity_shards):
     return lib().hbrbc_jit_encode_groups(data_shards, parity_shards)
 
@@ -630,6 +646,12 @@
         assert m.size == self.n
         _check(lib().hbrbc_decoder_specialise(self.coding.handle, m.ctypes.data, rows_per_block))
 
+    def repair_info(self, fused_unframe=False):
+        loaded, dcap = ctypes.c_int(0), ctypes.c_int(0)
+        _check(lib().hbrbc_repair_info(self.coding.handle, int(fused_unframe),
+                                       ctypes.byref(loaded), ctypes.byref(dcap)))
+        return bool(loaded.value), dcap.value
+
     def decode_cache_clear(self):
         _check(lib().hbrbc_decode_cache_clear(self.coding.handle))
 
diff --git a/hbbft_amd/csrc/api.hip b/hbbft_amd/csrc/api.hip
--- a/hbbft_amd/csrc/api.hip
+++ b/hbbft_amd/csrc/api.hip
@@ -244,6 +244,13 @@
         std::vector<uint8_t> present;
     };
     std::map<int, DecSpec> dec_spec;
+    struct Repair {
+        bool off = false;
+        int dcap = 0, rpw = 2;
+        int state[2] = {0, 0};
+        hipModule_t mod[2] = {nullptr, nullptr};
+        hipFunction_t fn[2] = {nullptr, nullptr};
+    } repair;
     std::string jit_missing;
     std::vector<hipStream_t> side;
     std::vector<hipEvent_t> side_ev;
@@ -251,7 +258,7 @@
     size_t ws_count = 0;
     int pc_cap = 0;
     size_t pc_inserted = 0;
-    DevBuf pc_hash, pc_keys, pc_coefs, pc_in, pc_out, pc_nout, pc_status, pc_fill;
+    DevBuf pc_hash, pc_keys, pc_coefs, pc_in, pc_out, pc_nout, pc_ndata, pc_status, pc_fill;
     DevBuf ws_pat, ws_own, ws_status, ws_list, ws_counter;
     std::mutex shim_mu;
     DevBuf st_slab, st_nodes, st_aux;
@@ -353,6 +360,7 @@
     HB_HIP(c->pc_in.ensure((slots * k + 4) * sizeof(uint32_t)));
     HB_HIP(c->pc_out.ensure((slots * m + 4) * sizeof(uint32_t)));
     HB_HIP(c->pc_nout.ensure(slots * sizeof(int)));
+    HB_HIP(c->pc_ndata.ensure(slots * sizeof(int)));
     HB_HIP(c->pc_status.ensure(slots * sizeof(int32_t)));
     HB_HIP(c->pc_fill.ensure(sizeof(uint32_t)));
     HB_HIP(c->ws_pat.ensure(count * sizeof(int)));
@@ -377,6 +385,7 @@
     pc.in_idx = c->pc_in.as<uint32_t>();
     pc.out_idx = c->pc_out.as<uint32_t>();
     pc.nout = c->pc_nout.as<int>();
+    pc.ndata = c->pc_ndata.as<int>();
     pc.status = c->pc_status.as<int32_t>();
     pc.fill = c->pc_fill.as<uint32_t>();
     pc.cap = c->pc_cap;
@@ -451,6 +460,7 @@
                      int rb, std::vector<XorProgram> &out, uint64_t &hash, int &rt, bool uf);
 int load_program(const XorProgram &p, bool compile, hbrbc_ctx::SpecGroup &g);
 void drop_groups(std::vector<hbrbc_ctx::SpecGroup> &gs);
+bool repair_ready(hbrbc_ctx *c, bool uf);
 
 bool uf_decoder(hbrbc_ctx *c, hbrbc_ctx::DecSpec &d, int rb) {
     if (d.uf_state == 0) {
@@ -534,6 +544,40 @@
         HB_HIP(launch_groups(c, uf_payload ? ds->second.uf_groups : ds->second.groups, 0,
                              ds->second.rt, x, count, s));
     }
+    const bool repair = rows.plain() && shard_len > 0 && c->n * rows.sst < 0x7FFFFFFFull &&
+                        repair_ready(c, uf_payload != nullptr);
+    if (repair) {
+        const int uf = uf_payload ? 1 : 0;
+        RepairArgs r{};
+        r.base = shards;
+        r.inst_stride = inst_stride;
+        r.shard_stride = rows.sst;
+        r.row_bytes = (unsigned)round_up(shard_len, 16);
+        r.waves_per_row = (r.row_bytes + 64 * 32 - 1) / (64 * 32);
+        r.S = (unsigned)shard_len;
+        r.rt = c->rt_rec;
+        r.pat = c->ws_pat.as<int>();
+        r.slot_hash = reinterpret_cast<const unsigned long *>(c->pc_hash.as<uint64_t>());
+        r.skip_hash = spec ? ds->second.hash : 0;
+        r.hash_slots = c->pc_cap;
+        r.coefs = c->pc_coefs.as<uint8_t>();
+        r.coef_stride = c->coef_stride();
+        r.in_idx = c->pc_in.as<uint32_t>();
+        r.out_idx = c->pc_out.as<uint32_t>();
+        r.nout = c->pc_nout.as<int>();
+        r.ndata = c->pc_ndata.as<int>();
+        r.uf_payload = uf_payload;
+        r.uf_stride = uf_stride;
+        r.uf_status = status;
+        const size_t blocks = (size_t)r.waves_per_row * count;
+        if (blocks > 0xFFFFFFFFull) return fail(HBRBC_E_INVALID_ARG, "too many workgroups");
+        void *args[] = {&r.base,      &r.inst_stride, &r.shard_stride, &r.row_bytes, &r.waves_per_row,
+                        &r.S,         &r.rt,          &r.pat,          &r.slot_hash, &r.skip_hash,
+                        &r.hash_slots, &r.coefs,      &r.coef_stride,  &r.in_idx,    &r.out_idx,
+                        &r.nout,      &r.ndata,       &r.uf_payload,   &r.uf_stride, &r.uf_status};
+        HB_HIP(hipModuleLaunchKernel(c->repair.fn[uf], (unsigned)blocks, 1, 1, 512, 1, 1, 0, s, args,
+                                     nullptr));
+    }
     GfApplyArgs g{};
     g.base = shards;
     g.inst_stride = inst_stride;
@@ -541,6 +585,8 @@
     g.n16 = (int)((shard_len + 15) / 16);
     g.coefs = c->pc_coefs.as<uint8_t>();
     g.coef_slot_stride = c->coef_stride();
+    g.ndata = c->pc_ndata.as<int>();
+    g.repair_dcap = repair ? c->repair.dcap : -1;
     g.in_idx = c->pc_in.as<uint32_t>();
     g.in_idx_stride = c->k;
     g.out_idx = c->pc_out.as<uint32_t>();
@@ -766,6 +812,62 @@
     gs.clear();
 }
 
+int repair_rpw() {
+    if (const char *e = getenv("HBRBC_REPAIR_RPW")) return std::max(1, std::min(12, atoi(e)));
+    return 4;
+}
+
+int repair_knob(const char *name, int def, int lo, int hi) {
+    const char *e = getenv(name);
+    return e ? std::max(lo, std::min(hi, atoi(e))) : def;
+}
+
+RepairProgram repair_program(size_t k, size_t m, const std::vector<uint8_t> &matrix, bool uf) {
+    RepairProgram p;
+    p.k = (int)k;
+    p.m = (int)m;
+    p.dcap = repair_dcap(k, m);
+    p.rpw = repair_rpw();
+    p.wpe = repair_knob("HBRBC_REPAIR_WPE", 6, 2, 8);
+    p.pf = repair_knob("HBRBC_REPAIR_PF", 4, 1, 8);
+    p.uf = uf;
+    p.parity.assign(matrix.begin() + k * k, matrix.begin() + (k + m) * k);
+    p.name = repair_kernel_name(k, m, p.dcap, p.rpw, p.wpe, p.pf, uf);
+    return p;
+}
+
+bool repair_ready(hbrbc_ctx *c, bool uf) {
+    hbrbc_ctx::Repair &r = c->repair;
+    if (r.off || r.dcap == 0) return false;
+    const int v = uf ? 1 : 0;
+    if (r.state[v] == 0) {
+        r.state[v] = -1;
+        const std::string saved = g_err;
+        const RepairProgram p = repair_program(c->k, c->m, c->matrix, uf);
+        const std::string path = jit_file(jit_dir(), p.name);
+        std::vector<char> code;
+        bool have = read_file(path, code);
+        if (!have && (jit_mode() == JIT_DEFAULT || jit_mode() == JIT_COMPILE)) {
+            std::string log;
+            have = compile_source(gen_repair_source(p), code, log) == 0;
+            if (have) {
+                mkdir(jit_dir().c_str(), 0755);
+                (void)write_file(path, code);
+            }
+        }
+        if (have && hipModuleLoadData(&r.mod[v], code.data()) == hipSuccess) {
+            if (hipModuleGetFunction(&r.fn[v], r.mod[v], p.name.c_str()) == hipSuccess) {
+                r.state[v] = 1;
+            } else {
+                (void)hipModuleUnload(r.mod[v]);
+                r.mod[v] = nullptr;
+            }
+        }
+        g_err = saved;
+    }
+    return r.state[v] == 1;
+}
+
 const std::vector<hbrbc_ctx::SpecGroup> *spec_encoder(hbrbc_ctx *c, int rb) {
     auto it = c->enc_spec.find(rb);
     if (it != c->enc_spec.end()) return it->second.empty() ? nullptr : &it->second;
@@ -1035,6 +1137,12 @@
         else if (!std::strcmp(e, "bitslice_pair")) c->gf_mode = 3;
         else if (!std::strcmp(e, "bitslice_x2")) c->gf_mode = 4;
         else c->gf_mode = 0;
+    }
+    {
+        const char *e = getenv("HBRBC_REPAIR");
+        c->repair.off = e ? !std::strcmp(e, "0") : getenv("HBRBC_GF") != nullptr;
+        c->repair.dcap = jit_mode() == JIT_OFF ? 0 : repair_dcap(c->k, c->m);
+        c->repair.rpw = repair_rpw();
     }
     if (const char *e = getenv("HBRBC_RT_ENC")) c->rt_enc = std::max(2, std::min(16, atoi(e) & ~1));
     if (const char *e = getenv("HBRBC_RT_REC")) {
@@ -1098,7 +1206,7 @@
     (void)hipSetDevice(c->device);
     if (c->stream) (void)hipStreamSynchronize(c->stream);
     for (DevBuf *b : {&c->d_matrix, &c->d_enc_coefs, &c->d_enc_in, &c->d_enc_out, &c->pc_hash,
-                      &c->pc_keys, &c->pc_coefs, &c->pc_in, &c->pc_out, &c->pc_nout, &c->pc_status,
+                      &c->pc_keys, &c->pc_coefs, &c->pc_in, &c->pc_out, &c->pc_nout, &c->pc_ndata, &c->pc_status,
                       &c->pc_fill, &c->ws_pat, &c->ws_own, &c->ws_status, &c->ws_list,
                       &c->ws_counter, &c->st_slab, &c->st_nodes, &c->st_aux})
         b->release();
@@ -1111,8 +1219,18 @@
         drop_groups(kv.second.groups);
         drop_groups(kv.second.uf_groups);
     }
+    for (hipModule_t mod : c->repair.mod)
+        if (mod) (void)hipModuleUnload(mod);
     if (c->stream) (void)hipStreamDestroy(c->stream);
     delete c;
+}
+
+int hbrbc_repair_info(hbrbc_ctx *c, int fused_unframe, int *loaded, int *dcap) {
+    if (!c || !loaded || !dcap) return fail(HBRBC_E_INVALID_ARG, "null argument");
+    HB_HIP(hipSetDevice(c->device));
+    *loaded = repair_ready(c, fused_unframe != 0) ? 1 : 0;
+    *dcap = *loaded ? c->repair.dcap : 0;
+    return HBRBC_OK;
 }
 
 size_t hbrbc_data_shard_count(const hbrbc_ctx *c) { return c ? c->k : 0; }
@@ -1577,6 +1695,42 @@
     const std::string path = jit_file(d, progs[group].name);
     return write_file(path, code) ? HBRBC_OK
                                   : fail(HBRBC_E_INVALID_ARG, "cannot write %s", path.c_str());
+}
+
+namespace {
+int repair_for_shape(size_t k, size_t m, int uf, RepairProgram &p) {
+    std::vector<uint8_t> mat;
+    if (k == 0 || k + m > 256) return fail(HBRBC_E_INVALID_ARG, "need data >= 1, data + parity <= 256");
+    if (!build_matrix(k, k + m, mat)) return fail(HBRBC_E_SINGULAR_MATRIX, "singular Vandermonde top block");
+    if (!repair_dcap(k, m)) return fail(HBRBC_E_INVALID_ARG, "no repair program for k = %zu, m = %zu", k, m);
+    p = repair_program(k, m, mat, uf != 0);
+    return HBRBC_OK;
+}
+}
+
+int hbrbc_jit_build_repair(size_t data_shards, size_t parity_shards, int fused_unframe,
+                           const char *dir) {
+    RepairProgram p;
+    if (const int st = repair_for_shape(data_shards, parity_shards, fused_unframe, p)) return st;
+    std::vector<char> code;
+    std::string log;
+    if (compile_source(gen_repair_source(p), code, log))
+        return fail(HBRBC_E_DEVICE, "hiprtc: %s", log.substr(0, 400).c_str());
+    const std::string d = dir ? std::string(dir) : jit_dir();
+    mkdir(d.c_str(), 0755);
+    const std::string path = jit_file(d, p.name);
+    return write_file(path, code) ? HBRBC_OK
+                                  : fail(HBRBC_E_INVALID_ARG, "cannot write %s", path.c_str());
+}
+
+int hbrbc_jit_repair_file_name(size_t data_shards, size_t parity_shards, int fused_unframe,
+                               char *buf, size_t buf_len) {
+    RepairProgram p;
+    if (const int st = repair_for_shape(data_shards, parity_shards, fused_unframe, p)) return st;
+    const std::string name = jit_file("", p.name).substr(1);
+    if (!buf || buf_len <= name.size()) return fail(HBRBC_E_INVALID_ARG, "buffer too small");
+    std::memcpy(buf, name.c_str(), name.size() + 1);
+    return HBRBC_OK;
 }
 
 int hbrbc_encode(hbrbc_ctx *c, uint8_t *const *shards, const size_t *lens, size_t n_shards) {
diff --git a/hbbft_amd/csrc/jit.hip b/hbbft_amd/csrc/jit.hip
--- a/hbbft_amd/csrc/jit.hip
+++ b/hbbft_amd/csrc/jit.hip
@@ -515,6 +515,239 @@
     return o.str();
 }
 
+void gen_row_network(std::ostringstream &o, uint8_t c) {
+    if (!c) return;
+    uint8_t col[8];
+    for (int q = 0; q < 8; ++q) col[q] = gf_mul_host(c, (uint8_t)(1u << q));
+    for (int q = 0; q < 8; ++q) {
+        std::vector<int> terms;
+        for (int pp = 0; pp < 8; ++pp)
+            if ((col[pp] >> q) & 1) terms.push_back(pp);
+        size_t i = 0;
+        for (; i + 1 < terms.size(); i += 2)
+            o << "        a[" << q << "] = __builtin_amdgcn_bitop3_b32(a[" << q << "], x[" << terms[i]
+              << "], x[" << terms[i + 1] << "], 0x96);\n";
+        if (i < terms.size()) o << "        a[" << q << "] ^= x[" << terms[i] << "];\n";
+    }
+}
+
+const char *kRepairHead = R"(
+#define HB_NA ((HB_K + 7) / 8)
+extern "C" __global__ __launch_bounds__(512) __attribute__((amdgpu_waves_per_eu(HB_WPE)))
+void HB_NAME(uint8_t *__restrict__ base, unsigned long inst_stride, unsigned long shard_stride,
+    unsigned row_bytes, unsigned waves_per_row, unsigned S, int rt,
+    const int *__restrict__ pat, const unsigned long *__restrict__ slot_hash,
+    unsigned long skip_hash, int hash_slots,
+    const uint8_t *__restrict__ coefs, unsigned long coef_stride,
+    const unsigned *__restrict__ in_idx, const unsigned *__restrict__ out_idx,
+    const int *__restrict__ nout_arr, const int *__restrict__ ndata,
+    uint8_t *__restrict__ uf_payload, unsigned long uf_stride, const int *__restrict__ uf_status) {
+  // plane slot j: the bit planes of data row j (present: written by stage A,
+  // missing: summed by stage B), [half][lane] 16-byte lane slots
+  __shared__ u32x4 hb_pl[HB_K][2][64];
+  const unsigned long inst = blockIdx.x / waves_per_row;
+  const int slot = pat[inst];
+  // the generic kernel makes the same three tests and takes the other side
+  if (skip_hash && slot < hash_slots && slot_hash[slot] == skip_hash) return;
+  const int nout = nout_arr[slot];
+  if (nout <= 0) return;
+  const int d = ndata[slot];
+  if (d > HB_DCAP) return;
+  const int w = __builtin_amdgcn_readfirstlane((int)(threadIdx.x >> 6));
+  const unsigned wchunk = blockIdx.x - (unsigned)inst * waves_per_row, lane = threadIdx.x & 63u;
+  unsigned off = wchunk * 2048u + lane * 16u;
+  const bool active = off < row_bytes;
+  if (!active) off = row_bytes - 16u;
+  const bool full = off + 1024u + 16u <= row_bytes;
+  const unsigned off2 = full ? off + 1024u : off;
+  uint8_t *const ib = base + inst * inst_stride;
+  const __amdgpu_buffer_rsrc_t rs = __builtin_amdgcn_make_buffer_rsrc(ib, (short)0, 0x7fffffff, 0x00020000);
+  const unsigned sst = (unsigned)shard_stride;
+  const unsigned *const iidx = in_idx + (unsigned long)slot * HB_K;
+  const unsigned *const oidx = out_idx + (unsigned long)slot * HB_M;
+  const int kd = HB_K - d;
+  char *const lp = (char *)hb_pl + lane * 16u;
+#define HB_PLANE(B, H) (*(u32x4 *)(lp + (B) + (H) * 1024u))
+#define HB_STORE(A, ROW) { const unsigned so_ = (ROW) * sst; \
+    __builtin_amdgcn_raw_buffer_store_b128((u32x4){A[0], A[1], A[2], A[3]}, rs, off, so_, HB_ST_AUX); \
+    if (full) __builtin_amdgcn_raw_buffer_store_b128((u32x4){A[4], A[5], A[6], A[7]}, rs, off2, so_, HB_ST_AUX); }
+#if HB_UF
+  uint8_t *const ufp = (uf_payload && uf_status[inst] == 0) ? uf_payload + inst * uf_stride : (uint8_t *)0;
+#define HB_PUT(A, ROW) if (ufp) { hb_uf_put(ufp, S, ROW, off, A[0], A[1], A[2], A[3]); \
+    if (full) hb_uf_put(ufp, S, ROW, off2, A[4], A[5], A[6], A[7]); }
+#else
+#define HB_PUT(A, ROW)
+#endif
+
+  // A. the first k present rows (in_idx: the k - d present data rows
+  // ascending, then d parity rows), input jj by wave jj % 8: loaded once and
+  // transposed once.  A present data row's planes go to its slot for stage C;
+  // every input's planes stay in this wave's registers for stage B.
+  u32x4 l[HB_NA], h[HB_NA];
+  unsigned r_[HB_NA];
+  _Pragma("unroll") for (int i = 0; i < HB_NA; ++i) {
+    const int jj = w + 8 * i;
+    if (jj < HB_K) {
+      r_[i] = iidx[jj];
+      l[i] = __builtin_amdgcn_raw_buffer_load_b128(rs, off, r_[i] * sst, 0);
+      h[i] = __builtin_amdgcn_raw_buffer_load_b128(rs, off2, r_[i] * sst, 0);
+    }
+  }
+  // the slots of the missing data rows start at zero: stage B adds into them
+  for (int t = w; t < d; t += 8) {
+    const unsigned b_ = oidx[t] * 2048u;
+    HB_PLANE(b_, 0) = (u32x4)(0u);
+    HB_PLANE(b_, 1) = (u32x4)(0u);
+  }
+  // (LDS only: the row loads stay in flight across the barrier)
+  __asm__ volatile("s_waitcnt lgkmcnt(0)\n\ts_barrier" ::: "memory");
+  uint32_t xs[HB_NA][8];
+  _Pragma("unroll") for (int i = 0; i < HB_NA; ++i) {
+    const int jj = w + 8 * i;
+    if (jj < HB_K) {
+      const u32x4 hh = full ? h[i] : (u32x4)(0u);
+      uint32_t x[8] = {l[i][0], l[i][1], l[i][2], l[i][3], hh[0], hh[1], hh[2], hh[3]};
+      if (jj < kd) { if (active) { HB_PUT(x, r_[i]) } }
+      hb_tr(x);
+      if (jj < kd) {
+        HB_PLANE(r_[i] * 2048u, 0) = (u32x4){x[0], x[1], x[2], x[3]};
+        HB_PLANE(r_[i] * 2048u, 1) = (u32x4){x[4], x[5], x[6], x[7]};
+      }
+      _Pragma("unroll") for (int q = 0; q < 8; ++q) xs[i][q] = x[q];
+    }
+  }
+
+  // B. the d missing data rows, runtime coefficients (rows t < d of the slot's
+  // table: [A^-1 B | A^-1] over the k inputs).  Every wave multiplies ITS OWN
+  // inputs -- the planes it holds -- into all d rows, HB_RPW rows at a time
+  // sharing each input's doubling chain, and adds its partial rows into the
+  // rows' slots with LDS atomics: the eight waves do equal work whatever d is.
+  {
+    const unsigned *const cf32 = (const unsigned *)(coefs + (unsigned long)slot * coef_stride);
+    for (int tb = 0; tb < d; tb += HB_RPW) {
+      uint32_t a[HB_RPW][8] = {};
+      unsigned ci[HB_RPW], sh[HB_RPW];
+      {   // table [pass][j][16]: row t is byte t % rt of pass t / rt
+        unsigned p_ = (unsigned)tb / (unsigned)rt, q_ = (unsigned)tb - p_ * (unsigned)rt;
+        _Pragma("unroll") for (int r = 0; r < HB_RPW; ++r) {
+          ci[r] = p_ * (HB_K * 4u) + (q_ >> 2);
+          sh[r] = 8u * (q_ & 3u);
+          if (++q_ == (unsigned)rt) { q_ = 0; ++p_; }
+        }
+      }
+      _Pragma("unroll") for (int i = 0; i < HB_NA; ++i) {
+        const int jj = w + 8 * i;
+        if (jj < HB_K) {
+          uint32_t cw[HB_RPW];
+          _Pragma("unroll") for (int r = 0; r < HB_RPW; ++r)   // a row past d: coefficient 0
+            cw[r] = tb + r < d ? (cf32[ci[r] + 4u * (unsigned)jj] >> sh[r]) & 0xFFu : 0u;
+          uint32_t x[8];
+          // (pinned: the next input's doubling chain must not start, and hold
+          // eight more registers, while this one's rows are still summed)
+          _Pragma("unroll") for (int q = 0; q < 8; ++q) { x[q] = xs[i][q]; __asm__ volatile("" : "+v"(x[q])); }
+          // at step b logical plane q of 2^b x is x[(q - b) & 7] (gf_bitslice_kernel)
+          _Pragma("unroll") for (int b = 0; b < 8; ++b) {
+            _Pragma("unroll") for (int r = 0; r < HB_RPW; ++r)
+              if ((cw[r] >> b) & 1u) {
+                _Pragma("unroll") for (int q = 0; q < 8; ++q) a[r][q] ^= x[(q - b) & 7];
+              }
+            if (b < 7) {
+              const uint32_t h_ = x[(7 - b) & 7];
+              x[(1 - b) & 7] ^= h_;
+              x[(2 - b) & 7] ^= h_;
+              x[(3 - b) & 7] ^= h_;
+            }
+          }
+          _Pragma("unroll") for (int r = 0; r < HB_RPW; ++r)
+            _Pragma("unroll") for (int q = 0; q < 8; ++q) __asm__ volatile("" : "+v"(a[r][q]));
+        }
+      }
+      _Pragma("unroll") for (int r = 0; r < HB_RPW; ++r)
+        if (tb + r < d) {
+          unsigned long *const s_ = (unsigned long *)(lp + oidx[tb + r] * 2048u);
+          _Pragma("unroll") for (int q = 0; q < 8; q += 2)
+            (void)__hip_atomic_fetch_xor(s_ + (q >> 2) * 128 + ((q >> 1) & 1),
+                                         (unsigned long)a[r][q] | ((unsigned long)a[r][q + 1] << 32),
+                                         __ATOMIC_RELAXED, __HIP_MEMORY_SCOPE_WORKGROUP);
+        }
+    }
+  }
+  __syncthreads();
+
+  // C. the rows to write, in turn over the waves (last first: the parity
+  // rows' networks start in the first round).  A rebuilt data row t < d is
+  // complete in its slot.  A missing parity row p is M[p] times the k data
+  // rows in slots 0..K-1: one wave-uniform switch per row into that row's
+  // straight-line network.
+  for (int t = nout - 1 - w; t >= 0; t -= 8) {
+    const unsigned orow = oidx[t];
+    uint32_t a[8] = {};
+    u32x4 pa[HB_PF], pb[HB_PF];
+    if (t < d) {
+      pa[0] = HB_PLANE(orow * 2048u, 0);
+      pb[0] = HB_PLANE(orow * 2048u, 1);
+      _Pragma("unroll") for (int q = 0; q < 4; ++q) { a[q] = pa[0][q]; a[4 + q] = pb[0][q]; }
+    } else
+    switch ((int)orow - HB_K) {
+)";
+
+const char *kRepairTail = R"(
+    default: break;
+    }
+    hb_tr(a);
+    if (active) {
+      HB_STORE(a, orow)
+      if (t < d) { HB_PUT(a, orow) }
+    }
+  }
+}
+#undef HB_PLANE
+#undef HB_STORE
+#undef HB_PUT
+#undef HB_NA
+)";
+
+}
+
+int repair_dcap(size_t k, size_t m) {
+    if (k == 0 || m == 0) return 0;
+    if (k > 32 || k * m > 1024) return 0;
+    return (int)std::min<size_t>(16, std::min(k, m));
+}
+
+std::string repair_kernel_name(size_t k, size_t m, int dcap, int rpw, int wpe, int pf, bool uf) {
+    char b[96];
+    snprintf(b, sizeof b, "hbrbc_rep_k%zu_m%zu_c%d_b%d_w%d_p%d%s", k, m, dcap, rpw, wpe, pf,
+             uf ? "_uf" : "");
+    return b;
+}
+
+std::string gen_repair_source(const RepairProgram &p) {
+    std::ostringstream o;
+    o << kPrelude << "#define HB_K " << p.k << "\n#define HB_M " << p.m << "\n#define HB_DCAP " << p.dcap
+      << "\n#define HB_RPW " << p.rpw << "\n#define HB_WPE " << p.wpe << "\n#define HB_PF " << p.pf << "\n#define HB_UF " << (p.uf ? 1 : 0) << "\n#define HB_NAME "
+      << p.name << "\n"
+      << kRepairHead;
+    for (int r = 0; r < p.m; ++r) {
+        o << "    case " << r << ": {\n      __asm__ volatile(\"; parity row " << r << "\" ::: \"memory\");\n";
+        for (int j = 0; j < p.pf && j < p.k; ++j)
+            o << "      pa[" << j << "] = hb_pl[" << j << "][0][lane]; pb[" << j << "] = hb_pl[" << j
+              << "][1][lane];\n";
+        for (int j = 0; j < p.k; ++j) {
+            const int c = j % p.pf;
+            o << "      { const uint32_t x[8] = {pa[" << c << "][0], pa[" << c << "][1], pa[" << c << "][2], pa["
+              << c << "][3], pb[" << c << "][0], pb[" << c << "][1], pb[" << c << "][2], pb[" << c << "][3]};\n";
+            if (j + p.pf < p.k)
+                o << "        pa[" << c << "] = hb_pl[" << j + p.pf << "][0][lane]; pb[" << c << "] = hb_pl[" << j + p.pf
+                  << "][1][lane];\n";
+            o << "        __asm__ volatile(\"\" ::: \"memory\");\n";
+            gen_row_network(o, p.parity[(size_t)r * p.k + j]);
+            o << "        for (int q_ = 0; q_ < 8; ++q_) __asm__ volatile(\"\" : \"+v\"(a[q_]));\n      }\n";
+        }
+        o << "      break; }\n";
+    }
+    o << kRepairTail;
+    return o.str();
 }
 
 int xor_waves(int npass) { return std::max(1, std::min(8, npass)); }
diff --git a/hbbft_amd/csrc/jit.hpp b/hbbft_amd/csrc/jit.hpp
--- a/hbbft_amd/csrc/jit.hpp
+++ b/hbbft_amd/csrc/jit.hpp
@@ -44,6 +44,40 @@
     const int *uf_status;
 };
 
+struct RepairProgram {
+    std::string name;
+    int k = 0, m = 0;
+    int dcap = 0;
+    int rpw = 4;
+    int wpe = 6;
+    int pf = 4;
+    bool uf = false;
+    std::vector<uint8_t> parity;
+};
+
+struct RepairArgs {
+    uint8_t *base;
+    unsigned long inst_stride, shard_stride;
+    unsigned row_bytes, waves_per_row, S;
+    int rt;
+    const int *pat;
+    const unsigned long *slot_hash;
+    unsigned long skip_hash;
+    int hash_slots;
+    const uint8_t *coefs;
+    unsigned long coef_stride;
+    const unsigned *in_idx;
+    const unsigned *out_idx;
+    const int *nout, *ndata;
+    uint8_t *uf_payload;
+    unsigned long uf_stride;
+    const int *uf_status;
+};
+
+int repair_dcap(size_t k, size_t m);
+std::string repair_kernel_name(size_t k, size_t m, int dcap, int rpw, int wpe, int pf, bool uf);
+std::string gen_repair_source(const RepairProgram &p);
+
 int xor_waves(int npass);
 std::string gen_xor_source(const XorProgram &p);
 int compile_source(const std::string &src, std::vector<char> &code, std::string &log);
diff --git a/hbbft_amd/csrc/kernels.hip b/hbbft_amd/csrc/kernels.hip
--- a/hbbft_amd/csrc/kernels.hip
+++ b/hbbft_amd/csrc/kernels.hip
@@ -191,10 +191,12 @@
     const int *__restrict__ nout_arr, int nout_uniform, const int *__restrict__ pat,
     const uint64_t *__restrict__ slot_hash, uint64_t skip_hash, int hash_slots, int nin,
     uint32_t waves_per_row, uint32_t piece, uint8_t *__restrict__ uf_payload, size_t uf_stride,
-    uint32_t uf_S, uint32_t uf_k, const int32_t *__restrict__ uf_status) {
+    uint32_t uf_S, uint32_t uf_k, const int32_t *__restrict__ uf_status,
+    const int *__restrict__ ndata, int repair_dcap) {
     const size_t inst = blockIdx.x / waves_per_row;
     const int slot = pat ? pat[inst] : (int)inst;
     if (skip_hash && slot < hash_slots && slot_hash[slot] == skip_hash) return;
+    if (repair_dcap >= 0 && nout_arr[slot] > 0 && ndata[slot] <= repair_dcap) return;
     const int wave = (int)(threadIdx.x >> 6), nwaves = (int)(blockDim.x >> 6);
     const uint32_t wchunk = blockIdx.x - (uint32_t)inst * waves_per_row, lane = threadIdx.x & 63;
     uint32_t off = piece == 16 ? (wchunk * 64 + lane) * 32 : wchunk * 2048 + lane * 16;
@@ -1035,6 +1037,7 @@
     for (int t = tid; t < nm; t += nt) c.out_idx[(size_t)slot * m + t] = missing[t];
     if (tid == 0) {
         c.nout[slot] = nm;
+        c.ndata[slot] = d;
         c.status[slot] = 0;
     }
 }
@@ -1263,7 +1266,8 @@
                        s, a.base, a.inst_stride, a.rows, row_bytes, a.coefs, a.coef_slot_stride, \
                        a.in_idx, a.in_idx_stride, a.out_idx, a.out_idx_stride, a.nout,          \
                        a.nout_uniform, a.pat, a.slot_hash, a.skip_hash, a.hash_slots, a.nin, wpr,   \
-                       piece, a.payload, a.payload_stride, a.payload_S, a.payload_k, a.rstatus)
+                       piece, a.payload, a.payload_stride, a.payload_S, a.payload_k, a.rstatus,     \
+                       a.ndata, (a.nout && a.ndata) ? a.repair_dcap : -1)
 #define HB_BS_CASE(RT)                                                                           \
     case RT:                                                                                     \
         if (a.mode == 4)                                                                         \
diff --git a/hbbft_amd/csrc/launchers.hpp b/hbbft_amd/csrc/launchers.hpp
--- a/hbbft_amd/csrc/launchers.hpp
+++ b/hbbft_amd/csrc/launchers.hpp
@@ -51,6 +51,8 @@
     const uint64_t *slot_hash;
     uint64_t skip_hash;
     int hash_slots;
+    const int *ndata = nullptr;
+    int repair_dcap = -1;
     int max_rows;
     int nin;
     int rt;
@@ -113,6 +115,7 @@
     uint32_t *in_idx;
     uint32_t *out_idx;
     int *nout;
+    int *ndata;
     int32_t *status;
     uint32_t *fill;
     int cap;
diff --git a/include/hbrbc.h b/include/hbrbc.h
--- a/include/hbrbc.h
+++ b/include/hbrbc.h
@@ -164,6 +164,11 @@
                                        size_t buf_len);
 int hbrbc_jit_decode_file_name(size_t data_shards, size_t parity_shards, const uint8_t *present,
                                size_t rows_per_block, size_t group, char *buf, size_t buf_len);
+int hbrbc_jit_build_repair(size_t data_shards, size_t parity_shards, int fused_unframe,
+                           const char *dir);
+int hbrbc_jit_repair_file_name(size_t data_shards, size_t parity_shards, int fused_unframe,
+                               char *buf, size_t buf_len);
+int hbrbc_repair_info(hbrbc_ctx *ctx, int fused_unframe, int *loaded, int *dcap);
 
 enum hbrbc_stage {
     HBRBC_STAGE_FRAME = 0,
```
